# bruno-maruszczak/lap-time-optimization

Hardware: AMD Instinct MI355X
Metric: MPC solves/sec (N=40, nx=8 [7 + progress s], nu=2) (higher is better)
Workload: dtype f64

## Files before the change

### include/ltompc.h

```cpp
#ifndef LTOMPC_H
#define LTOMPC_H

#ifdef __cplusplus
extern "C" {
#endif

#define LTOMPC_NX 8
#define LTOMPC_NU 2
#define LTOMPC_NO_BOUND 1.0e30
#define LTOMPC_TABLE_ROWS 6
#define LTOMPC_NTHETA 16
#define LTOMPC_NLOOP 24

#define LTOMPC_STATUS_SOLVED 0
#define LTOMPC_STATUS_ACCEPTABLE 1
#define LTOMPC_STATUS_MAX_ITER 2
#define LTOMPC_STATUS_NUMERICAL 3
#define LTOMPC_STATUS_STALLED 4
#define LTOMPC_STATUS_INFEASIBLE 5

typedef struct ltompc_params {
  double mass, inertia_z, length_f, length_r, width;
  double B_f, C_f, D_f, B_r, C_r, D_r;
  double C_m, Cr_0, Cr_2, gravity;
  double ptv;
  double q_n, q_mu, q_vy, q_v, vref_scale, q_B;
  double r_du[LTOMPC_NU];
  double x_lb[LTOMPC_NX], x_ub[LTOMPC_NX];
  double u_lb[LTOMPC_NU], u_ub[LTOMPC_NU];
  double ell_penalty, ell_rho, ell_D_f, ell_D_r;
} ltompc_params;

typedef struct ltompc_options {
  double t_step;
  double tol;
  double acceptable_tol;
  double mu_init;
  double mu_min;
  double kappa_eps;
  double kappa_mu;
  double theta_mu;
  double tau_min;
  double bound_push;
  double s_max;
  double delta_w_first;
  double smooth_eps_min;
  double smooth_scale;
  double mu_init_warm;
  double soft_rho;
  double resto_rho;
  double resto_rho_max;
  double resto_rho_factor;
  double dual_inf_max;
  int max_iter;
  int acceptable_iter;
  int n_linesearch;
  int stall_iter;
  int max_ls_fail;
  int warm_shift;
  int warm_reset_on_fail;
  int periodic_tables;
  int max_soc;
  int resto_sticky;
  int node0_check;
  int warm_fallback_iter;
  int resto_shift_retry;
  int max_mu_stay;
  int infeasible_sticky;
  int latency_mode;
} ltompc_options;

typedef struct ltompc_solver* ltompc_handle;

void ltompc_default_params(ltompc_params* p);
void ltompc_default_options(ltompc_options* o);
const char* ltompc_last_error(void);
const char* ltompc_version(void);

int ltompc_create(const ltompc_params* params, const ltompc_options* options, const double* tables,
                  int n_table, int n_horizon, int batch, int device, ltompc_handle* out);
int ltompc_destroy(ltompc_handle h);

int ltompc_set_stream(ltompc_handle h, void* hip_stream);

int ltompc_set_initial_guess(ltompc_handle h, const double* x0);

int ltompc_make_step(ltompc_handle h, const double* x0, double* u0, int* status, int* iters);

int ltompc_make_step_dev(ltompc_handle h, const double* x0_dev, double* u0_dev);

int ltompc_synchronize(ltompc_handle h);

int ltompc_rollout_dev(ltompc_handle h, double* x_dev, int n_ticks, int n_sub, double* u_log_dev, int* status_log_dev,
                       int* iters_log_dev);
int ltompc_rollout_info(ltompc_handle h, long long* iterations, long long* launches);

int ltompc_get_prediction(ltompc_handle h, double* X, double* U);

int ltompc_get_stats(ltompc_handle h, int* status, int* iters, double* kkt_error, double* objective,
                     double* mu);

int ltompc_get_iterate(ltompc_handle h, double* X, double* C, double* U, double* L1, double* L2);

int ltompc_get_ineq(ltompc_handle h, double* T, double* NU, int* n_ineq);

int ltompc_plant_step(ltompc_handle h, const double* x, const double* u, int n_sub, double* x_next);
int ltompc_plant_step_dev(ltompc_handle h, const double* x_dev, const double* u_dev, int n_sub,
                          double* x_next_dev);

int ltompc_slip_forces(ltompc_handle h, const double* x, int batch, double* alpha, double* Fy);

int ltompc_set_initial_guess_dev(ltompc_handle h, const double* x0_dev);

int ltompc_get_counters(ltompc_handle h, int* n_reg, int* n_lsfail);

int ltompc_get_restoration(ltompc_handle h, int* n_resto, double* violation);

int ltompc_get_recovery(ltompc_handle h, int* n_shift, int* n_fallback, double* g0, int* solver_status, double* penalty);

int ltompc_get_sensitivities(ltompc_handle h, double* du0_dp, double* dX_dp, double* dU_dp, int* ok, double* margin);
int ltompc_sensitivities_dev(ltompc_handle h, double* du0_dp_dev, int* ok_dev);

int ltompc_get_param_sensitivities(ltompc_handle h, double* du0_dth, double* dX_dth, double* dU_dth, int* ok);
int ltompc_param_sensitivities_dev(ltompc_handle h, double* du0_dth_dev, int* ok_dev);

int ltompc_get_adjoint(ltompc_handle h, const double* gX, const double* gU, double* grad_p, double* grad_theta, int* ok);
int ltompc_adjoint_dev(ltompc_handle h, const double* gX_dev, const double* gU_dev, double* grad_p_dev, double* grad_theta_dev,
                       int* ok_dev);

int ltompc_get_adjoint_tables(ltompc_handle h, const double* gX, const double* gU, double* grad_tables, double* slot_grad, int* ok);
int ltompc_adjoint_tables_dev(ltompc_handle h, const double* gX_dev, const double* gU_dev, double* grad_tables_dev, double* slot_grad_dev,
                              int* ok_dev);
int ltompc_adjoint_tables_add_dev(ltompc_handle h, const double* gX_dev, const double* gU_dev, double* grad_tables_dev,
                                  double* slot_grad_dev, int* ok_dev);

int ltompc_get_prediction_dev(ltompc_handle h, double* X_dev, double* U_dev);

int ltompc_get_jvp(ltompc_handle h, const double* dp, const double* dtheta, double* tX, double* tU, int* ok);
int ltompc_jvp_dev(ltompc_handle h, const double* dp_dev, const double* dtheta_dev, double* tX_dev, double* tU_dev, int* ok_dev);

int ltompc_set_u_prev(ltompc_handle h, const double* u_prev);
int ltompc_set_u_prev_dev(ltompc_handle h, const double* u_prev_dev);

#define LTOMPC_TABLE_VALUE_ROWS 4
int ltompc_set_table_values(ltompc_handle h, int row, const double* values);
int ltompc_set_table_values_dev(ltompc_handle h, int row, const double* values_dev);
int ltompc_get_table_values(ltompc_handle h, int row, double* values);

int ltompc_set_table_sets(ltompc_handle h, int n_sets, const double* values, const int* set_of_instance);
int ltompc_set_table_sets_dev(ltompc_handle h, int n_sets, const double* values_dev, const int* set_of_instance_dev);
int ltompc_get_table_sets(ltompc_handle h, int* n_sets, double* values, int* set_of_instance);
int ltompc_get_adjoint_table_sets(ltompc_handle h, const double* gX, const double* gU, double* grad_sets, double* slot_grad, int* ok);
int ltompc_adjoint_table_sets_dev(ltompc_handle h, const double* gX_dev, const double* gU_dev, double* grad_sets_dev, double* slot_grad_dev,
                                  int* ok_dev);
int ltompc_adjoint_table_sets_add_dev(ltompc_handle h, const double* gX_dev, const double* gU_dev, double* grad_sets_dev,
                                      double* slot_grad_dev, int* ok_dev);

int ltompc_set_instance_params(ltompc_handle h, const double* theta);
int ltompc_set_instance_params_dev(ltompc_handle h, const double* theta_dev);
int ltompc_get_instance_params(ltompc_handle h, double* theta);

int ltompc_plant_sensitivities(ltompc_handle h, const double* x, const double* u, int n_sub, double* x_next, double* dxn_dx,
                               double* dxn_du, double* dxn_dtheta);
int ltompc_plant_sensitivities_dev(ltompc_handle h, const double* x_dev, const double* u_dev, int n_sub, double* x_next_dev,
                                   double* dxn_dx_dev, double* dxn_du_dev, double* dxn_dtheta_dev);

int ltompc_loop_begin(ltompc_handle h, int mode);
int ltompc_loop_tick_dev(ltompc_handle h, const double* x_dev, const double* u0_dev, int n_sub, double* x_next_dev);
int ltompc_loop_tick(ltompc_handle h, const double* x, const double* u0, int n_sub, double* x_next);
int ltompc_get_loop_sensitivities(ltompc_handle h, double* dx_dq, double* du_dq, int* ok, int* ticks);
int ltompc_loop_sensitivities_dev(ltompc_handle h, double* dx_dq_dev, double* du_dq_dev, int* ok_dev);
int ltompc_loop_end(ltompc_handle h);

int ltompc_reset_instances(ltompc_handle h, const int* mask, const double* x0);
int ltompc_reset_instances_dev(ltompc_handle h, const int* mask_dev, const double* x0_dev);
int ltompc_set_guess(ltompc_handle h, const int* mask, const double* X, const double* C, const double* U, const double* u_prev);
int ltompc_set_guess_dev(ltompc_handle h, const int* mask_dev, const double* X_dev, const double* C_dev, const double* U_dev,
                         const double* u_prev_dev);
int ltompc_warm_state_size(ltompc_handle h);
int ltompc_export_state(ltompc_handle h, const int* idx, int n, double* blob);
int ltompc_export_state_dev(ltompc_handle h, const int* idx_dev, int n, double* blob_dev);
int ltompc_import_state(ltompc_handle h, const int* idx, int n, const double* blob);
int ltompc_import_state_dev(ltompc_handle h, const int* idx_dev, int n, const double* blob_dev);

typedef struct ltompc_record_s* ltompc_record;
long long ltompc_record_size(ltompc_handle h);
int ltompc_record_save(ltompc_handle h, ltompc_record* rec);
int ltompc_record_select(ltompc_handle h, ltompc_record rec);
int ltompc_record_release(ltompc_handle h, ltompc_record rec);
int ltompc_record_trim(ltompc_handle h);
int ltompc_record_stats(ltompc_handle h, int* in_use, int* free_);

int ltompc_set_profiling(ltompc_handle h, int on);
int ltompc_get_timing(ltompc_handle h, double* ms_by_kernel8, int* launches_by_kernel8, int* launches,
                      int* ip_iterations);
int ltompc_get_launch_log(ltompc_handle h, int* kind, int* width, double* ms, int capacity);

int ltompc_get_launch_log_iterations(ltompc_handle h, int* iteration, int capacity);

int ltompc_get_active_history(ltompc_handle h, int* active, int capacity);

int ltompc_get_status_counts(ltompc_handle h, int* counts8, long long* iterations_sum);
int ltompc_get_solver_status_counts(ltompc_handle h, int* counts8);

int ltompc_get_history(ltompc_handle h, int* triples, int capacity);

int ltompc_set_poll_every(ltompc_handle h, int n);

int ltompc_set_narrow_width(ltompc_handle h, int width);

long long ltompc_debug_fetch(ltompc_handle h, int which, void* out, long long nbytes);

int ltompc_test_model(ltompc_handle h, int n, double eps, const double* x, const double* lam, double* f,
                      double* J, double* H, double* cval, double* cgrad, double* cH, double* gval,
                      double* ggrad, double* gH);

int ltompc_test_ellipse(ltompc_handle h, int n, const double* x, double* val, double* grad, double* H);

typedef struct ltompc_vp_vehicle {
  int kind;
  int n_map;
  double mass, friction_coef;
  double lam, D;
  double T, C_m, Cr_0, Cr_2;
  double map_v[16], map_f[16];
} ltompc_vp_vehicle;

int ltompc_velocity_profile(int device, const ltompc_vp_vehicle* vehicle, int n, int batch, const double* s, const double* k,
                            const double* s_max, double* v, double* v_local, double* v_acclim, double* v_declim);

#ifdef __cplusplus
}
#endif
#endif
```

### lap-time-optimization_amd/csrc/aux_kernels.h

```cpp
#pragma once
#include "linearise.h"

namespace ltompc {

template <bool PI = false, bool TS = false>
__device__ __forceinline__ void d_init_slot(const Consts& K, const Work& W, const int k, const int b, const int cold) {
  const int N = W.N;
  double x0[8];
#pragma unroll
  for (int i = 0; i < 8; i++) x0[i] = W.x0[(size_t)i * W.Bp + b];
  if (k == 0) {
#pragma unroll
    for (int i = 0; i < 8; i++) PL(W.X, i, 0, N + 1) = x0[i];
  }
  if (cold) {
#pragma unroll
    for (int i = 0; i < 8; i++) {
      PL(W.X, i, k + 1, N + 1) = x0[i], PL(W.C, i, k, N) = x0[i];
      PL(W.L1, i, k, N) = 0.0, PL(W.L2, i, k, N) = 0.0;
    }
    PL(W.U, 0, k, N) = 0.0, PL(W.U, 1, k, N) = 0.0;
  }
  const int prev = W.si[(size_t)SI_PREV * W.Bp + b];
  const bool resto_ok = K.o.resto_rho > 0.0 && !(K.o.soft_rho > 0.0);
// ... 62 lines not shown
  d_init_slot<true>(K, W, k, b, cold);
}
__global__ void k_init_ts(const Consts* __restrict__ Kp, const WorkTS* __restrict__ Wp, int cold) {
  const Consts& K = *Kp;
  const Work& W = *Wp;
  int tid = blockIdx.x * blockDim.x + threadIdx.x;
  int b = tid % W.Bp, k = tid / W.Bp;
  if (k >= W.N || b >= W.B) return;
  d_init_slot<true, true>(K, W, k, b, cold);
}

__global__ void k_shift(Work W, int pass) {
  int tid = blockIdx.x * blockDim.x + threadIdx.x;
  int b = tid % W.Bp, k = tid / W.Bp;
  const int N = W.N;
  if (k > N || b >= W.B) return;
  if (pass == 0) {
    const int kx = k + 1 <= N ? k + 1 : N, ks = k + 1 <= N - 1 ? k + 1 : N - 1;
#pragma unroll
    for (int i = 0; i < 8; i++) PL(W.dX, i, k, N + 1) = PL(W.X, i, kx, N + 1);
    if (k < N) {
#pragma unroll
      for (int i = 0; i < 8; i++) {
        PL(W.dC, i, k, N) = PL(W.C, i, ks, N);
        PL(W.nL1, i, k, N) = PL(W.L1, i, ks, N), PL(W.nL2, i, k, N) = PL(W.L2, i, ks, N);
      }
      PL(W.dU, 0, k, N) = PL(W.U, 0, ks, N), PL(W.dU, 1, k, N) = PL(W.U, 1, ks, N);
    }
  } else {
#pragma unroll
    for (int i = 0; i < 8; i++) PL(W.X, i, k, N + 1) = PL(W.dX, i, k, N + 1);
    if (k < N) {
#pragma unroll
      for (int i = 0; i < 8; i++) {
        PL(W.C, i, k, N) = PL(W.dC, i, k, N);
        PL(W.L1, i, k, N) = PL(W.nL1, i, k, N), PL(W.L2, i, k, N) = PL(W.nL2, i, k, N);
      }
      PL(W.U, 0, k, N) = PL(W.dU, 0, k, N), PL(W.U, 1, k, N) = PL(W.dU, 1, k, N);
    }
  }
}


__global__ void k_act_identity(int* act, int* nact, int B) {
  int b = blockIdx.x * blockDim.x + threadIdx.x;
  if (b < B) act[b] = b;
  if (b == 0) nact[0] = B;
}
__global__ void __launch_bounds__(1024) k_compact(const int* __restrict__ src, const int* __restrict__ nsrc_p,
                                                   const int* __restrict__ done, int* __restrict__ dst, int* __restrict__ ndst) {
  __shared__ int cnt[1024];
  const int t = threadIdx.x, nsrc = nsrc_p[0];
  const int chunk = (nsrc + 1023) / 1024, lo = t * chunk, hi = min(nsrc, lo + chunk);
  int c = 0;
  for (int j = lo; j < hi; j++) c += done[src[j]] ? 0 : 1;
  cnt[t] = c;
  __syncthreads();
  for (int off = 1; off < 1024; off <<= 1) {
    int v = t >= off ? cnt[t - off] : 0;
    __syncthreads();
    cnt[t] += v;
    __syncthreads();
  }
  int pos = cnt[t] - c;
  for (int j = lo; j < hi; j++) {
    int b = src[j];
    if (!done[b]) dst[pos++] = b;
  }
  if (t == 1023) ndst[0] = cnt[1023];
}

__global__ void __launch_bounds__(1024) k_pack_perm(const int* __restrict__ nslots_p, const int* __restrict__ done, int* __restrict__ perm,
                                                     int* __restrict__ act, int* __restrict__ nact) {
  __shared__ int cnt[1024];
  const int t = threadIdx.x, n = nslots_p[0];
  const int chunk = (n + 1023) / 1024, lo = min(n, t * chunk), hi = min(n, lo + chunk);
  int c = 0;
  for (int j = lo; j < hi; j++) c += done[j] ? 0 : 1;
  cnt[t] = c;
  __syncthreads();
  for (int off = 1; off < 1024; off <<= 1) {
    int v = t >= off ? cnt[t - off] : 0;
    __syncthreads();
    cnt[t] += v;
    __syncthreads();
  }
  const int n_act = cnt[1023];
  int pa = cnt[t] - c, pd = n_act + lo - pa;
  for (int j = lo; j < hi; j++) {
    if (!done[j]) act[pa] = pa, perm[pa++] = j;
    else perm[pd++] = j;
  }
  if (t == 0) nact[0] = n_act;
}
__global__ void k_pack_inverse(const int* __restrict__ orig, int* __restrict__ inv, int B) {
  int j = blockIdx.x * blockDim.x + threadIdx.x;
  if (j < B) inv[orig[j]] = j;
}
__global__ void k_pack(Work W, const int* __restrict__ perm, const int* __restrict__ nslots_p, int nslots_max, int* __restrict__ orig,
                       int ni, int nel, int pass) {
  const int tid = blockIdx.x * blockDim.x + threadIdx.x;
  const int j = tid % nslots_max, k = tid / nslots_max, N = W.N;
  const int nslots = nslots_p ? nslots_p[0] : nslots_max;
  if (k > N || j >= nslots) return;
  const size_t Bp = W.Bp;
  const size_t s = pass == 0 ? perm[j] : j;
  auto mv = [&](gptr<double> dst, gptr<double> src, int nf, int NK) {
    for (int f = 0; f < nf; f++) dst[((size_t)f * NK + k) * Bp + j] = src[((size_t)f * NK + k) * Bp + s];
  };
  if (pass == 0) {
    mv(W.dX, W.X, 8, N + 1);
    if (k < N) mv(W.dC, W.C, 8, N), mv(W.dU, W.U, 2, N), mv(W.nL1, W.L1, 8, N), mv(W.nL2, W.L2, 8, N), mv(W.dT, W.T, ni + 3 + nel, N), mv(W.dNU, W.NU, ni, N);
  } else {
    mv(W.X, W.dX, 8, N + 1);
    if (k < N) mv(W.C, W.dC, 8, N), mv(W.U, W.dU, 2, N), mv(W.L1, W.nL1, 8, N), mv(W.L2, W.nL2, 8, N), mv(W.T, W.dT, ni + 3 + nel, N), mv(W.NU, W.dNU, ni, N);
  }
  if (k == 0) {
    gptr<double> tmp = W.RC;
    gptr<int> itmp = (gptr<int>)(W.RC + (size_t)(10 + ST_NF + 2 * FILTER_MAX) * Bp);
    for (int f = 0; f < 10 + ST_NF + 2 * FILTER_MAX; f++) {
      gptr<double> a = f < 8 ? W.x0 + (size_t)f * Bp : f < 10 ? W.uprev + (size_t)(f - 8) * Bp
                       : f < 10 + ST_NF ? W.st + (size_t)(f - 10) * Bp : W.filt + (size_t)(f - 10 - ST_NF) * Bp;
      if (pass == 0) tmp[(size_t)f * Bp + j] = a[s];
      else a[j] = tmp[(size_t)f * Bp + j];
    }
    for (int f = 0; f <= SI_NF; f++) {
      gptr<int> a = f < SI_NF ? W.si + (size_t)f * Bp : (gptr<int>)orig;
      if (pass == 0) itmp[(size_t)f * Bp + j] = a[s];
      else a[j] = itmp[(size_t)f * Bp + j];
    }
  }
}

__device__ __forceinline__ void d_load_x0(const Work& W, const double* __restrict__ x0_rm, const int b, const size_t r, const int sticky, const int update) {
#pragma unroll
  for (int i = 0; i < 8; i++) W.x0[(size_t)i * W.Bp + b] = x0_rm[r * 8 + i];
  const int node0 = W.si[(size_t)SI_NODE0 * W.Bp + b];
  const int prev = node0 ? node0 - 1 : W.si[(size_t)SI_STATUS * W.Bp + b];
  W.si[(size_t)SI_PREV * W.Bp + b] = prev;
  if (update && sticky > 0) {
    const bool jammed = W.si[(size_t)SI_NRESTO * W.Bp + b] > 0 && !W.si[(size_t)SI_STARTEL * W.Bp + b];
    const int c = W.si[(size_t)SI_STICKY * W.Bp + b];
    W.si[(size_t)SI_STICKY * W.Bp + b] = (prev == LTOMPC_STATUS_INFEASIBLE || jammed) ? sticky : (c > 0 ? c - 1 : 0);
  }
}
__global__ void k_load_x0(Work W, const double* __restrict__ x0_rm, const int* __restrict__ orig, int sticky, int update) {
  int b = blockIdx.x * blockDim.x + threadIdx.x;
  if (b >= W.B) return;
  d_load_x0(W, x0_rm, b, orig ? orig[b] : b, sticky, update);
}
__global__ void k_zero_uprev(Work W) {
  int b = blockIdx.x * blockDim.x + threadIdx.x;
  if (b >= W.B) return;
  W.uprev[b] = 0.0, W.uprev[(size_t)W.Bp + b] = 0.0;
}
__global__ void k_store_u0(Work W, double* __restrict__ u0_rm, const int* __restrict__ orig) {
  int b = blockIdx.x * blockDim.x + threadIdx.x;
  if (b >= W.B) return;
  const int N = W.N;
  const size_t r = orig ? orig[b] : b;
  double a = PL(W.U, 0, 0, N), c = PL(W.U, 1, 0, N);
  if (u0_rm) u0_rm[r * 2] = a, u0_rm[r * 2 + 1] = c;
  W.uprev[b] = a, W.uprev[(size_t)W.Bp + b] = c;
}

__global__ void k_status_counts(Work W, int* __restrict__ counts, unsigned long long* __restrict__ iters_sum) {
  int b = blockIdx.x * blockDim.x + threadIdx.x;
  if (b >= W.B) return;
  const int s = W.si[(size_t)SI_STATUS * W.Bp + b];
  atomicAdd(&counts[s < 0 ? 7 : (s > 7 ? 7 : s)], 1);
  const int n0 = W.si[(size_t)SI_NODE0 * W.Bp + b], ss = n0 ? n0 - 1 : s;
  atomicAdd(&counts[16 + (ss < 0 ? 7 : (ss > 7 ? 7 : ss))], 1);
  atomicAdd(iters_sum, (unsigned long long)W.si[(size_t)SI_ITERS * W.Bp + b]);
}

template <bool PI = false, class TP = const double*, bool TS = false, class VP = const double*>
__device__ __forceinline__ void d_plant(const Consts& K, const double* x, const double* uu, const double dt, const int n_sub, double* y,
                                        const TP th = nullptr, const size_t Bp = 0, const size_t col = 0, const VP tsv = nullptr,
                                        const int set = 0) {
  decltype(auto) p = sel_params<PI>(K.p, th, Bp, col);
  decltype(auto) T = sel_tables<TS>(K.T, tsv, set);
#pragma unroll
  for (int i = 0; i < 8; i++) y[i] = x[i];
  const double hs = dt / n_sub;
  for (int s = 0; s < n_sub; s++) {
    double k1[8], k2[8], k3[8], k4[8], z[8];
    rhs_val(p, T, 0.0, y, uu, k1);
#pragma unroll
    for (int i = 0; i < 8; i++) z[i] = y[i] + 0.5 * hs * k1[i];
    rhs_val(p, T, 0.0, z, uu, k2);
#pragma unroll
    for (int i = 0; i < 8; i++) z[i] = y[i] + 0.5 * hs * k2[i];
    rhs_val(p, T, 0.0, z, uu, k3);
#pragma unroll
    for (int i = 0; i < 8; i++) z[i] = y[i] + hs * k3[i];
    rhs_val(p, T, 0.0, z, uu, k4);
#pragma unroll
    for (int i = 0; i < 8; i++) y[i] += hs / 6.0 * (k1[i] + 2.0 * k2[i] + 2.0 * k3[i] + k4[i]);
  }
}
__global__ void __launch_bounds__(64) k_plant(Consts K, int B, const double* __restrict__ x, const double* __restrict__ u, double dt,
                                              int n_sub, double* __restrict__ xn) {
  int b = blockIdx.x * blockDim.x + threadIdx.x;
  if (b >= B) return;
  double xb[8], y[8], uu[2] = {u[(size_t)b * 2], u[(size_t)b * 2 + 1]};
#pragma unroll
  for (int i = 0; i < 8; i++) xb[i] = x[(size_t)b * 8 + i];
  d_plant(K, xb, uu, dt, n_sub, y);
#pragma unroll
  for (int i = 0; i < 8; i++) xn[(size_t)b * 8 + i] = y[i];
}
__global__ void __launch_bounds__(64) k_plant_pi(Consts K, const double* __restrict__ th, int Bp, int B, const double* __restrict__ x,
                                                 const double* __restrict__ u, double dt, int n_sub, double* __restrict__ xn) {
  int b = blockIdx.x * blockDim.x + threadIdx.x;
  if (b >= B) return;
  double xb[8], y[8], uu[2] = {u[(size_t)b * 2], u[(size_t)b * 2 + 1]};
#pragma unroll
  for (int i = 0; i < 8; i++) xb[i] = x[(size_t)b * 8 + i];
  d_plant<true>(K, xb, uu, dt, n_sub, y, th, Bp, b);
#pragma unroll
  for (int i = 0; i < 8; i++) xn[(size_t)b * 8 + i] = y[i];
}
__global__ void __launch_bounds__(64) k_plant_ts(Consts K, const double* __restrict__ th, const double* __restrict__ tsv,
                                                 const int* __restrict__ tsi, int Bp, int B, const double* __restrict__ x,
                                                 const double* __restrict__ u, double dt, int n_sub, double* __restrict__ xn) {
  int b = blockIdx.x * blockDim.x + threadIdx.x;
  if (b >= B) return;
  double xb[8], y[8], uu[2] = {u[(size_t)b * 2], u[(size_t)b * 2 + 1]};
#pragma unroll
  for (int i = 0; i < 8; i++) xb[i] = x[(size_t)b * 8 + i];
  d_plant<true, const double*, true>(K, xb, uu, dt, n_sub, y, th, Bp, b, tsv, tsi[b]);
#pragma unroll
  for (int i = 0; i < 8; i++) xn[(size_t)b * 8 + i] = y[i];
}

__global__ void k_ts_index(const int* __restrict__ idx, int* __restrict__ tsi, int B, int n_sets) {
  const int b = blockIdx.x * blockDim.x + threadIdx.x;
  if (b >= B) return;
  const int s = idx[b];
  tsi[b] = s < 0 ? 0 : (s >= n_sets ? n_sets - 1 : s);
}

__global__ void k_theta_rows(const double* __restrict__ rows, double* __restrict__ th, int B, int Bp) {
  const int t = blockIdx.x * blockDim.x + threadIdx.x;
  if (t >= B * LTOMPC_NTHETA) return;
  const int b = t / LTOMPC_NTHETA, j = t % LTOMPC_NTHETA;
  th[(size_t)j * Bp + b] = rows[t];
}

__global__ void k_slip_forces(Consts K, int B, const double* __restrict__ x, double* __restrict__ alpha,
                              double* __restrict__ Fy) {
  int b = blockIdx.x * blockDim.x + threadIdx.x;
  if (b >= B) return;
  const ltompc_params& p = K.p;
  const double* xb = x + (size_t)b * 8;
  double af = atan2(xb[4] + p.length_f * xb[5], xb[3]) - xb[6];
  double ar = atan2(xb[4] - p.length_r * xb[5], xb[3]);
  double L = p.length_f + p.length_r;
  double Fnf = p.length_r * p.mass * p.gravity / L, Fnr = p.length_f * p.mass * p.gravity / L;
  alpha[(size_t)b * 2] = af, alpha[(size_t)b * 2 + 1] = ar;
  Fy[(size_t)b * 2] = -Fnf * p.D_f * sin(p.C_f * atan(p.B_f * af));
  Fy[(size_t)b * 2 + 1] = -Fnr * p.D_r * sin(p.C_r * atan(p.B_r * ar));
}

__global__ void k_test_model(Consts K, int n, double eps, const double* __restrict__ x, const double* __restrict__ lam,
                             double* __restrict__ f, double* __restrict__ J, double* __restrict__ H,
                             double* __restrict__ cval, double* __restrict__ cgrad, double* __restrict__ cH,
                             double* __restrict__ gval, double* __restrict__ ggrad, double* __restrict__ gH) {
  int t = blockIdx.x * blockDim.x + threadIdx.x;
  if (t >= n) return;
  double xx[8], ll[8], ff[8], JJ[48], HH[36];
#pragma unroll
  for (int i = 0; i < 8; i++) xx[i] = x[(size_t)t * 8 + i], ll[i] = lam[(size_t)t * 8 + i];
#pragma unroll
  for (int i = 0; i < 36; i++) HH[i] = 0.0;
  rhs_derivs(K.p, K.T, eps, xx, ff, JJ, ll, 1.0, HH);
  for (int i = 0; i < 6; i++) f[(size_t)t * 8 + i] = ff[i];
  f[(size_t)t * 8 + 6] = f[(size_t)t * 8 + 7] = 0.0;
  for (int i = 0; i < 48; i++) J[(size_t)t * 64 + i] = JJ[i];
  for (int i = 48; i < 64; i++) J[(size_t)t * 64 + i] = 0.0;
  for (int i = 0; i < 8; i++)
    for (int j = 0; j < 8; j++) H[(size_t)t * 64 + i * 8 + j] = HH[sidx(i, j)];
  for (int term = 0; term < 2; term++) {
    double g[8] = {0, 0, 0, 0, 0, 0, 0, 0}, Hc[36];
    for (int i = 0; i < 36; i++) Hc[i] = 0.0;
    cval[(size_t)t * 2 + term] = cost_eval(K.p, K.T, eps, xx, term == 1, g, Hc);
    for (int i = 0; i < 8; i++) {
      cgrad[((size_t)t * 2 + term) * 8 + i] = g[i];
      for (int j = 0; j < 8; j++) cH[((size_t)t * 2 + term) * 64 + i * 8 + j] = Hc[sidx(i, j)];
    }
  }
  double gv[3], gs[3], gn[3], gm[3], hss[3], hmm[3];
  cons_eval(K.p, K.T, eps, xx, gv, gs, gn, gm, hss, hmm);
  for (int q = 0; q < 3; q++) {
    gval[(size_t)t * 3 + q] = gv[q];
    for (int i = 0; i < 8; i++) ggrad[((size_t)t * 3 + q) * 8 + i] = 0.0;
    ggrad[((size_t)t * 3 + q) * 8 + 0] = gs[q], ggrad[((size_t)t * 3 + q) * 8 + 1] = gn[q], ggrad[((size_t)t * 3 + q) * 8 + 2] = gm[q];
    for (int i = 0; i < 64; i++) gH[((size_t)t * 3 + q) * 64 + i] = 0.0;
    gH[((size_t)t * 3 + q) * 64 + 0] = hss[q], gH[((size_t)t * 3 + q) * 64 + 2 * 8 + 2] = hmm[q];
  }
}


__global__ void k_test_ellipse(Consts K, int n, const double* __restrict__ x, double* __restrict__ val, double* __restrict__ grad, double* __restrict__ H) {
  int t = blockIdx.x * blockDim.x + threadIdx.x;
  if (t >= n) return;
  double xx[8], v[2], g[2][5], h[2][15], v2[2];
  for (int i = 0; i < 8; i++) xx[i] = x[(size_t)t * 8 + i];
  ellipse_eval(K.p, xx, v, g, h);
  ellipse_val(K.p, xx, v2);
  for (int q = 0; q < 2; q++) {
    val[(size_t)t * 2 + q] = v[q] + (v2[q] - v[q]) * 0.0 + (fabs(v2[q] - v[q]) <= 1e-12 * (1.0 + fabs(v[q])) ? 0.0 : 1e300);
    for (int i = 0; i < 8; i++) grad[((size_t)t * 2 + q) * 8 + i] = i >= 3 ? g[q][i - 3] : 0.0;
    for (int i = 0; i < 8; i++)
      for (int j = 0; j < 8; j++) H[((size_t)t * 2 + q) * 64 + i * 8 + j] = (i >= 3 && j >= 3) ? h[q][sidx(i - 3, j - 3)] : 0.0;
  }
}

}
```

### lap-time-optimization_amd/csrc/linearise.h

```cpp
#pragma once
#include "layout.h"

namespace ltompc {

__device__ __forceinline__ double sym_get(const double* H, int i, int j) { return H[sidx(i, j)]; }


struct BoundsAny {
  static constexpr bool fixed = false;
  static constexpr unsigned ulb = 0, uub = 0, xlb = 0, xub = 0;
};
template <unsigned ULB, unsigned UUB, unsigned XLB, unsigned XUB>
struct BoundsFixed {
  static constexpr bool fixed = true;
  static constexpr unsigned ulb = ULB, uub = UUB, xlb = XLB, xub = XUB;
};
using BoundsRef = BoundsFixed<0x3, 0x3, 0xCD, 0xC4>;

template <class BP, typename F>
__device__ __forceinline__ int for_each_bound(const ltompc_params& p, F&& f) {
  int m = 0;
#pragma unroll
  for (int i = 0; i < 2; i++) {
    if (BP::fixed ? ((BP::ulb >> i) & 1u) != 0 : p.u_lb[i] > -LTOMPC_NO_BOUND) f(m++, 0, i, -1.0, p.u_lb[i]);
    if (BP::fixed ? ((BP::uub >> i) & 1u) != 0 : p.u_ub[i] < LTOMPC_NO_BOUND) f(m++, 0, i, 1.0, p.u_ub[i]);
  }
#pragma unroll
  for (int kind = 1; kind <= 2; kind++) {
#pragma unroll
    for (int i = 0; i < 8; i++) {
      if (BP::fixed ? ((BP::xlb >> i) & 1u) != 0 : p.x_lb[i] > -LTOMPC_NO_BOUND) f(m++, kind, i, -1.0, p.x_lb[i]);
      if (BP::fixed ? ((BP::xub >> i) & 1u) != 0 : p.x_ub[i] < LTOMPC_NO_BOUND) f(m++, kind, i, 1.0, p.x_ub[i]);
    }
  }
  return m;
}

__device__ __forceinline__ void track_barrier(const double rho, const double gv, const double t, const double nu,
                                              const double e, double& Sg, double& s0, double& s1) {
  if (rho > 0.0) {
    const double inu = 1.0 / nu, iz = 1.0 / (rho - nu);
    Sg = 1.0 / (t * inu + e * iz), s0 = nu + Sg * gv, s1 = Sg * (inu - iz);
  } else {
    const double it = 1.0 / t;
    Sg = nu * it, s0 = nu * (gv + t) * it, s1 = it;
  }
}
__device__ __forceinline__ void track_soft_step(const double rho, const double mu, const double tau, const double gv,
                                                const double gd, const double t, const double nu, const double e,
                                                double& dtt, double& dn, double& dee, double& r_pri, double& a_dua,
                                                double& gphid) {
  const double z = rho - nu, inu = 1.0 / nu, iz = 1.0 / z, it = 1.0 / t, ie = 1.0 / e;
  const double Sg = 1.0 / (t * inu + e * iz);
  dn = Sg * (gd + gv + mu * inu - mu * iz);
  dtt = mu * inu - t - t * inu * dn;
  dee = mu * iz - e + e * iz * dn;
  r_pri = fmax(r_pri, fmax(-dtt * it, -dee * ie));
  if (dn < 0.0) a_dua = fmin(a_dua, -tau * nu / dn);
  if (dn > 0.0) a_dua = fmin(a_dua, tau * z / dn);
  gphid += rho * dee - mu * dtt * it - mu * dee * ie;
}

template <class BP, bool TS = false>
__device__ __forceinline__ void init_slot_slacks(const Consts& K, const Work& W, const int k, const int b, const double mu,
                                                 const double eps, const double rho, const double* xp, const double* c,
                                                 const double* u) {
  const int N = W.N;
  const int m = for_each_bound<BP>(K.p, [&](int mm, int kind, int j, double sg, double val) {
    const double xv = kind == 0 ? u[j] : (kind == 1 ? c[j] : xp[j]);
    const double hv = sg * (xv - val);
    const double t = -hv > K.o.bound_push ? -hv : K.o.bound_push;
    PL(W.T, mm, k, N) = t, PL(W.NU, mm, k, N) = mu / t;
  });
  double gv[3] = {-1.0, -1.0, -1.0};
  if (k + 1 <= N - 1) cons_eval(K.p, inst_tables<TS>(K.T, W, b), eps, xp, gv, nullptr, nullptr, nullptr, nullptr, nullptr);
#pragma unroll
  for (int q = 0; q < 3; q++) {
    double t = -gv[q] > K.o.bound_push ? -gv[q] : K.o.bound_push, e = 0.0;
    if (rho > 0.0) {
      t = fmax(t, 2.0 * mu / rho);
      e = mu / (rho - mu / t);
      if (gv[q] > ELASTIC_CP_VIOL) {
        const double g = gv[q], bq = rho * g - 2.0 * mu;
        t = (-bq + sqrt(bq * bq + 4.0 * rho * mu * g)) / (2.0 * rho);
        e = g + t;
      }
    }
    PL(W.T, m + q, k, N) = t, PL(W.T, K.bd.ni + q, k, N) = e, PL(W.NU, m + q, k, N) = mu / t;
  }
  if (K.bd.nel) {
    const double pen = K.p.ell_penalty;
    double ge[2] = {-1.0, -1.0};
    if (k + 1 <= N - 1) ellipse_val(K.p, xp, ge);
#pragma unroll
    for (int q = 0; q < 2; q++) {
      double t = fmax(-ge[q] > K.o.bound_push ? -ge[q] : K.o.bound_push, 2.0 * mu / pen), e = mu / (pen - mu / t);
      if (ge[q] > ELASTIC_CP_VIOL) {
        const double g = ge[q], bq = pen * g - 2.0 * mu;
        t = (-bq + sqrt(bq * bq + 4.0 * pen * mu * g)) / (2.0 * pen);
        e = g + t;
      }
      PL(W.T, m + 3 + q, k, N) = t, PL(W.T, K.bd.ni + 3 + q, k, N) = e, PL(W.NU, m + 3 + q, k, N) = mu / t;
    }
  }
}
template <class BP, bool TS = false>
__device__ __forceinline__ void reinit_slot(const Consts& K, const Work& W, const int k, const int b) {
  const int N = W.N;
  const double mu = W.st[(size_t)ST_MU * W.Bp + b], eps = W.st[(size_t)ST_EPS * W.Bp + b], rho = W.st[(size_t)ST_RHO * W.Bp + b];
  double xp[8], c[8], u[2];
#pragma unroll
  for (int i = 0; i < 8; i++) xp[i] = PL(W.X, i, k + 1, N + 1), c[i] = PL(W.C, i, k, N);
  u[0] = PL(W.U, 0, k, N), u[1] = PL(W.U, 1, k, N);
  init_slot_slacks<BP, TS>(K, W, k, b, mu, eps, rho, xp, c, u);
#pragma unroll
  for (int i = 0; i < 8; i++) PL(W.L1, i, k, N) = 0.0, PL(W.L2, i, k, N) = 0.0;
}

struct Slot {
  double xk[8], xp[8], c[8], u[2];
  double E1[64], E2[64], G1[8], G2[8];
  double Hc[36], gc0[8], gc1[8];
  double Hxp[36], gxp0[8], gxp1[8];
  double Du[2], gub0[2], gub1[2];
  double dcd[8], dxd[8], dud[2];
  double gcost[8];
  double gs[3], gn[3], gm[3];
  double gv[3];
  double gve[2], ge[2][5];
  double rp_ineq, cmax, cmin, smult;
  double th_ineq, sumlog;
  double emax;
  double cost;
  int m_nl;
  bool nl;
};

template <bool WITH_DUAL, class BP, bool ELL, bool PI = false, bool TS = false>
__device__ __forceinline__ void linearise_slot(const Consts& K, const Work& W, int k, int b, double eps, Slot& S) {
  const int N = W.N;
  const double hdt = K.o.t_step, rho = W.st[(size_t)ST_RHO * W.Bp + b];
#pragma unroll
  for (int i = 0; i < 8; i++) {
    S.xk[i] = k == 0 ? W.x0[(size_t)i * W.Bp + b] : PL(W.X, i, k, N + 1);
    S.xp[i] = PL(W.X, i, k + 1, N + 1);
    S.c[i] = PL(W.C, i, k, N);
  }
  S.u[0] = PL(W.U, 0, k, N), S.u[1] = PL(W.U, 1, k, N);
  double l1[8], l2[8];
#pragma unroll
  for (int i = 0; i < 8; i++) l1[i] = PL(W.L1, i, k, N), l2[i] = PL(W.L2, i, k, N);
#pragma unroll
  for (int i = 0; i < 36; i++) S.Hc[i] = 0.0, S.Hxp[i] = 0.0;
  double f1[8], f2[8], J[48];
  rhs_derivs(inst_params<PI>(K.p, W, b), inst_tables<TS>(K.T, W, b), eps, S.c, f1, J, l1, hdt, S.Hc);
#pragma unroll
  for (int i = 0; i < 64; i++) S.E1[i] = 0.0, S.E2[i] = 0.0;
#pragma unroll
  for (int i = 0; i < 48; i++) S.E1[i] = hdt * J[i];
  rhs_derivs(inst_params<PI>(K.p, W, b), inst_tables<TS>(K.T, W, b), eps, S.xp, f2, J, l2, hdt, S.Hxp);
#pragma unroll
  for (int i = 0; i < 48; i++) S.E2[i] = hdt * J[i];
  f1[6] = f2[6] = S.u[0], f1[7] = f2[7] = S.u[1];
#pragma unroll
  for (int i = 0; i < 8; i++) {
    S.E1[i * 8 + i] -= 1.5, S.E2[i * 8 + i] -= 2.5;
    S.G1[i] = hdt * f1[i] + 2.0 * S.xk[i] - 1.5 * S.c[i] - 0.5 * S.xp[i];
    S.G2[i] = hdt * f2[i] - 2.0 * S.xk[i] + 4.5 * S.c[i] - 2.5 * S.xp[i];
  }
#pragma unroll
  for (int i = 0; i < 8; i++) S.gcost[i] = 0.0, S.gc0[i] = 0.0, S.gc1[i] = 0.0, S.gxp1[i] = 0.0, S.dcd[i] = 0.0;
  S.cost = cost_eval(inst_params<PI>(K.p, W, b), inst_tables<TS>(K.T, W, b), eps, S.xp, k == N - 1, S.gcost, S.Hxp);
#pragma unroll
  for (int i = 0; i < 8; i++) S.gxp0[i] = S.gcost[i], S.dxd[i] = S.gcost[i];
  S.Du[0] = S.Du[1] = 0.0, S.gub0[0] = S.gub0[1] = 0.0, S.gub1[0] = S.gub1[1] = 0.0, S.dud[0] = S.dud[1] = 0.0;
  S.rp_ineq = 0.0, S.cmax = 0.0, S.cmin = 1e300, S.smult = 0.0, S.th_ineq = 0.0, S.sumlog = 0.0, S.emax = 0.0;
  double lprod = 1.0;
  const int m_nl = for_each_bound<BP>(K.p, [&](int m, int kind, int j, double sg, double val) {
    const double xv = kind == 0 ? S.u[j] : (kind == 1 ? S.c[j] : S.xp[j]);
    const double hv = sg * (xv - val);
    const double t = PL(W.T, m, k, N), nu = PL(W.NU, m, k, N), it = 1.0 / t;
    const double Sg = nu * it, g0 = sg * nu * (hv + t) * it, g1 = sg * it;
    if (kind == 0) {
      S.Du[j] += Sg, S.gub0[j] += g0, S.gub1[j] += g1;
      if (WITH_DUAL) S.dud[j] += sg * nu;
    } else if (kind == 1) {
      S.Hc[sidx(j, j)] += Sg, S.gc0[j] += g0, S.gc1[j] += g1;
      if (WITH_DUAL) S.dcd[j] += sg * nu;
    } else {
      S.Hxp[sidx(j, j)] += Sg, S.gxp0[j] += g0, S.gxp1[j] += g1;
      if (WITH_DUAL) S.dxd[j] += sg * nu;
    }
    if (WITH_DUAL) {
      S.rp_ineq = fmax(S.rp_ineq, fabs(hv + t));
      S.cmax = fmax(S.cmax, t * nu), S.cmin = fmin(S.cmin, t * nu), S.smult += fabs(nu);
      S.th_ineq += fabs(hv + t), lprod *= t;
      if ((m & 7) == 7) S.sumlog += log(lprod), lprod = 1.0;
    }
  });
  S.m_nl = m_nl;
  S.nl = (k + 1 <= N - 1);
  if (S.nl) {
    double tq[3], nq[3], eq[3];
#pragma unroll
    for (int q = 0; q < 3; q++) {
      tq[q] = PL(W.T, m_nl + q, k, N), nq[q] = PL(W.NU, m_nl + q, k, N);
      eq[q] = rho > 0.0 ? PL(W.T, K.bd.ni + q, k, N) : 0.0;
    }
#if defined(__HIP_DEVICE_COMPILE__)
    asm volatile("" : "+v"(tq[0]), "+v"(tq[1]), "+v"(tq[2]), "+v"(nq[0]), "+v"(nq[1]), "+v"(nq[2]), "+v"(eq[0]), "+v"(eq[1]), "+v"(eq[2]));
#endif
    double hss[3], hmm[3];
    cons_eval(K.p, inst_tables<TS>(K.T, W, b), eps, S.xp, S.gv, S.gs, S.gn, S.gm, hss, hmm);
#pragma unroll
    for (int q = 0; q < 3; q++) {
      int mm = m_nl + q;
      double t = tq[q], nu = nq[q];
      const double e = eq[q];
      double Sg, s0, s1;
      track_barrier(rho, S.gv[q], t, nu, e, Sg, s0, s1);
      double g3[3] = {S.gs[q], S.gn[q], S.gm[q]};
#pragma unroll
      for (int a = 0; a < 3; a++) {
        S.gxp0[a] += s0 * g3[a], S.gxp1[a] += s1 * g3[a];
        if (WITH_DUAL) S.dxd[a] += nu * g3[a];
#pragma unroll
        for (int c = 0; c <= a; c++) S.Hxp[sidx(a, c)] += Sg * g3[a] * g3[c];
      }
      S.Hxp[sidx(0, 0)] += nu * hss[q];
      S.Hxp[sidx(2, 2)] += nu * hmm[q];
      if (WITH_DUAL) {
        S.rp_ineq = fmax(S.rp_ineq, fabs(S.gv[q] - e + t));
        S.cmax = fmax(S.cmax, t * nu), S.cmin = fmin(S.cmin, t * nu), S.smult += fabs(nu);
        S.th_ineq += fabs(S.gv[q] - e + t), lprod *= t;
        if (rho > 0.0) {
          const double ez = e * (rho - nu);
          S.cmax = fmax(S.cmax, ez), S.cmin = fmin(S.cmin, ez), S.smult += fabs(rho - nu);
          lprod *= e, S.cost += rho * e, S.emax = fmax(S.emax, e);
        }
        if ((mm & 7) == 7) S.sumlog += log(lprod), lprod = 1.0;
      }
    }
  } else {
#pragma unroll
    for (int q = 0; q < 3; q++) S.gv[q] = -1.0, S.gs[q] = S.gn[q] = S.gm[q] = 0.0;
  }
  if (ELL && S.nl) {
    const double pen = K.p.ell_penalty;
    double te[2], ne[2], ee[2];
#pragma unroll
    for (int q = 0; q < 2; q++) te[q] = PL(W.T, m_nl + 3 + q, k, N), ne[q] = PL(W.NU, m_nl + 3 + q, k, N), ee[q] = PL(W.T, K.bd.ni + 3 + q, k, N);
    double h15[2][15];
    ellipse_eval(K.p, S.xp, S.gve, S.ge, h15);
#pragma unroll
    for (int q = 0; q < 2; q++) {
      const int mm = m_nl + 3 + q;
      const double t = te[q], nu = ne[q], e = ee[q];
      double Sg, s0, s1;
      track_barrier(pen, S.gve[q], t, nu, e, Sg, s0, s1);
#pragma unroll
      for (int a = 0; a < 5; a++) {
        S.gxp0[3 + a] += s0 * S.ge[q][a], S.gxp1[3 + a] += s1 * S.ge[q][a];
        if (WITH_DUAL) S.dxd[3 + a] += nu * S.ge[q][a];
#pragma unroll
        for (int c = 0; c <= a; c++) S.Hxp[sidx(3 + a, 3 + c)] += Sg * S.ge[q][a] * S.ge[q][c] + nu * h15[q][sidx(a, c)];
      }
      if (WITH_DUAL) {
        const double ez = e * (pen - nu);
        S.rp_ineq = fmax(S.rp_ineq, fabs(S.gve[q] - e + t));
        S.cmax = fmax(S.cmax, fmax(t * nu, ez)), S.cmin = fmin(S.cmin, fmin(t * nu, ez)), S.smult += fabs(nu) + fabs(pen - nu);
        S.th_ineq += fabs(S.gve[q] - e + t), lprod *= t, lprod *= e, S.cost += pen * e;
        if ((mm & 7) == 7) S.sumlog += log(lprod), lprod = 1.0;
      }
    }
  }
  if (WITH_DUAL) S.sumlog += log(lprod);
}

__host__ __device__ constexpr int gs_(int i) { return i < 3 ? 0 : (i < 6 ? 3 : 6); }
__host__ __device__ constexpr int ge_(int i) { return i < 3 ? 2 : (i < 6 ? 5 : 7); }
__host__ __device__ constexpr int elo_(int i) { return i < 6 ? gs_(i) : i; }
__host__ __device__ constexpr int ehi_(int i) { return i < 3 ? 5 : (i < 6 ? 7 : i); }
__host__ __device__ constexpr int yrow_(int col) { return col < 8 ? ge_(col) : 7; }
__host__ __device__ constexpr bool hnz_(int i, int j) { return (i <= 4 && j <= 4) || (i >= 3 && i <= 6 && j >= 3 && j <= 6) || i == j; }
__host__ __device__ constexpr int imin_(int x, int y) { return x < y ? x : y; }
__host__ __device__ constexpr int imax_(int x, int y) { return x > y ? x : y; }

struct M8Blocks {
  double iaa[9], ibb[9];
  double ab[9], ac[6], bc[6];
};

__device__ __forceinline__ bool inv33(const double* m, double* r) {
  const double c00 = m[4] * m[8] - m[5] * m[7], c01 = m[5] * m[6] - m[3] * m[8], c02 = m[3] * m[7] - m[4] * m[6];
  const double det = m[0] * c00 + m[1] * c01 + m[2] * c02;
  const double id = 1.0 / det;
  r[0] = c00 * id, r[1] = (m[2] * m[7] - m[1] * m[8]) * id, r[2] = (m[1] * m[5] - m[2] * m[4]) * id;
  r[3] = c01 * id, r[4] = (m[0] * m[8] - m[2] * m[6]) * id, r[5] = (m[2] * m[3] - m[0] * m[5]) * id;
  r[6] = c02 * id, r[7] = (m[1] * m[6] - m[0] * m[7]) * id, r[8] = (m[0] * m[4] - m[1] * m[3]) * id;
  return fabs(det) > 1e-12;
}

template <int RMAX>
__device__ __forceinline__ void m8_solve(const M8Blocks& M, const double* v, double* y) {
  double yc[2] = {0.0, 0.0}, yb[3] = {0.0, 0.0, 0.0};
  if (RMAX >= 6) {
    yc[0] = v[6] * (1.0 / 12.0), yc[1] = v[7] * (1.0 / 12.0);
    y[6] = yc[0], y[7] = yc[1];
  }
  if (RMAX >= 3) {
    double rb[3];
#pragma unroll
    for (int i = 0; i < 3; i++) {
      rb[i] = v[3 + i];
      if (RMAX >= 6) rb[i] -= M.bc[i * 2] * yc[0] + M.bc[i * 2 + 1] * yc[1];
    }
#pragma unroll
    for (int i = 0; i < 3; i++) yb[i] = M.ibb[i * 3] * rb[0] + M.ibb[i * 3 + 1] * rb[1] + M.ibb[i * 3 + 2] * rb[2], y[3 + i] = yb[i];
  }
  double ra[3];
#pragma unroll
  for (int i = 0; i < 3; i++) {
    ra[i] = v[i];
    if (RMAX >= 3) ra[i] -= M.ab[i * 3] * yb[0] + M.ab[i * 3 + 1] * yb[1] + M.ab[i * 3 + 2] * yb[2];
    if (RMAX >= 6) ra[i] -= M.ac[i * 2] * yc[0] + M.ac[i * 2 + 1] * yc[1];
  }
#pragma unroll
  for (int i = 0; i < 3; i++) y[i] = M.iaa[i * 3] * ra[0] + M.iaa[i * 3 + 1] * ra[1] + M.iaa[i * 3 + 2] * ra[2];
}
__device__ __forceinline__ void m8_solve_t(const M8Blocks& M, const double* v, double* x) {
#pragma unroll
  for (int i = 0; i < 3; i++) x[i] = M.iaa[i] * v[0] + M.iaa[3 + i] * v[1] + M.iaa[6 + i] * v[2];
  double rb[3];
#pragma unroll
  for (int i = 0; i < 3; i++) rb[i] = v[3 + i] - (M.ab[i] * x[0] + M.ab[3 + i] * x[1] + M.ab[6 + i] * x[2]);
#pragma unroll
  for (int i = 0; i < 3; i++) x[3 + i] = M.ibb[i] * rb[0] + M.ibb[3 + i] * rb[1] + M.ibb[6 + i] * rb[2];
#pragma unroll
  for (int i = 0; i < 2; i++) {
    double s = v[6 + i];
#pragma unroll
    for (int l = 0; l < 3; l++) s -= M.ac[l * 2 + i] * x[l] + M.bc[l * 2 + i] * x[3 + l];
    x[6 + i] = s * (1.0 / 12.0);
  }
}

template <int COL>
__device__ __forceinline__ void condense_column(const Consts& K, const Slot& S, const M8Blocks& M, double* Y, double* AB) {
  const double hdt = K.o.t_step;
  constexpr int RM = yrow_(COL);
  double v[8] = {0, 0, 0, 0, 0, 0, 0, 0}, y[8] = {0, 0, 0, 0, 0, 0, 0, 0};
  if (COL < 8) {
#pragma unroll
    for (int i = 0; i <= RM; i++) v[i] = ((i == COL) ? 2.0 : 0.0) - ((COL >= elo_(i) && COL <= ehi_(i)) ? 4.0 * S.E2[i * 8 + COL] : 0.0);
  } else if (COL < 10) {
    constexpr int j = 6 + COL - 8;
#pragma unroll
    for (int i = 0; i < 8; i++) v[i] = -hdt * (((i == j) ? 1.0 : 0.0) + ((j >= elo_(i) && j <= ehi_(i)) ? 2.0 * S.E2[i * 8 + j] : 0.0));
  } else {
#pragma unroll
    for (int i = 0; i < 8; i++) {
      double s = -S.G2[i];
#pragma unroll
      for (int l = elo_(i); l <= ehi_(i); l++) s -= 2.0 * S.E2[i * 8 + l] * S.G1[l];
      v[i] = s;
    }
  }
  m8_solve<RM>(M, v, y);
#pragma unroll
  for (int i = 0; i <= RM; i++) Y[i * 11 + COL] = y[i];
#pragma unroll
  for (int i = 0; i < 8; i++) {
    double s;
    if (COL < 8) s = (i == COL) ? 2.0 : 0.0;
    else if (COL < 10) s = (i == 6 + COL - 8) ? hdt : 0.0;
    else s = S.G1[i];
#pragma unroll
    for (int l = elo_(i); l <= imin_(ehi_(i), RM); l++) s += S.E1[i * 8 + l] * y[l];
    AB[i * 11 + COL] = 2.0 * s;
  }
}

__device__ __forceinline__ bool factor_m8(const Slot& S, M8Blocks& M) {
  double maa[9], mbb[9];
#pragma unroll
  for (int i = 0; i < 6; i++)
#pragma unroll
    for (int j = gs_(i); j < 8; j++) {
      double s = (i == j) ? 4.5 : 0.0;
#pragma unroll
      for (int l = elo_(i); l <= imin_(ehi_(i), ge_(j)); l++)
        if (j >= elo_(l) && j <= ehi_(l)) s += 2.0 * S.E2[i * 8 + l] * S.E1[l * 8 + j];
      if (i < 3) {
        if (j < 3) maa[i * 3 + j] = s;
        else if (j < 6) M.ab[i * 3 + j - 3] = s;
        else M.ac[i * 2 + j - 6] = s;
      } else {
        if (j < 6) mbb[(i - 3) * 3 + j - 3] = s;
        else M.bc[(i - 3) * 2 + j - 6] = s;
      }
    }
  return inv33(maa, M.iaa) & inv33(mbb, M.ibb);
}

__device__ __forceinline__ bool condense_slot(const Consts& K, const Slot& S, M8Blocks& M, double* Y, double* AB) {
  const bool ok = factor_m8(S, M);
#pragma unroll
  for (int q = 0; q < 88; q++) Y[q] = 0.0, AB[q] = 0.0;
  condense_column<0>(K, S, M, Y, AB), condense_column<1>(K, S, M, Y, AB), condense_column<2>(K, S, M, Y, AB);
  condense_column<3>(K, S, M, Y, AB), condense_column<4>(K, S, M, Y, AB), condense_column<5>(K, S, M, Y, AB);
  condense_column<6>(K, S, M, Y, AB), condense_column<7>(K, S, M, Y, AB), condense_column<8>(K, S, M, Y, AB);
  condense_column<9>(K, S, M, Y, AB), condense_column<10>(K, S, M, Y, AB);
  return ok;
}


template <class BP, bool ELL, bool PI = false, bool TS = false>
__device__ __forceinline__ void d_eval(const Consts& K, const Work& W, const int k, const int b, const bool force) {
  const int N = W.N;
  if (W.si[(size_t)SI_DONE * W.Bp + b]) return;
  if (!force && (W.si[(size_t)SI_RETRY * W.Bp + b] || W.si[(size_t)SI_SKIP_EVAL * W.Bp + b])) return;
  const double hdt = K.o.t_step;
  const double eps = W.st[(size_t)ST_EPS * W.Bp + b];
  const bool reinit = W.si[(size_t)SI_REINIT * W.Bp + b] != 0;
  if (reinit) reinit_slot<BP, TS>(K, W, k, b);
  Slot S;
  linearise_slot<true, BP, ELL, PI, TS>(K, W, k, b, eps, S);
#pragma unroll
  for (int i = 0; i < 36; i++) PG(W.QP, QP_Qx + i, k + 1, QP_NF) = S.Hxp[i];
#pragma unroll
  for (int i = 0; i < 8; i++) PG(W.QP, QP_qx0 + i, k + 1, QP_NF) = S.gxp0[i], PG(W.QP, QP_qx1 + i, k + 1, QP_NF) = S.gxp1[i];
  {
    double l1[8], l2[8], l1n[8], l2n[8], rd = 0.0, rp = 0.0, sm = 0.0;
    const int kn = k + 1 < N ? k + 1 : k;
    const bool nxt = k + 1 < N && !reinit;
#pragma unroll
    for (int i = 0; i < 8; i++) l1[i] = PL(W.L1, i, k, N), l2[i] = PL(W.L2, i, k, N), l1n[i] = PL(W.L1, i, kn, N), l2n[i] = PL(W.L2, i, kn, N);
#pragma unroll
    for (int a = 0; a < 8; a++) {
      double rcx = S.dcd[a] + 4.5 * l2[a];
      double rxp = S.dxd[a] - 0.5 * l1[a];
#pragma unroll
      for (int i = 0; i <= ge_(a); i++)
        if (a >= elo_(i) && a <= ehi_(i)) rcx += S.E1[i * 8 + a] * l1[i], rxp += S.E2[i * 8 + a] * l2[i];
      {
        const double t = 2.0 * l1n[a] - 2.0 * l2n[a];
        const double r2 = rxp + t;
        rxp = nxt ? r2 : rxp;
      }
      rd = fmax(rd, fmax(fabs(rcx), fabs(rxp)));
      rp = fmax(rp, fmax(fabs(S.G1[a]), fabs(S.G2[a])));
      sm += fabs(l1[a]) + fabs(l2[a]);
    }
    double cost = S.cost;
#pragma unroll
    for (int i = 0; i < 2; i++) {
      double v = k ? PL(W.U, i, k - 1, N) : W.uprev[(size_t)i * W.Bp + b];
      double du = S.u[i] - v;
      const double rdu = inst_r_du<PI>(K.p, W, b, i);
      cost += rdu * du * du;
      double ru = S.dud[i] + 2.0 * rdu * du + hdt * (l1[6 + i] + l2[6 + i]);
      if (k + 1 < N) ru -= 2.0 * rdu * (PL(W.U, i, k + 1, N) - S.u[i]);
      rd = fmax(rd, fabs(ru));
    }
    rp = fmax(rp, S.rp_ineq), sm += S.smult;
    const double cmax = S.cmax, cmin = S.cmin;
    double th0 = S.th_ineq;
#pragma unroll
    for (int a = 0; a < 8; a++) th0 += fabs(S.G1[a]) + fabs(S.G2[a]);
    PL(W.LS, 0, k, N) = th0, PL(W.LS, 1, k, N) = cost, PL(W.LS, 2, k, N) = S.sumlog;
    PL(W.RS, RS_rd, k, N) = rd, PL(W.RS, RS_rp, k, N) = rp, PL(W.RS, RS_cmax, k, N) = cmax;
    PL(W.RS, RS_cmin, k, N) = cmin, PL(W.RS, RS_smult, k, N) = sm, PL(W.RS, RS_cost, k, N) = cost;
    PL(W.RS, RS_emax, k, N) = S.emax;
  }
  M8Blocks M8;
  double Y[88], AB[88];
  condense_slot(K, S, M8, Y, AB);
#pragma unroll
  for (int i = 0; i < 8; i++) {
#pragma unroll
    for (int j = 0; j < 8; j++) PG(W.QP, QP_A + i * 8 + j, k, QP_NF) = AB[i * 11 + j];
    PG(W.QP, QP_B + i * 2 + 0, k, QP_NF) = AB[i * 11 + 8], PG(W.QP, QP_B + i * 2 + 1, k, QP_NF) = AB[i * 11 + 9];
    PG(W.QP, QP_b + i, k, QP_NF) = AB[i * 11 + 10];
  }
  double HY[88];
#pragma unroll
  for (int i = 0; i < 8; i++)
#pragma unroll
    for (int col = 0; col < 11; col++) {
      double s = 0.0;
#pragma unroll
      for (int l = 0; l <= yrow_(col); l++)
        if (hnz_(i, l)) s += sym_get(S.Hc, i, l) * Y[l * 11 + col];
      HY[i * 11 + col] = s;
    }
#pragma unroll
  for (int i = 0; i < 10; i++) {
#pragma unroll
    for (int j = 0; j < 10; j++) {
      if (j > i) continue;
      double s = 0.0;
#pragma unroll
      for (int l = 0; l <= yrow_(i); l++) s += Y[l * 11 + i] * HY[l * 11 + j];
      if (i < 8) PG(W.QP, QP_Q + sidx(i, j), k, QP_NF) = s;
      else if (j < 8) PG(W.QP, QP_S + (i - 8) * 8 + j, k, QP_NF) = s;
      else PG(W.QP, QP_R + sidx(i - 8, j - 8), k, QP_NF) = s + ((i == j) ? S.Du[i - 8] : 0.0);
    }
    double s0 = 0.0, s1 = 0.0;
#pragma unroll
    for (int l = 0; l <= yrow_(i); l++) s0 += Y[l * 11 + i] * (HY[l * 11 + 10] + S.gc0[l]), s1 += Y[l * 11 + i] * S.gc1[l];
    if (i < 8) PG(W.QP, QP_q0 + i, k, QP_NF) = s0, PG(W.QP, QP_q1 + i, k, QP_NF) = s1;
    else PG(W.QP, QP_r0 + i - 8, k, QP_NF) = s0 + S.gub0[i - 8], PG(W.QP, QP_r1 + i - 8, k, QP_NF) = s1 + S.gub1[i - 8];
  }
}

template <class BP, bool ELL>
// ... 207 lines not shown
```

### lap-time-optimization_amd/csrc/linesearch.h

```cpp
#pragma once
#include "layout.h"

namespace ltompc {

template <class BP, bool PIN, bool ELL, bool PI = false, bool TS = false>
__device__ __forceinline__ void d_linesearch(const Consts& K, const Work& W, const int k, const int b, const int l_begin,
                                             const int l_end) {
  const int N = W.N;
  const double hdt = K.o.t_step;
  if (W.si[(size_t)SI_DONE * W.Bp + b] || !W.si[(size_t)SI_STEP * W.Bp + b]) return;
  const double eps = W.st[(size_t)ST_EPS * W.Bp + b], rho = W.st[(size_t)ST_RHO * W.Bp + b];
  double a_pri = 1.0;
  for (int kk = 0; kk < N; kk += 20) {
    double v20[20];
#pragma unroll
    for (int q = 0; q < 20; q++) v20[q] = PL(W.SP, SP_apri, kk + q < N ? kk + q : N - 1, N);
#pragma unroll
    for (int q = 0; q < 20; q++) a_pri = fmin(a_pri, v20[q]);
  }
  double xk[8], xp[8], c[8], u[2], v[2], dxk[8], dxp[8], dc[8], du[2], dv[2];
#pragma unroll
  for (int i = 0; i < 8; i++) {
    xk[i] = k == 0 ? W.x0[(size_t)i * W.Bp + b] : PL(W.X, i, k, N + 1);
    dxk[i] = PL(W.dX, i, k, N + 1);
    xp[i] = PL(W.X, i, k + 1, N + 1), dxp[i] = PL(W.dX, i, k + 1, N + 1);
    c[i] = PL(W.C, i, k, N), dc[i] = PL(W.dC, i, k, N);
  }
#pragma unroll
  for (int i = 0; i < 2; i++) {
    u[i] = PL(W.U, i, k, N), du[i] = PL(W.dU, i, k, N);
    v[i] = k ? PL(W.U, i, k - 1, N) : W.uprev[(size_t)i * W.Bp + b];
    dv[i] = k ? PL(W.dU, i, k - 1, N) : 0.0;
  }
  const bool nl = (k + 1 <= N - 1);
  for (int l = l_begin; l <= l_end; l++) {
    const double alpha = l == 0 ? 0.0 : ldexp(a_pri, -(l - 1));
    double txk[8], txp[8], tc[8], tu[2], tv[2];
#pragma unroll
    for (int i = 0; i < 8; i++) txk[i] = xk[i] + alpha * dxk[i], txp[i] = xp[i] + alpha * dxp[i], tc[i] = c[i] + alpha * dc[i];
#pragma unroll
    for (int i = 0; i < 2; i++) tu[i] = u[i] + alpha * du[i], tv[i] = v[i] + alpha * dv[i];
    double f1[8], f2[8];
    rhs_val(inst_params<PI>(K.p, W, b), inst_tables<TS>(K.T, W, b), eps, tc, tu, f1);
    rhs_val(inst_params<PI>(K.p, W, b), inst_tables<TS>(K.T, W, b), eps, txp, tu, f2);
    double th = 0.0;
#pragma unroll
    for (int i = 0; i < 8; i++) {
      th += fabs(hdt * f1[i] + 2.0 * txk[i] - 1.5 * tc[i] - 0.5 * txp[i]);
      th += fabs(hdt * f2[i] - 2.0 * txk[i] + 4.5 * tc[i] - 2.5 * txp[i]);
    }
    double co = cost_eval(inst_params<PI>(K.p, W, b), inst_tables<TS>(K.T, W, b), eps, txp, k == N - 1, nullptr, nullptr);
#pragma unroll
    for (int i = 0; i < 2; i++) co += inst_r_du<PI>(K.p, W, b, i) * (tu[i] - tv[i]) * (tu[i] - tv[i]);
    double sl = 0.0, pr = 1.0;
    double tt[BP::fixed ? MAX_NI : 1];
    if (BP::fixed) {
      double t0[MAX_NI] = {}, d0[MAX_NI] = {};
      const int nb = for_each_bound<BP>(K.p, [&](int mm, int, int, double, double) { t0[mm] = PL(W.T, mm, k, N), d0[mm] = PL(W.dT, mm, k, N); });
#pragma unroll
      for (int q = 0; q < MAX_NI; q += 8)
        if (PIN && q < nb) {
#if defined(__HIP_DEVICE_COMPILE__)
          double* a = t0 + q;
          double* c = d0 + q;
          asm volatile("" : "+v"(a[0]), "+v"(a[1]), "+v"(a[2]), "+v"(a[3]), "+v"(a[4]), "+v"(a[5]), "+v"(a[6]), "+v"(a[7]),
                            "+v"(c[0]), "+v"(c[1]), "+v"(c[2]), "+v"(c[3]), "+v"(c[4]), "+v"(c[5]), "+v"(c[6]), "+v"(c[7]));
#endif
        }
#pragma unroll
      for (int q = 0; q < MAX_NI; q++)
        if (q < nb) tt[q] = t0[q] + alpha * d0[q];
    }
    const int m = for_each_bound<BP>(K.p, [&](int mm, int kind, int jj, double sg, double val) {
      const double xv = kind == 0 ? tu[jj] : (kind == 1 ? tc[jj] : txp[jj]);
      const double t = BP::fixed ? tt[mm] : PL(W.T, mm, k, N) + alpha * PL(W.dT, mm, k, N);
      th += fabs(sg * (xv - val) + t), pr *= t;
      if ((mm & 7) == 7) sl += log(pr), pr = 1.0;
    });
    if (nl) {
      double gv[3];
      cons_eval(K.p, inst_tables<TS>(K.T, W, b), eps, txp, gv, nullptr, nullptr, nullptr, nullptr, nullptr);
#pragma unroll
      for (int q = 0; q < 3; q++) {
        double t = PL(W.T, m + q, k, N) + alpha * PL(W.dT, m + q, k, N);
        double e = 0.0;
        pr *= t;
        if (rho > 0.0) {
          e = PL(W.T, K.bd.ni + q, k, N) + alpha * PL(W.dT, K.bd.ni + q, k, N);
          pr *= e, co += rho * e;
        }
        th += fabs(gv[q] - e + t);
        if (((m + q) & 7) == 7) sl += log(pr), pr = 1.0;
      }
      if (ELL) {
        double ge[2];
        ellipse_val(K.p, txp, ge);
#pragma unroll
        for (int q = 0; q < 2; q++) {
          const int mm = m + 3 + q, me = K.bd.ni + 3 + q;
          const double t = PL(W.T, mm, k, N) + alpha * PL(W.dT, mm, k, N);
          const double e = PL(W.T, me, k, N) + alpha * PL(W.dT, me, k, N);
          pr *= t, pr *= e, co += K.p.ell_penalty * e;
          th += fabs(ge[q] - e + t);
          if ((mm & 7) == 7) sl += log(pr), pr = 1.0;
        }
      }
    }
    sl += log(pr);
    PL(W.LS, 3 * l + 0, k, N) = th, PL(W.LS, 3 * l + 1, k, N) = co, PL(W.LS, 3 * l + 2, k, N) = sl;
  }
}

template <class BP, bool ELL>
__global__ void __launch_bounds__(64) k_linesearch(const Consts* __restrict__ Kp, const Work* __restrict__ Wp, Launch la, int phase, int jw) {
  const Consts& K = *Kp;
  const Work& W = *Wp;
  const int tid = blockIdx.x * blockDim.x + threadIdx.x;
  const int N = W.N;
  const int j0 = tid % jw, rest = tid / jw, k = rest % N, cand = rest / N;
  if (phase == 0 ? (rest >= N) : (cand >= K.o.n_linesearch - 1)) return;
  const int count = phase == 0 ? la.nact[0] : W.ls_count[0];
  const int l = phase == 0 ? 1 : 2 + cand;
  for (int j = j0; j < count; j += jw) d_linesearch<BP, true, ELL>(K, W, k, phase == 0 ? la.act[j] : W.ls_list[j], l, l);
}
template <class BP>
__global__ void __launch_bounds__(64) k_linesearch_pi(const Consts* __restrict__ Kp, const WorkPI* __restrict__ Wp, Launch la, int phase, int jw) {
  const Consts& K = *Kp;
  const Work& W = *Wp;
  const int tid = blockIdx.x * blockDim.x + threadIdx.x;
  const int N = W.N;
  const int j0 = tid % jw, rest = tid / jw, k = rest % N, cand = rest / N;
  if (phase == 0 ? (rest >= N) : (cand >= K.o.n_linesearch - 1)) return;
  const int count = phase == 0 ? la.nact[0] : W.ls_count[0];
  const int l = phase == 0 ? 1 : 2 + cand;
  for (int j = j0; j < count; j += jw) d_linesearch<BP, true, false, true>(K, W, k, phase == 0 ? la.act[j] : W.ls_list[j], l, l);
}

template <class BP>
__global__ void __launch_bounds__(64) k_linesearch_ts(const Consts* __restrict__ Kp, const WorkTS* __restrict__ Wp, Launch la, int phase, int jw) {
  const Consts& K = *Kp;
  const Work& W = *Wp;
  const int tid = blockIdx.x * blockDim.x + threadIdx.x;
  const int N = W.N;
  const int j0 = tid % jw, rest = tid / jw, k = rest % N, cand = rest / N;
  if (phase == 0 ? (rest >= N) : (cand >= K.o.n_linesearch - 1)) return;
  const int count = phase == 0 ? la.nact[0] : W.ls_count[0];
  const int l = phase == 0 ? 1 : 2 + cand;
  for (int j = j0; j < count; j += jw) d_linesearch<BP, true, false, true, true>(K, W, k, phase == 0 ? la.act[j] : W.ls_list[j], l, l);
}

constexpr int PICK_Q = 5;
template <bool PI = false, bool TS = false>
__device__ __forceinline__ void d_pick(const Consts& K, const Work& W, const int b, const int i, const int phase,
                                       const bool append_list) {
  const int N = W.N;
  double* st = W.st;
  int* si = W.si;
  const ltompc_options& o = K.o;
  int done = STI(SI_DONE), step = STI(SI_STEP);
  double mu = STD(ST_MU), eps = STD(ST_EPS), eps_next = STD(ST_EPS_NEXT), force_reg = STD(ST_FORCE_REG), theta0 = STD(ST_THETA0);
  double theta_max = STD(ST_THMAX), theta_min = STD(ST_THMIN), c00 = STD(ST_C00), rho = STD(ST_RHO);
  int nfilt = STI(SI_NFILT), nlsfail = STI(SI_NLSFAIL), ntiny = STI(SI_NTINY), resto = STI(SI_RESTO), nresto = STI(SI_NRESTO);
  int warm = STI(SI_WARM), nshift = STI(SI_NSHIFT), blowup = STI(SI_BLOWUP), iters = STI(SI_ITERS);
  double x0[8];
#pragma unroll
  for (int q = 0; q < 8; q++) x0[q] = W.x0[(size_t)q * W.Bp + b];
  double fth[FILTER_MAX], fph[FILTER_MAX];
#pragma unroll
  for (int f = 0; f < FILTER_MAX; f++) fth[f] = W.filt[(size_t)(2 * f) * W.Bp + b], fph[f] = W.filt[(size_t)(2 * f + 1) * W.Bp + b];
  double sp[3][PICK_Q], ls[6][PICK_Q];
#pragma unroll
  for (int q = 0; q < PICK_Q; q++) {
    const int k = i + 8 * q < N ? i + 8 * q : N - 1;
    sp[0][q] = PL(W.SP, SP_apri, k, N), sp[1][q] = PL(W.SP, SP_adua, k, N), sp[2][q] = PL(W.SP, SP_gphid, k, N);
#pragma unroll
    for (int f = 0; f < 6; f++) ls[f][q] = PL(W.LS, f, k, N);
  }
#if defined(__HIP_DEVICE_COMPILE__)
#define LT_PIN8(a) asm volatile("" : "+v"((a)[0]), "+v"((a)[1]), "+v"((a)[2]), "+v"((a)[3]), "+v"((a)[4]), "+v"((a)[5]), "+v"((a)[6]), "+v"((a)[7]))
  asm volatile("" : "+v"(mu), "+v"(eps), "+v"(eps_next), "+v"(force_reg), "+v"(theta0), "+v"(theta_max), "+v"(theta_min), "+v"(c00), "+v"(rho));
  asm volatile("" : "+v"(nfilt), "+v"(nlsfail), "+v"(ntiny), "+v"(resto), "+v"(nresto), "+v"(warm), "+v"(nshift), "+v"(blowup), "+v"(iters),
                    "+v"(done), "+v"(step));
  LT_PIN8(x0);
  static_assert(FILTER_MAX % 8 == 0, "the filter is pinned in chunks of 8 pairs");
#pragma unroll
  for (int f = 0; f < FILTER_MAX; f += 8) LT_PIN8(fth + f);
#pragma unroll
  for (int f = 0; f < FILTER_MAX; f += 8) LT_PIN8(fph + f);
#pragma unroll
  for (int q = 0; q < PICK_Q; q++)
    asm volatile("" : "+v"(sp[0][q]), "+v"(sp[1][q]), "+v"(sp[2][q]), "+v"(ls[0][q]), "+v"(ls[1][q]), "+v"(ls[2][q]), "+v"(ls[3][q]), "+v"(ls[4][q]), "+v"(ls[5][q]));
#undef LT_PIN8
#endif
  if (done || !step) return;
  double a_pri = 1.0, a_dua = 1.0, gphid = 0.0;
#pragma unroll
  for (int q = 0; q < PICK_Q; q++)
    if (i + 8 * q < N) a_pri = fmin(a_pri, sp[0][q]), a_dua = fmin(a_dua, sp[1][q]), gphid += sp[2][q];
  for (int k0 = i + 8 * PICK_Q; k0 < N; k0 += 8 * PICK_Q) {
    double v[3][PICK_Q];
#pragma unroll
    for (int q = 0; q < PICK_Q; q++) {
      const int k = k0 + 8 * q < N ? k0 + 8 * q : k0;
      v[0][q] = PL(W.SP, SP_apri, k, N), v[1][q] = PL(W.SP, SP_adua, k, N), v[2][q] = PL(W.SP, SP_gphid, k, N);
    }
#pragma unroll
    for (int q = 0; q < PICK_Q; q++)
      if (k0 + 8 * q < N) a_pri = fmin(a_pri, v[0][q]), a_dua = fmin(a_dua, v[1][q]), gphid += v[2][q];
  }
  a_pri = grp_min(a_pri), a_dua = grp_min(a_dua), gphid = grp_sum(gphid);
  auto sums6 = [&](const int lA, const int lB, const int kbeg, double (&s)[6]) {
    for (int k0 = kbeg; k0 < N; k0 += 8 * PICK_Q) {
      double v[6][PICK_Q];
#pragma unroll
      for (int q = 0; q < PICK_Q; q++) {
        const int k = k0 + 8 * q < N ? k0 + 8 * q : k0;
#pragma unroll
        for (int f = 0; f < 3; f++) v[f][q] = PL(W.LS, 3 * lA + f, k, N), v[3 + f][q] = PL(W.LS, 3 * lB + f, k, N);
      }
#pragma unroll
      for (int q = 0; q < PICK_Q; q++)
        if (k0 + 8 * q < N) {
#pragma unroll
          for (int f = 0; f < 6; f++) s[f] += v[f][q];
        }
    }
  };
  auto measures = [&](double (&s)[6], double& thA, double& phA, double& thB, double& phB) {
#pragma unroll
    for (int f = 0; f < 6; f++) s[f] = grp_sum(s[f]);
    thA = s[0], phA = (c00 + s[1]) - mu * s[2], thB = s[3], phB = (c00 + s[4]) - mu * s[5];
  };
  double th0, ph0, th1, ph1;
  {
    double s[6] = {};
#pragma unroll
    for (int q = 0; q < PICK_Q; q++)
      if (i + 8 * q < N) {
#pragma unroll
        for (int f = 0; f < 6; f++) s[f] += ls[f][q];
      }
    sums6(0, 1, i + 8 * PICK_Q, s);
    measures(s, th0, ph0, th1, ph1);
  }
  const bool th_init = theta0 < 0.0;
  if (th_init) {
    theta0 = th0, theta_max = 1e4 * fmax(1.0, theta0), theta_min = 1e-4 * fmax(1.0, theta0);
    nfilt = 0;
  }
  const double g_th = 1e-5, g_ph = 1e-8, eta_ph = 1e-8, s_th = 1.1, s_ph = 2.3, dlt = 1.0;
  const double S = pen_scale(rho), iS = 1.0 / S;
  bool accepted = false;
  double alpha = a_pri;
  const int n_ls = o.n_linesearch;
  const int n_try = (phase == 0) ? 1 : n_ls;
  bool f_shift = false;
  int f_at = -1;
  auto try_candidate = [&](const double th, const double ph) -> bool {
    if (!isfinite(th) || !isfinite(ph) || th > theta_max) return false;
    bool in_filter = false;
#pragma unroll
    for (int f = 0; f < FILTER_MAX; f++) in_filter = in_filter || (f < nfilt && th >= fth[f] && ph >= fph[f]);
    if (in_filter) return false;
    bool sw = (gphid < 0.0) && (alpha * pow(-gphid * iS, s_ph) > dlt * pow(th0, s_th));
    bool armijo = ph <= ph0 + eta_ph * alpha * gphid;
    bool ok;
    if (th0 <= theta_min && sw) ok = armijo;
    else ok = (th <= (1.0 - g_th) * th0) || (ph <= ph0 - g_ph * S * th0);
    if (!ok) return false;
    if (!(sw && armijo)) {
      if (nfilt == FILTER_MAX) f_shift = true, nfilt--;
      f_at = nfilt;
      nfilt++;
    }
    return true;
  };
  accepted = try_candidate(th1, ph1);
  if (!accepted) alpha *= 0.5;
  for (int l = 1; l < n_try && !accepted; l += 2) {
    double thA, phA, thB, phB;
    double s[6] = {};
    sums6(l + 1, l + 2 <= n_ls ? l + 2 : l + 1, i, s);
    measures(s, thA, phA, thB, phB);
    accepted = try_candidate(thA, phA);
    if (!accepted) {
      alpha *= 0.5;
      if (l + 1 < n_try) {
        accepted = try_candidate(thB, phB);
        if (!accepted) alpha *= 0.5;
      }
    }
  }
  if (i != 0) return;
  if (phase == 0 && !accepted && n_ls > 1) {
    STI(SI_LSMORE) = 1;
    if (th_init) STD(ST_THETA0) = theta0, STD(ST_THMAX) = theta_max, STD(ST_THMIN) = theta_min;
    if (append_list) W.ls_list[atomicAdd(W.ls_count, 1)] = b;
    return;
  }
  const bool resto_ready = o.resto_rho > 0.0 && !(o.soft_rho > 0.0) && resto == 0;
  bool take = true, give_up = false, enter_resto = false, stalled = false, shift = false;
  bool th_reset = false;
  if (!accepted) {
    nlsfail += 1;
    const double fr = force_reg;
    if (resto_ready) {
      enter_resto = true, take = false;
    } else if (o.max_ls_fail > 0 && nlsfail >= o.max_ls_fail) {
      give_up = true, take = false;
    } else if (fr < 1e4 * S) {
      force_reg = fr == 0.0 ? 1e-2 * S : fr * 100.0;
      take = false;
    } else {
      nfilt = 0;
      alpha = a_pri * pow(0.5, (double)(n_ls - 1));
    }
  }
  if (give_up) stalled = true;
  if (take) {
    force_reg = 0.0;
    ntiny = alpha <= 1e-3 ? ntiny + 1 : 0;
    if ((o.stall_iter > 0 && ntiny >= o.stall_iter) || (resto_ready && blowup)) {
      if (resto_ready) enter_resto = true;
      else stalled = true;
      take = false;
    }
  }
  if (enter_resto) {
    shift = o.resto_shift_retry && !o.warm_shift && warm && nshift == 0;
    double rho_new = 0.0;
    if (!shift) resto = 1, nresto += 1, rho_new = o.resto_rho;
    rho = rho_new, mu = o.mu_init * pen_scale(rho_new);
    eps_next = (o.smooth_scale > 0 || o.smooth_eps_min > 0) ? fmax(o.smooth_eps_min, o.smooth_scale * o.mu_init) : 0.0;
    if (eps_next == eps) nfilt = 0, th_reset = true;
    force_reg = 0.0, ntiny = 0;
  }
  if (!stalled) iters += 1;
  const bool eps_switched = eps_next != eps;
  if (eps_switched) {
    c00 = cost_eval(inst_params<PI>(K.p, W, b), inst_tables<TS>(K.T, W, b), eps_next, x0, false, nullptr, nullptr);
    nfilt = 0, th_reset = true;
  }
  STI(SI_LSMORE) = 0;
  if (f_shift) {
#pragma unroll
    for (int f = 0; f + 1 < FILTER_MAX; f++) W.filt[(size_t)(2 * f) * W.Bp + b] = fth[f + 1], W.filt[(size_t)(2 * f + 1) * W.Bp + b] = fph[f + 1];
  }
  if (f_at >= 0) {
    W.filt[(size_t)(2 * f_at) * W.Bp + b] = (1.0 - g_th) * th0;
    W.filt[(size_t)(2 * f_at + 1) * W.Bp + b] = ph0 - g_ph * S * th0;
  }
  if (th_init) STD(ST_THMAX) = theta_max, STD(ST_THMIN) = theta_min;
  if (th_init || th_reset) STD(ST_THETA0) = th_reset ? -1.0 : theta0;
  if (!accepted) STI(SI_NLSFAIL) = nlsfail;
  if (stalled) STI(SI_STATUS) = LTOMPC_STATUS_STALLED, STI(SI_DONE) = 1;
  if (enter_resto) {
    if (shift) STI(SI_SHIFT) = 1, STI(SI_NSHIFT) = 1;
    else STI(SI_RESTO) = resto, STI(SI_NRESTO) = nresto;
    STI(SI_REINIT) = 1;
    STD(ST_RHO) = rho, STD(ST_MU) = mu;
    STD(ST_EPS_NEXT) = eps_next;
    STD(ST_DW_LAST) = 0.0;
    STI(SI_NACC) = 0, STI(SI_SINCEMU) = 0;
  }
  STD(ST_FORCE_REG) = force_reg;
  STI(SI_NTINY) = ntiny;
  STD(ST_ALPHA) = take ? alpha : 0.0, STD(ST_ADUA) = a_dua;
  STI(SI_STEP) = take ? 1 : 0;
  STI(SI_ITERS) = iters;
  if (eps_switched) STD(ST_EPS) = eps_next, STD(ST_C00) = c00;
  STI(SI_NFILT) = nfilt;
  STI(SI_SKIP_EVAL) = (!take && !eps_switched && !enter_resto) ? 1 : 0;
}

__global__ void __launch_bounds__(64) k_pick(const Consts* __restrict__ Kp, const Work* __restrict__ Wp, Launch la, int phase) {
  const Consts& K = *Kp;
  const Work& W = *Wp;
  const int lane = threadIdx.x, g = lane & 7, i = lane >> 3;
  const int count = phase == 0 ? la.nact[0] : W.ls_count[0];
  for (int j = blockIdx.x * 8 + g; j < count; j += gridDim.x * 8) d_pick(K, W, phase == 0 ? la.act[j] : W.ls_list[j], i, phase, true);
}
__global__ void __launch_bounds__(64) k_pick_pi(const Consts* __restrict__ Kp, const WorkPI* __restrict__ Wp, Launch la, int phase) {
  const Consts& K = *Kp;
  const Work& W = *Wp;
  const int lane = threadIdx.x, g = lane & 7, i = lane >> 3;
  const int count = phase == 0 ? la.nact[0] : W.ls_count[0];
  for (int j = blockIdx.x * 8 + g; j < count; j += gridDim.x * 8) d_pick<true>(K, W, phase == 0 ? la.act[j] : W.ls_list[j], i, phase, true);
}

__global__ void __launch_bounds__(64) k_pick_ts(const Consts* __restrict__ Kp, const WorkTS* __restrict__ Wp, Launch la, int phase) {
  const Consts& K = *Kp;
  const Work& W = *Wp;
  const int lane = threadIdx.x, g = lane & 7, i = lane >> 3;
  const int count = phase == 0 ? la.nact[0] : W.ls_count[0];
  for (int j = blockIdx.x * 8 + g; j < count; j += gridDim.x * 8) d_pick<true, true>(K, W, phase == 0 ? la.act[j] : W.ls_list[j], i, phase, true);
}

__device__ __forceinline__ void d_update(const Consts& K, const Work& W, const int k, const int b) {
  const int N = W.N;
  if (W.si[(size_t)SI_SHIFT * W.Bp + b] && !W.si[(size_t)SI_DONE * W.Bp + b]) {
    const size_t ob = W.orig[b];
    const int ks = k + 1 <= N - 1 ? k + 1 : N - 1;
    double v[18];
#pragma unroll
// ... 147 lines not shown
```

### lap-time-optimization_amd/csrc/ltompc.hip

```cpp
#include <hip/hip_runtime.h>

#include <algorithm>
#include <cmath>
#include <cstdio>
#include <cstdlib>
#include <cstring>
#include <string>
#include <type_traits>
#include <vector>

#include "kernels.h"

using namespace ltompc;

namespace {

thread_local std::string g_err;

int fail(const std::string& msg) {
  g_err = msg;
  return -1;
}
#define HIPCHECK(expr)                                                                         \
  do {                                                                                         \
// ... 1105 lines not shown
        hipLaunchKernelGGL(k_roll_plant_ts, dim3((n_launch + 63) / 64), dim3(64), 0, ps, h->K, h->Wts, x_dev, h->K.o.t_step, n_sub, (const int*)(d_cnt + 1),
                           (const int*)d_list);
      else if (h->pi_solve)
        hipLaunchKernelGGL(k_roll_plant_pi, dim3((n_launch + 63) / 64), dim3(64), 0, ps, h->K, h->Wpi, x_dev, h->K.o.t_step, n_sub, (const int*)(d_cnt + 1),
                           (const int*)d_list);
      else
      hipLaunchKernelGGL(k_roll_plant, dim3((n_launch + 63) / 64), dim3(64), 0, ps, h->K, h->W, x_dev, h->K.o.t_step, n_sub, (const int*)(d_cnt + 1),
                         (const int*)d_list);
      ROLLCHECK(hipEventRecord(h->ev_done[slot], ps));
      done_pending[slot] = true;
    }
    first = false;
    if ((it + 1) % h->poll_every == 0) {
      ROLLCHECK(hipMemcpyAsync(h->h_active, d_cnt, sizeof(int), hipMemcpyDeviceToHost, h->stream));
      ROLLCHECK(hipMemcpyAsync(h->h_active + 1, h->W.ls_count + 1, sizeof(int), hipMemcpyDeviceToHost, h->stream));
      ROLLCHECK(hipStreamSynchronize(h->stream));
      const int n_left = h->h_active[0];
      h->history.push_back((int)it), h->history.push_back(n_left), h->history.push_back(n_launch);
      if (h->ls_width_env == 0) {
        const int last = h->h_active[1];
        ls_width = std::min(std::max(64, (last + last / 2 + 63) / 64 * 64), 2048);
      }
      if (n_left == 0) break;
      if (it >= it_cap) { rc = fail("ltompc_rollout: iteration cap reached (internal error)"); break; }
      if (h->compaction && n_left <= (h->pack_num * n_launch) / 8) {
        hipLaunchKernelGGL(k_compact, dim3(1), dim3(1024), 0, h->stream, h->d_act[cur], h->d_nact[cur], h->W.si + (size_t)SI_FINAL * Bp,
                           h->d_act[cur ^ 1], h->d_nact[cur ^ 1]);
        cur ^= 1;
        set_launch(n_left);
      }
    }
  }
#undef ROLLCHECK
  for (int i = 0; i < h->n_plant_streams; i++)
    if (hipStreamSynchronize(h->plant_streams[i]) != hipSuccess && rc == 0) rc = fail("ltompc_rollout: plant stream failed");
  if (hipStreamSynchronize(h->stream) != hipSuccess && rc == 0) rc = fail("ltompc_rollout: solver stream failed");
  if (hipGetLastError() != hipSuccess && rc == 0) rc = fail("ltompc_rollout: a kernel launch failed");
  h->profiling = prof;
  h->cold_next = false;
  h->roll_iterations = it + 1, h->roll_launches = L.launches;
  h->last_iterations = 0;
  h->after_rollout = true;
  if (rc == 0) h->dv.solved(false);
  return rc;
}

int ltompc_get_prediction_dev(ltompc_handle h, double* X_dev, double* U_dev) {
  if (!h) return fail("null handle");
  if (!X_dev && !U_dev) return 0;
  HIPCHECK(hipSetDevice(h->device));
  const size_t nthreads = (size_t)(h->N + 1) * h->Bp;
  hipLaunchKernelGGL(k_prediction_dev, dim3((unsigned)((nthreads + 255) / 256)), dim3(256), 0, h->stream, h->W, X_dev, U_dev);
  HIPCHECK(hipGetLastError());
  return 0;
}

int ltompc_set_instance_params(ltompc_handle h, const double* theta) {
  static const char* names[LTOMPC_NTHETA] = {"mass", "inertia_z", "B_f", "C_f", "D_f", "B_r", "C_r", "D_r", "C_m", "Cr_0", "Cr_2",
                                             "q_n", "q_mu", "q_B", "r_du[0]", "r_du[1]"};
  if (!h) return fail("null handle");
  if (!theta) {
    h->pi_pend = false;
    return 0;
  }
  const char* who = "ltompc_set_instance_params";
  for (int b = 0; b < h->B; b++)
    for (int j = 0; j < LTOMPC_NTHETA; j++) {
      const double v = theta[(size_t)b * LTOMPC_NTHETA + j];
      const char* why = !std::isfinite(v) ? "is not finite" : (j < 2 && !(v > 0.0)) ? "must be > 0" : (j >= 11 && !(v >= 0.0)) ? "must be >= 0" : nullptr;
      if (why) return fail(std::string(who) + ": row " + std::to_string(b) + ", column " + std::to_string(j) + " (" + names[j] + ") " + why);
    }
  HIPCHECK(hipSetDevice(h->device));
  if (theta_prepare(h, who)) return -1;
  const size_t Bp = h->Bp;
  std::vector<double> plane((size_t)LTOMPC_NTHETA * h->B);
  for (int b = 0; b < h->B; b++)
    for (int j = 0; j < LTOMPC_NTHETA; j++) plane[(size_t)j * h->B + b] = theta[(size_t)b * LTOMPC_NTHETA + j];
  HIPCHECK(hipMemcpy2DAsync(h->d_th_pend, Bp * sizeof(double), plane.data(), h->B * sizeof(double), h->B * sizeof(double), LTOMPC_NTHETA,
                            hipMemcpyHostToDevice, h->stream));
  HIPCHECK(hipStreamSynchronize(h->stream));
  h->pi_pend = true;
  return 0;
}

int ltompc_set_instance_params_dev(ltompc_handle h, const double* theta_dev) {
  if (!h) return fail("null handle");
  if (!theta_dev) {
    h->pi_pend = false;
    return 0;
  }
  HIPCHECK(hipSetDevice(h->device));
  if (theta_prepare(h, "ltompc_set_instance_params_dev")) return -1;
  hipLaunchKernelGGL(k_theta_rows, dim3((h->B * LTOMPC_NTHETA + 255) / 256), dim3(256), 0, h->stream, theta_dev, h->d_th_pend, h->B, h->Bp);
  HIPCHECK(hipGetLastError());
  h->pi_pend = true;
  return 0;
}

int ltompc_get_instance_params(ltompc_handle h, double* theta) {
  if (!h || !theta) return fail("ltompc_get_instance_params: null argument");
  if (!h->pi_pend) {
    for (int b = 0; b < h->B; b++) theta_of(h->K.p, theta + (size_t)b * LTOMPC_NTHETA);
    return 0;
  }
  HIPCHECK(hipSetDevice(h->device));
  return planes_to_host(h, h->d_th_pend, LTOMPC_NTHETA, 1, theta);
}

int ltompc_rollout_info(ltompc_handle h, long long* iterations, long long* launches) {
  if (!h) return fail("null handle");
  if (iterations) *iterations = h->roll_iterations;
  if (launches) *launches = h->roll_launches;
  return 0;
}

int ltompc_make_step(ltompc_handle h, const double* x0, double* u0, int* status, int* iters) {
  if (!h || !x0 || !u0) return fail("ltompc_make_step: null argument");
  HIPCHECK(hipSetDevice(h->device));
  for (size_t i = 0; i < (size_t)8 * h->B; i++)
    if (!std::isfinite(x0[i])) return fail("ltompc_make_step: non-finite x0");
  HIPCHECK(hipMemcpyAsync(h->d_x0_rm, x0, sizeof(double) * 8 * h->B, hipMemcpyHostToDevice, h->stream));
  int rc = ltompc_make_step_dev(h, h->d_x0_rm, h->d_u0_rm);
  if (rc) return rc;
  HIPCHECK(hipMemcpyAsync(u0, h->d_u0_rm, sizeof(double) * 2 * h->B, hipMemcpyDeviceToHost, h->stream));
  HIPCHECK(hipStreamSynchronize(h->stream));
  if (status || iters) return ltompc_get_stats(h, status, iters, nullptr, nullptr, nullptr);
  return 0;
}

int ltompc_get_prediction(ltompc_handle h, double* X, double* U) {
  if (!h) return fail("null handle");
  HIPCHECK(hipSetDevice(h->device));
  if (ensure_unpacked(h)) return -1;
  if (planes_to_host(h, h->W.X, 8, h->N + 1, X)) return -1;
  return planes_to_host(h, h->W.U, 2, h->N, U);
}

int ltompc_get_iterate(ltompc_handle h, double* X, double* C, double* U, double* L1, double* L2) {
  if (!h) return fail("null handle");
  HIPCHECK(hipSetDevice(h->device));
  if (ensure_unpacked(h)) return -1;
  if (planes_to_host(h, h->W.X, 8, h->N + 1, X)) return -1;
  if (planes_to_host(h, h->W.C, 8, h->N, C)) return -1;
  if (planes_to_host(h, h->W.U, 2, h->N, U)) return -1;
  if (planes_to_host(h, h->W.L1, 8, h->N, L1)) return -1;
  return planes_to_host(h, h->W.L2, 8, h->N, L2);
}

int ltompc_get_ineq(ltompc_handle h, double* T, double* NU, int* n_ineq) {
  if (!h) return fail("null handle");
  HIPCHECK(hipSetDevice(h->device));
  if (ensure_unpacked(h)) return -1;
  if (n_ineq) *n_ineq = h->K.bd.ni;
  if (planes_to_host(h, h->W.T, h->K.bd.ni, h->N, T)) return -1;
  return planes_to_host(h, h->W.NU, h->K.bd.ni, h->N, NU);
}

int ltompc_plant_step_dev(ltompc_handle h, const double* x_dev, const double* u_dev, int n_sub, double* x_next_dev) {
  if (!h || !x_dev || !u_dev || !x_next_dev) return fail("ltompc_plant_step: null argument");
  if (n_sub < 1) return fail("ltompc_plant_step: n_sub must be >= 1");
  HIPCHECK(hipSetDevice(h->device));
  if (h->n_sets)
    hipLaunchKernelGGL(k_plant_ts, dim3((h->B + 63) / 64), dim3(64), 0, h->stream, h->K, (const double*)(h->pi_pend ? h->d_th_pend : h->d_th_unif),
                       (const double*)h->d_ts_vals, (const int*)h->d_ts_idx, h->Bp, h->B, x_dev, u_dev, h->K.o.t_step, n_sub, x_next_dev);
  else if (h->pi_pend)
    hipLaunchKernelGGL(k_plant_pi, dim3((h->B + 63) / 64), dim3(64), 0, h->stream, h->K, (const double*)h->d_th_pend, h->Bp, h->B, x_dev, u_dev,
                       h->K.o.t_step, n_sub, x_next_dev);
  else hipLaunchKernelGGL(k_plant, dim3((h->B + 63) / 64), dim3(64), 0, h->stream, h->K, h->B, x_dev, u_dev, h->K.o.t_step, n_sub, x_next_dev);
  HIPCHECK(hipGetLastError());
  return 0;
}

int ltompc_plant_step(ltompc_handle h, const double* x, const double* u, int n_sub, double* x_next) {
  if (!h || !x || !u || !x_next) return fail("ltompc_plant_step: null argument");
  HIPCHECK(hipSetDevice(h->device));
  return via_io(h, x, u, x_next, [&](double* dx, double* du, double* dn) { return ltompc_plant_step_dev(h, dx, du, n_sub, dn); });
}

int ltompc_slip_forces(ltompc_handle h, const double* x, int batch, double* alpha, double* Fy) {
  if (!h || !x || !alpha || !Fy) return fail("ltompc_slip_forces: null argument");
  if (batch < 1 || batch > h->B) return fail("ltompc_slip_forces: batch must be in [1, handle batch]");
  HIPCHECK(hipSetDevice(h->device));
  double *dx = h->d_io, *da = h->d_io + 8 * (size_t)h->Bp, *df = h->d_io + 10 * (size_t)h->Bp;
  HIPCHECK(hipMemcpyAsync(dx, x, sizeof(double) * 8 * batch, hipMemcpyHostToDevice, h->stream));
  hipLaunchKernelGGL(k_slip_forces, dim3((batch + 63) / 64), dim3(64), 0, h->stream, h->K, batch, dx, da, df);
  HIPCHECK(hipGetLastError());
  HIPCHECK(hipMemcpyAsync(alpha, da, sizeof(double) * 2 * batch, hipMemcpyDeviceToHost, h->stream));
  HIPCHECK(hipMemcpyAsync(Fy, df, sizeof(double) * 2 * batch, hipMemcpyDeviceToHost, h->stream));
  HIPCHECK(hipStreamSynchronize(h->stream));
  return 0;
}

int ltompc_get_timing(ltompc_handle h, double* ms_by_kernel8, int* launches_by_kernel8, int* launches, int* ip_iterations) {
  if (!h) return fail("null handle");
  for (int i = 0; i < NKERN; i++) {
    if (ms_by_kernel8) ms_by_kernel8[i] = h->ms_by_kernel[i];
    if (launches_by_kernel8) launches_by_kernel8[i] = h->launches_by_kernel[i];
  }
  if (launches) *launches = h->last_launches;
  if (ip_iterations) *ip_iterations = h->last_iterations;
  return 0;
}

int ltompc_get_launch_log(ltompc_handle h, int* kind, int* width, double* ms, int capacity) {
  if (!h) return fail("null handle");
  const int n = (int)h->log_kind.size();
  for (int i = 0; i < n && i < capacity; i++) {
    if (kind) kind[i] = h->log_kind[i];
    if (width) width[i] = h->log_width[i];
    if (ms) ms[i] = h->log_ms[i];
  }
  return n;
}

int ltompc_get_launch_log_iterations(ltompc_handle h, int* iteration, int capacity) {
  if (!h) return fail("null handle");
  const int n = (int)h->log_iter.size();
  for (int i = 0; i < n && i < capacity; i++)
    if (iteration) iteration[i] = h->log_iter[i];
  return n;
}

int ltompc_get_active_history(ltompc_handle h, int* active, int capacity) {
  if (!h) return fail("null handle");
  HIPCHECK(hipSetDevice(h->device));
  const int n = h->after_rollout ? 0 : std::min(h->last_iterations, h->max_iter + 2);
  if (active && capacity > 0 && n > 0) {
    HIPCHECK(hipMemcpyAsync(active, h->W.active, sizeof(int) * std::min(n, capacity), hipMemcpyDeviceToHost, h->stream));
    HIPCHECK(hipStreamSynchronize(h->stream));
  }
  return n;
}

int ltompc_get_status_counts(ltompc_handle h, int* counts8, long long* iterations_sum) {
  if (!h) return fail("null handle");
  HIPCHECK(hipSetDevice(h->device));
  HIPCHECK(hipMemsetAsync(h->d_counts, 0, sizeof(int) * 32, h->stream));
  hipLaunchKernelGGL(k_status_counts, dim3((h->B + 255) / 256), dim3(256), 0, h->stream, h->W, h->d_counts,
                     reinterpret_cast<unsigned long long*>(h->d_counts + 8));
  HIPCHECK(hipGetLastError());
  int host[32];
  HIPCHECK(hipMemcpyAsync(host, h->d_counts, sizeof host, hipMemcpyDeviceToHost, h->stream));
  HIPCHECK(hipStreamSynchronize(h->stream));
  for (int i = 0; i < 8; i++) {
    if (counts8) counts8[i] = host[i];
    h->solver_counts[i] = host[16 + i];
  }
  if (iterations_sum) std::memcpy(iterations_sum, host + 8, sizeof(long long));
  return 0;
}

int ltompc_get_solver_status_counts(ltompc_handle h, int* counts8) {
  if (!h || !counts8) return fail("ltompc_get_solver_status_counts: null argument");
  for (int i = 0; i < 8; i++) counts8[i] = h->solver_counts[i];
  return 0;
}

int ltompc_get_history(ltompc_handle h, int* triples, int capacity) {
  if (!h) return fail("null handle");
  int n = (int)h->history.size() / 3;
  for (int i = 0; i < n && i < capacity; i++)
    for (int j = 0; j < 3; j++) triples[3 * i + j] = h->history[3 * i + j];
  return n;
}

long long ltompc_debug_fetch(ltompc_handle h, int which, void* out, long long nbytes) {
  if (!h) return fail("null handle");
  if (hipSetDevice(h->device) != hipSuccess || ensure_unpacked(h)) return fail("ltompc_debug_fetch: could not restore the caller's order");
  const size_t N = h->N, Bp = h->Bp, ni = h->K.bd.ni;
  const Work& W = h->W;
  const void* src[15] = {W.QP, W.RC, W.RS, W.SP, W.LS, W.dX, W.dU, W.dC, W.dT, W.dNU, W.nL1, W.nL2, W.st, W.si, W.DBG};
  const size_t sz[15] = {QP_NF * (N + 1) * Bp * 8, RC_NF * (N + 1) * Bp * 8, RS_NF * N * Bp * 8, SP_NF * N * Bp * 8,
                         3 * ((size_t)h->K.o.n_linesearch + 1) * N * Bp * 8, 8 * (N + 1) * Bp * 8, 2 * N * Bp * 8, 8 * N * Bp * 8,
                         ni * N * Bp * 8, ni * N * Bp * 8, 8 * N * Bp * 8, 8 * N * Bp * 8, (size_t)ST_NF * Bp * 8, (size_t)SI_NF * Bp * 4,
                         W.DBG ? 8 * N * Bp * 8 : 0};
  if (which < 0 || which > 14) return fail("ltompc_debug_fetch: bad array id");
  if (out && nbytes > 0) {
    size_t n = std::min((size_t)nbytes, sz[which]);
    if (hipSetDevice(h->device) != hipSuccess || hipMemcpyAsync(out, src[which], n, hipMemcpyDeviceToHost, h->stream) != hipSuccess ||
        hipStreamSynchronize(h->stream) != hipSuccess)
      return fail("ltompc_debug_fetch: copy failed");
  }
  return (long long)sz[which];
}

int ltompc_test_model(ltompc_handle h, int n, double eps, const double* x, const double* lam, double* f, double* J,
                      double* H, double* cval, double* cgrad, double* cH, double* gval, double* ggrad, double* gH) {
  if (!h || n < 1) return fail("ltompc_test_model: bad argument");
  HIPCHECK(hipSetDevice(h->device));
  const size_t sizes[12] = {8, 8, 8, 64, 64, 2, 16, 128, 3, 24, 192, 0};
  double* dev[11];
  const double* src[2] = {x, lam};
  double* dst[9] = {f, J, H, cval, cgrad, cH, gval, ggrad, gH};
  for (int i = 0; i < 11; i++) HIPCHECK(hipMalloc((void**)&dev[i], sizeof(double) * sizes[i] * n));
  for (int i = 0; i < 2; i++) HIPCHECK(hipMemcpy(dev[i], src[i], sizeof(double) * sizes[i] * n, hipMemcpyHostToDevice));
  hipLaunchKernelGGL(k_test_model, dim3((n + 63) / 64), dim3(64), 0, h->stream, h->K, n, eps, dev[0], dev[1], dev[2], dev[3],
                     dev[4], dev[5], dev[6], dev[7], dev[8], dev[9], dev[10]);
  HIPCHECK(hipStreamSynchronize(h->stream));
  for (int i = 0; i < 9; i++) HIPCHECK(hipMemcpy(dst[i], dev[2 + i], sizeof(double) * sizes[2 + i] * n, hipMemcpyDeviceToHost));
  for (int i = 0; i < 11; i++) (void)hipFree(dev[i]);
  return 0;
}

int ltompc_test_ellipse(ltompc_handle h, int n, const double* x, double* val, double* grad, double* H) {
  if (!h || n < 1 || !x || !val || !grad || !H) return fail("ltompc_test_ellipse: bad argument");
  HIPCHECK(hipSetDevice(h->device));
  double *dx, *dv, *dg, *dH;
  HIPCHECK(hipMalloc((void**)&dx, sizeof(double) * 8 * n));
  HIPCHECK(hipMalloc((void**)&dv, sizeof(double) * 2 * n));
  HIPCHECK(hipMalloc((void**)&dg, sizeof(double) * 16 * n));
  HIPCHECK(hipMalloc((void**)&dH, sizeof(double) * 128 * n));
  HIPCHECK(hipMemcpy(dx, x, sizeof(double) * 8 * n, hipMemcpyHostToDevice));
  hipLaunchKernelGGL(k_test_ellipse, dim3((n + 63) / 64), dim3(64), 0, h->stream, h->K, n, dx, dv, dg, dH);
  HIPCHECK(hipStreamSynchronize(h->stream));
  HIPCHECK(hipMemcpy(val, dv, sizeof(double) * 2 * n, hipMemcpyDeviceToHost));
  HIPCHECK(hipMemcpy(grad, dg, sizeof(double) * 16 * n, hipMemcpyDeviceToHost));
  HIPCHECK(hipMemcpy(H, dH, sizeof(double) * 128 * n, hipMemcpyDeviceToHost));
  (void)hipFree(dx), (void)hipFree(dv), (void)hipFree(dg), (void)hipFree(dH);
  return 0;
}

int ltompc_velocity_profile(int device, const ltompc_vp_vehicle* veh, int n, int batch, const double* s, const double* k,
                            const double* s_max, double* v, double* v_local, double* v_acclim, double* v_declim) {
  if (!veh || !s || !k || !s_max || !v) return fail("ltompc_velocity_profile: null argument");
  if (n < 2 || batch < 1) return fail("ltompc_velocity_profile: need n >= 2 samples and batch >= 1");
  if (veh->kind != 0 && veh->kind != 1) return fail("ltompc_velocity_profile: vehicle kind must be 0 (engine map) or 1 (MX-5)");
  if (veh->kind == 0 && (veh->n_map < 2 || veh->n_map > 16)) return fail("ltompc_velocity_profile: engine map needs 2 .. 16 points");
  if (!(veh->mass > 0)) return fail("ltompc_velocity_profile: mass must be positive");
  for (size_t i = 0; i < (size_t)n * batch; i++)
    if (!(k[i] >= 0.0) || !std::isfinite(s[i])) return fail("ltompc_velocity_profile: curvature must be >= 0 and s finite");
  int ndev = 0;
  HIPCHECK(hipGetDeviceCount(&ndev));
  if (device < 0 || device >= ndev) return fail("ltompc_velocity_profile: no such HIP device");
  HIPCHECK(hipSetDevice(device));
  const size_t nb = sizeof(double) * (size_t)n * batch;
  double *d_s = nullptr, *d_k = nullptr, *d_m = nullptr, *d_out = nullptr;
  hipError_t e = hipMalloc((void**)&d_s, nb);
  if (e == hipSuccess) e = hipMalloc((void**)&d_k, nb);
  if (e == hipSuccess) e = hipMalloc((void**)&d_m, sizeof(double) * batch);
  if (e == hipSuccess) e = hipMalloc((void**)&d_out, 4 * nb);
  if (e == hipSuccess) e = hipMemcpy(d_s, s, nb, hipMemcpyHostToDevice);
  if (e == hipSuccess) e = hipMemcpy(d_k, k, nb, hipMemcpyHostToDevice);
  if (e == hipSuccess) e = hipMemcpy(d_m, s_max, sizeof(double) * batch, hipMemcpyHostToDevice);
  if (e == hipSuccess) {
    const size_t nn = (size_t)n * batch;
    hipLaunchKernelGGL(k_velocity_profile, dim3((batch + 63) / 64), dim3(64), 0, 0, *veh, n, batch, d_s, d_k, d_m, d_out, d_out + nn, d_out + 2 * nn, d_out + 3 * nn);
    e = hipGetLastError();
    if (e == hipSuccess) e = hipDeviceSynchronize();
    if (e == hipSuccess) e = hipMemcpy(v, d_out, nb, hipMemcpyDeviceToHost);
    if (e == hipSuccess && v_local) e = hipMemcpy(v_local, d_out + nn, nb, hipMemcpyDeviceToHost);
    if (e == hipSuccess && v_acclim) e = hipMemcpy(v_acclim, d_out + 2 * nn, nb, hipMemcpyDeviceToHost);
    if (e == hipSuccess && v_declim) e = hipMemcpy(v_declim, d_out + 3 * nn, nb, hipMemcpyDeviceToHost);
  }
  (void)hipFree(d_s), (void)hipFree(d_k), (void)hipFree(d_m), (void)hipFree(d_out);
  if (e != hipSuccess) return fail(std::string("ltompc_velocity_profile: ") + hipGetErrorString(e));
  return 0;
}

}
```

### lap-time-optimization_amd/csrc/model.h

```cpp
#pragma once
#if defined(LTOMPC_HOST_HARNESS)
#include "hip_shim.h"
#else
#include <hip/hip_runtime.h>
#endif

#include "../../include/ltompc.h"

namespace ltompc {

constexpr int NX = 8;
constexpr int NU = 2;
constexpr int MAX_XB = 16;
constexpr int MAX_UB = 4;
constexpr int NNL = 3;
constexpr int NEL = 2;
constexpr int MAX_NI = MAX_UB + 2 * MAX_XB + NNL + NEL;

__host__ __device__ constexpr int sidx(int i, int j) { return i >= j ? i * (i + 1) / 2 + j : j * (j + 1) / 2 + i; }

#if defined(__HIP_DEVICE_COMPILE__)
template <class T> using gptr = __attribute__((address_space(1))) T*;
#else
template <class T> using gptr = T*;
#endif

struct Tables {
  int n;
  gptr<const double> s_kappa, kappa, s_arc, n_left, n_right, v_ref;
  double g0_kappa, inv_kappa, g0_arc, inv_arc;
  double period;
};

struct Bounds {
  int n_xb, n_ub, ni;
  int nel;
  int xb_idx[MAX_XB];
  double xb_sgn[MAX_XB];
  double xb_val[MAX_XB];
  int ub_idx[MAX_UB];
  double ub_sgn[MAX_UB];
  double ub_val[MAX_UB];
};

__device__ __forceinline__ void lut_eval(const double* __restrict__ grid, const double* __restrict__ y, int n, double g0,
                                         double inv, double period, double s, double eps, double& val, double& slope, double& curv) {
  if (period > 0.0) s -= period * floor((s - g0) / period);
  const double fi = (s - g0) * inv;
  int i = fi <= 0.0 ? 0 : (fi >= (double)(n - 2) ? n - 2 : (int)fi);
  int im = i > 0 ? i - 1 : 0, ip = i + 2 < n ? i + 2 : n - 1;
  double gm = grid[im], gi = grid[i], gi1 = grid[i + 1], gp = grid[ip];
  double ym = y[im], yi = y[i], yi1 = y[i + 1], yp = y[ip];
#if defined(__HIP_DEVICE_COMPILE__)
  asm volatile("" : "+v"(gm), "+v"(gi), "+v"(gi1), "+v"(gp), "+v"(ym), "+v"(yi), "+v"(yi1), "+v"(yp));
#endif
  if ((i > 0 && s < gi) || (i < n - 2 && s >= gi1)) {
    while (i > 0 && s < grid[i]) --i;
    while (i < n - 2 && s >= grid[i + 1]) ++i;
    im = i > 0 ? i - 1 : 0, ip = i + 2 < n ? i + 2 : n - 1;
    gm = grid[im], gi = grid[i], gi1 = grid[i + 1], gp = grid[ip];
    ym = y[im], yi = y[i], yi1 = y[i + 1], yp = y[ip];
  }
  double d = gi1 - gi;
  double sl = (yi1 - yi) / d;
  val = yi + sl * (s - gi);
  slope = sl;
  curv = 0.0;
  if (eps > 0.0) {
    int kn = -1;
    double z = 0.0, W = 0.0, sg = 0.0;
    if (i > 0) {
      double Wk = 0.5 * fmin(gi - gm, d), zz = s - gi;
      if (zz >= 0.0 && zz < Wk) kn = i, z = zz, W = Wk, sg = 1.0;
    }
    if (kn < 0 && i + 1 < n - 1) {
      double Wk = 0.5 * fmin(d, gp - gi1), zz = s - gi1;
      if (zz < 0.0 && -zz < Wk) kn = i + 1, z = zz, W = Wk, sg = -1.0;
    }
    if (kn > 0) {
      const bool left = kn == i;
      const double ga = left ? gm : gi, gb = left ? gi : gi1, gc = left ? gi1 : gp;
      const double ya = left ? ym : yi, yb = left ? yi : yi1, yc = left ? yi1 : yp;
      double sa = (yb - ya) / (gb - ga);
      double sb = (yc - yb) / (gc - gb);
      double J = sb - sa, R = sqrt(z * z + eps * eps), RW = sqrt(W * W + eps * eps);
      double a = (1.0 - W / RW) / (2.0 * W), b = W - RW - a * W * W;
      val += 0.5 * J * (R + a * z * z + b - sg * z);
      slope += 0.5 * J * (z / R + 2.0 * a * z - sg);
      curv = 0.5 * J * (eps * eps / (R * R * R) + 2.0 * a);
    }
  }
}
__device__ __forceinline__ double lut_val(const double* __restrict__ grid, const double* __restrict__ y, int n, double g0,
                                          double inv, double period, double s, double eps) {
  double v, sl, cv;
  lut_eval(grid, y, n, g0, inv, period, s, eps, v, sl, cv);
  return v;
}

struct Jet4 {
  double v, g[4], h[10];
};

__device__ __forceinline__ void pacejka_jet(double vx, double vy, double r, double delta, double l, double delta_on,
                                            double Bp, double Cp, double K, Jet4& F) {
  double a = vy + l * r;
  double q = a * a + vx * vx, iq = 1.0 / q;
  double ta = vx * iq, tb = -a * iq;
  double taa = -2.0 * a * vx * iq * iq, tbb = -taa, tab = (a * a - vx * vx) * iq * iq;
  double alpha = atan2(a, vx) - delta_on * delta;
  double ag[4] = {tb, ta, l * ta, -delta_on};
  double ah[10];
  ah[sidx(0, 0)] = tbb;
  ah[sidx(1, 0)] = tab;
  ah[sidx(1, 1)] = taa;
  ah[sidx(2, 0)] = l * tab;
  ah[sidx(2, 1)] = l * taa;
  ah[sidx(2, 2)] = l * l * taa;
  ah[sidx(3, 0)] = ah[sidx(3, 1)] = ah[sidx(3, 2)] = ah[sidx(3, 3)] = 0.0;
  double z = Bp * alpha, d = 1.0 + z * z, t = atan(z);
  double sc, cc;
  sincos(Cp * t, &sc, &cc);
  double cb = Cp * Bp / d;
  double p0 = -K * sc;
  double p1 = -K * cc * cb;
  double p2 = K * sc * cb * cb + 2.0 * K * cc * Cp * Bp * Bp * z / (d * d);
  F.v = p0;
#pragma unroll
  for (int i = 0; i < 4; i++) F.g[i] = p1 * ag[i];
#pragma unroll
  for (int i = 0; i < 4; i++)
#pragma unroll
    for (int j = 0; j <= i; j++) F.h[sidx(i, j)] = p2 * ag[i] * ag[j] + p1 * ah[sidx(i, j)];
}

__device__ __forceinline__ void jet4_mul_delta(const Jet4& F, double s0, double s1, double s2, Jet4& P) {
  P.v = F.v * s0;
#pragma unroll
  for (int i = 0; i < 4; i++) P.g[i] = F.g[i] * s0;
  P.g[3] += F.v * s1;
#pragma unroll
  for (int i = 0; i < 4; i++)
#pragma unroll
    for (int j = 0; j <= i; j++) P.h[sidx(i, j)] = F.h[sidx(i, j)] * s0;
#pragma unroll
  for (int i = 0; i < 3; i++) P.h[sidx(3, i)] += F.g[i] * s1;
  P.h[sidx(3, 3)] += 2.0 * F.g[3] * s1 + F.v * s2;
}

__device__ __forceinline__ void rhs_val(const ltompc_params& p, const Tables& T, double eps, const double* x,
                                        const double* u, double* f) {
  double kap = lut_val(T.s_kappa, T.kappa, T.n, T.g0_kappa, T.inv_kappa, T.period, x[0], eps);
  double n = x[1], mu = x[2], vx = x[3], vy = x[4], r = x[5], de = x[6], th = x[7];
  double sm, cm, sd, cd;
  sincos(mu, &sm, &cm);
  sincos(de, &sd, &cd);
  double sdot = (vx * cm - vy * sm) / (1.0 - n * kap);
  double af = atan2(vy + p.length_f * r, vx) - de;
  double ar = atan2(vy - p.length_r * r, vx);
  double L = p.length_f + p.length_r;
  double Fnf = p.length_r * p.mass * p.gravity / L, Fnr = p.length_f * p.mass * p.gravity / L;
  double Fyf = -Fnf * p.D_f * sin(p.C_f * atan(p.B_f * af));
  double Fyr = -Fnr * p.D_r * sin(p.C_r * atan(p.B_r * ar));
  double Fx = p.C_m * th - p.Cr_0 - p.Cr_2 * vx * vx;
  f[0] = sdot;
  f[1] = vx * sm + vy * cm;
  f[2] = r - kap * sdot;
  f[3] = (Fx - Fyf * sd + p.mass * vy * r) / p.mass;
  f[4] = (Fyr + Fyf * cd - p.mass * vx * r) / p.mass;
  f[5] = (Fyf * p.length_f * cd - Fyr * p.length_r + p.ptv * (sd / cd * vx / L - r)) / p.inertia_z;
  f[6] = u[0];
  f[7] = u[1];
}

__device__ __forceinline__ void rhs_derivs(const ltompc_params& p, const Tables& T, double eps, const double* x,
                                           double* f, double* J, const double* lam, double scale, double* H) {
  double s = x[0], n = x[1], mu = x[2], vx = x[3], vy = x[4], r = x[5], de = x[6], th = x[7];
#pragma unroll
  for (int i = 0; i < 48; i++) J[i] = 0.0;
  double kap, kp, kpp;
  lut_eval(T.s_kappa, T.kappa, T.n, T.g0_kappa, T.inv_kappa, T.period, s, eps, kap, kp, kpp);
  double sm, cm;
  sincos(mu, &sm, &cm);
  double w = vx * cm - vy * sm, nd = vx * sm + vy * cm;
  double g = 1.0 / (1.0 - n * kap), g2 = g * g, g3 = g2 * g;
  double g_s = n * kp * g2, g_n = kap * g2;
  double g_ss = n * kpp * g2 + 2.0 * n * n * kp * kp * g3;
  double g_sn = kp * g2 + 2.0 * n * kap * kp * g3;
  double g_nn = 2.0 * kap * kap * g3;
  double sdot = w * g;
  double S1[5] = {w * g_s, w * g_n, -nd * g, cm * g, -sm * g};
  f[0] = sdot;
  f[1] = nd;
  f[2] = r - kap * sdot;
#pragma unroll
  for (int j = 0; j < 5; j++) J[0 * 8 + j] = S1[j];
  J[1 * 8 + 2] = w, J[1 * 8 + 3] = sm, J[1 * 8 + 4] = cm;
  J[2 * 8 + 0] = -kp * sdot - kap * S1[0];
#pragma unroll
  for (int j = 1; j < 5; j++) J[2 * 8 + j] = -kap * S1[j];
  J[2 * 8 + 5] = 1.0;
  if (lam) {
    double S2[15];
    S2[sidx(0, 0)] = w * g_ss;
    S2[sidx(1, 0)] = w * g_sn;
    S2[sidx(1, 1)] = w * g_nn;
    S2[sidx(2, 0)] = -nd * g_s;
    S2[sidx(2, 1)] = -nd * g_n;
    S2[sidx(2, 2)] = -w * g;
    S2[sidx(3, 0)] = cm * g_s;
    S2[sidx(3, 1)] = cm * g_n;
    S2[sidx(3, 2)] = -sm * g;
    S2[sidx(3, 3)] = 0.0;
    S2[sidx(4, 0)] = -sm * g_s;
    S2[sidx(4, 1)] = -sm * g_n;
    S2[sidx(4, 2)] = -cm * g;
    S2[sidx(4, 3)] = 0.0;
    S2[sidx(4, 4)] = 0.0;
    double l0 = scale * lam[0], l1 = scale * lam[1], l2 = scale * lam[2];
    double c0 = l0 - l2 * kap;
#pragma unroll
    for (int i = 0; i < 15; i++) H[i] += c0 * S2[i];
    H[sidx(0, 0)] += l2 * (-kpp * sdot - 2.0 * kp * S1[0]);
#pragma unroll
    for (int j = 1; j < 5; j++) H[sidx(j, 0)] += l2 * (-kp * S1[j]);
    H[sidx(2, 2)] += l1 * (-nd);
    H[sidx(3, 2)] += l1 * cm;
    H[sidx(4, 2)] += l1 * (-sm);
  }
  double L = p.length_f + p.length_r;
  double Kf = p.length_r * p.mass * p.gravity / L * p.D_f, Kr = p.length_f * p.mass * p.gravity / L * p.D_r;
  Jet4 Ff, Fr, Ps, Pc;
  pacejka_jet(vx, vy, r, de, p.length_f, 1.0, p.B_f, p.C_f, Kf, Ff);
  pacejka_jet(vx, vy, r, de, -p.length_r, 0.0, p.B_r, p.C_r, Kr, Fr);
  double sd, cd;
  sincos(de, &sd, &cd);
  jet4_mul_delta(Ff, sd, cd, -sd, Ps);
  jet4_mul_delta(Ff, cd, -sd, -cd, Pc);
  double im = 1.0 / p.mass, iz = 1.0 / p.inertia_z;
  f[3] = (p.C_m * th - p.Cr_0 - p.Cr_2 * vx * vx - Ps.v) * im + vy * r;
  f[4] = (Fr.v + Pc.v) * im - vx * r;
  const double td = sd / cd, sec2 = 1.0 / (cd * cd), pz = p.ptv * iz, iL = 1.0 / L;
  f[5] = (p.length_f * Pc.v - p.length_r * Fr.v) * iz + pz * (td * vx * iL - r);
#pragma unroll
  for (int j = 0; j < 4; j++) {
    J[3 * 8 + 3 + j] = -Ps.g[j] * im;
    J[4 * 8 + 3 + j] = (Fr.g[j] + Pc.g[j]) * im;
    J[5 * 8 + 3 + j] = (p.length_f * Pc.g[j] - p.length_r * Fr.g[j]) * iz;
  }
  J[5 * 8 + 3] += pz * td * iL, J[5 * 8 + 5] += -pz, J[5 * 8 + 6] += pz * vx * sec2 * iL;
  J[3 * 8 + 3] += -2.0 * p.Cr_2 * vx * im;
  J[3 * 8 + 4] += r;
  J[3 * 8 + 5] += vy;
  J[3 * 8 + 7] = p.C_m * im;
  J[4 * 8 + 3] += -r;
  J[4 * 8 + 5] += -vx;
  if (lam) {
    double l3 = scale * lam[3], l4 = scale * lam[4], l5 = scale * lam[5];
    double cs = -l3 * im;
    double cc = l4 * im + l5 * p.length_f * iz;
    double cr = l4 * im - l5 * p.length_r * iz;
#pragma unroll
    for (int i = 0; i < 4; i++)
#pragma unroll
      for (int j = 0; j <= i; j++)
        H[sidx(3 + i, 3 + j)] += cs * Ps.h[sidx(i, j)] + cc * Pc.h[sidx(i, j)] + cr * Fr.h[sidx(i, j)];
    H[sidx(3, 3)] += l3 * (-2.0 * p.Cr_2 * im);
    H[sidx(6, 3)] += l5 * pz * sec2 * iL;
    H[sidx(6, 6)] += l5 * pz * vx * 2.0 * sec2 * td * iL;
    H[sidx(5, 4)] += l3;
    H[sidx(5, 3)] += -l4;
  }
}

__device__ __forceinline__ double cost_eval(const ltompc_params& p, const Tables& T, double eps, const double* x,
                                            bool terminal, double* g, double* H) {
  double n = x[1], mu = x[2], vx = x[3], vy = x[4], de = x[6];
  double val = p.q_n * n * n + p.q_mu * mu * mu + p.q_vy * vy * vy;
  if (g) {
    g[1] += 2.0 * p.q_n * n, g[2] += 2.0 * p.q_mu * mu, g[4] += 2.0 * p.q_vy * vy;
    H[sidx(1, 1)] += 2.0 * p.q_n, H[sidx(2, 2)] += 2.0 * p.q_mu, H[sidx(4, 4)] += 2.0 * p.q_vy;
  }
  if (terminal) return val;
  double vr, vr1, vr2;
  lut_eval(T.s_arc, T.v_ref, T.n, T.g0_arc, T.inv_arc, T.period, x[0], eps, vr, vr1, vr2);
  double cv = p.vref_scale;
  double e = vx - cv * vr;
  double rho = p.length_r / (p.length_f + p.length_r);
  double q = vx * vx + vy * vy, iq = 1.0 / q;
  double d = 1.0 + rho * rho * de * de;
  double b = atan(vy / vx) - atan(rho * de);
  val += p.q_v * e * e + p.q_B * b * b;
  if (g) {
    g[0] += -2.0 * p.q_v * e * cv * vr1;
    g[3] += 2.0 * p.q_v * e;
    H[sidx(0, 0)] += 2.0 * p.q_v * (cv * cv * vr1 * vr1 - e * cv * vr2);
    H[sidx(3, 0)] += -2.0 * p.q_v * cv * vr1;
    H[sidx(3, 3)] += 2.0 * p.q_v;
    double bx = -vy * iq, by = vx * iq, bd = -rho / d;
    double bxx = 2.0 * vx * vy * iq * iq, byy = -bxx, bxy = (vy * vy - vx * vx) * iq * iq;
    double bdd = 2.0 * rho * rho * rho * de / (d * d);
    double k2 = 2.0 * p.q_B;
    g[3] += k2 * b * bx, g[4] += k2 * b * by, g[6] += k2 * b * bd;
    H[sidx(3, 3)] += k2 * (bx * bx + b * bxx);
    H[sidx(4, 3)] += k2 * (bx * by + b * bxy);
    H[sidx(4, 4)] += k2 * (by * by + b * byy);
    H[sidx(6, 3)] += k2 * (bx * bd);
    H[sidx(6, 4)] += k2 * (by * bd);
    H[sidx(6, 6)] += k2 * (bd * bd + b * bdd);
  }
  return val;
}

__device__ __forceinline__ void cons_eval(const ltompc_params& p, const Tables& T, double eps, const double* x,
                                          double* val, double* gs, double* gn, double* gm, double* hss, double* hmm) {
  double NL, NL1, NL2, NR, NR1, NR2;
  lut_eval(T.s_arc, T.n_left, T.n, T.g0_arc, T.inv_arc, T.period, x[0], eps, NL, NL1, NL2);
  lut_eval(T.s_arc, T.n_right, T.n, T.g0_arc, T.inv_arc, T.period, x[0], eps, NR, NR1, NR2);
  double hl = 0.5 * (p.length_f + p.length_r), hw = 0.5 * p.width;
  double mu = x[2], sm, cm;
  sincos(mu, &sm, &cm);
  double sg = (mu > 0.0) - (mu < 0.0);
  double sabs = sg * sm;
  val[0] = x[1] - hl * sabs + hw * cm - NL;
  val[1] = -x[1] + hl * sm + hw * cm - NR;
  val[2] = -x[1] - hl * sm + hw * cm - NR;
  if (gs) {
    gs[0] = -NL1, gs[1] = -NR1, gs[2] = -NR1;
    gn[0] = 1.0, gn[1] = -1.0, gn[2] = -1.0;
    gm[0] = -hl * sg * cm - hw * sm;
    gm[1] = hl * cm - hw * sm;
    gm[2] = -hl * cm - hw * sm;
    hss[0] = -NL2, hss[1] = -NR2, hss[2] = -NR2;
    hmm[0] = hl * sg * sg * sabs - hw * cm;
    hmm[1] = -hl * sm - hw * cm;
    hmm[2] = hl * sm - hw * cm;
  }
}

__device__ __forceinline__ void ellipse_eval(const ltompc_params& p, const double* x, double* val, double (*g)[5], double (*h)[15]) {
  const double vx = x[3], vy = x[4], r = x[5], de = x[6], th = x[7];
  const double L = p.length_f + p.length_r;
  const double Kf = p.length_r * p.mass * p.gravity / L * p.D_f, Kr = p.length_f * p.mass * p.gravity / L * p.D_r;
  Jet4 F[2];
  pacejka_jet(vx, vy, r, de, p.length_f, 1.0, p.B_f, p.C_f, Kf, F[0]);
  pacejka_jet(vx, vy, r, de, -p.length_r, 0.0, p.B_r, p.C_r, Kr, F[1]);
  const double c = p.ell_rho * 0.5 * p.C_m, lng = c * th;
  const double iD[2] = {1.0 / (p.ell_D_f * p.ell_D_f), 1.0 / (p.ell_D_r * p.ell_D_r)};
#pragma unroll
  for (int q = 0; q < 2; q++) {
    val[q] = (lng * lng + F[q].v * F[q].v) * iD[q] - 1.0;
    if (g) {
#pragma unroll
      for (int a = 0; a < 4; a++) g[q][a] = 2.0 * F[q].v * F[q].g[a] * iD[q];
      g[q][4] = 2.0 * c * c * th * iD[q];
#pragma unroll
      for (int a = 0; a < 5; a++)
#pragma unroll
        for (int b = 0; b <= a; b++)
          h[q][sidx(a, b)] = a < 4 ? 2.0 * (F[q].g[a] * F[q].g[b] + F[q].v * F[q].h[sidx(a, b)]) * iD[q] : (b == 4 ? 2.0 * c * c * iD[q] : 0.0);
    }
  }
}
__device__ __forceinline__ void ellipse_val(const ltompc_params& p, const double* x, double* val) {
  const double vx = x[3], vy = x[4], r = x[5], de = x[6], th = x[7];
  const double af = atan2(vy + p.length_f * r, vx) - de, ar = atan2(vy - p.length_r * r, vx);
  const double L = p.length_f + p.length_r;
  const double Fnf = p.length_r * p.mass * p.gravity / L, Fnr = p.length_f * p.mass * p.gravity / L;
  const double Fyf = -Fnf * p.D_f * sin(p.C_f * atan(p.B_f * af)), Fyr = -Fnr * p.D_r * sin(p.C_r * atan(p.B_r * ar));
  const double lng = p.ell_rho * 0.5 * p.C_m * th;
  val[0] = (lng * lng + Fyf * Fyf) / (p.ell_D_f * p.ell_D_f) - 1.0;
  val[1] = (lng * lng + Fyr * Fyr) / (p.ell_D_r * p.ell_D_r) - 1.0;
}

__device__ __forceinline__ double bound_h(double sgn, double val, double x) { return sgn < 0.0 ? val - x : x - val; }

}
```

### lap-time-optimization_amd/solver.py

```python
from __future__ import annotations

import ctypes as C

import numpy as np

from . import _lib
from ._lib import LOOP_NAMES, NLOOP, NTHETA, NX, NU, TABLE_ROW_NAMES, TABLE_SLOT_NAMES, THETA_NAMES, Options, Params, check, dptr, iptr, lib
from .tables import TrackTables

KERNEL_CLASSES = ("eval", "riccati", "expand", "linesearch", "pick", "update", "riccati1", "step1")


class SolveRecord:

    def __init__(self, mpc, rec=None, parts=None):
        self._mpc, self._rec, self.parts, self._released = mpc, rec, parts, False

    @property
    def released(self) -> bool:
        return self._released

    def release(self):
        if self._released:
            return
# ... 324 lines not shown
                                               dptr(dth) if theta else None))
        out = dict(x_next=xn, dx=dx, du=du, names=THETA_NAMES)
        if theta:
            out["dtheta"] = dth
        return out

    def plant_sensitivities_dev(self, x_ptr: int, u_ptr: int, xn_ptr: int = 0, dx_ptr: int = 0, du_ptr: int = 0, dtheta_ptr: int = 0,
                                n_sub: int = 400):
        check(lib().ltompc_plant_sensitivities_dev(self._h, C.c_void_p(x_ptr), C.c_void_p(u_ptr), int(n_sub), C.c_void_p(xn_ptr or None),
                                                   C.c_void_p(dx_ptr or None), C.c_void_p(du_ptr or None), C.c_void_p(dtheta_ptr or None)))

    def loop_begin(self, mode: int = 3):
        check(lib().ltompc_loop_begin(self._h, int(mode)))

    def loop_tick_dev(self, x_ptr: int, u_ptr: int, xn_ptr: int, n_sub: int = 400):
        check(lib().ltompc_loop_tick_dev(self._h, C.c_void_p(x_ptr), C.c_void_p(u_ptr), int(n_sub), C.c_void_p(xn_ptr)))

    def loop_tick(self, x, u0, n_sub: int = 400):
        x, u0 = self._x(x), np.ascontiguousarray(np.asarray(u0, float).reshape(self.B, NU))
        xn = np.empty_like(x)
        check(lib().ltompc_loop_tick(self._h, dptr(x), dptr(u0), int(n_sub), dptr(xn)))
        return xn

    def loop_sensitivities(self):
        dx, du = np.empty((self.B, NX, NLOOP)), np.empty((self.B, NU, NLOOP))
        ok, ticks = np.empty(self.B, dtype=np.int32), np.empty(self.B, dtype=np.int32)
        check(lib().ltompc_get_loop_sensitivities(self._h, dptr(dx), dptr(du), iptr(ok), iptr(ticks)))
        return dict(dx=dx, du=du, ok=ok != 0, ticks=ticks, names=LOOP_NAMES)

    def loop_sensitivities_dev(self, dx_ptr: int = 0, du_ptr: int = 0, ok_ptr: int = 0):
        check(lib().ltompc_loop_sensitivities_dev(self._h, C.c_void_p(dx_ptr or None), C.c_void_p(du_ptr or None), C.c_void_p(ok_ptr or None)))

    def loop_end(self):
        check(lib().ltompc_loop_end(self._h))

    def theta(self):
        p = self.params
        return np.array([getattr(p, n) for n in THETA_NAMES[:-2]] + [p.r_du[0], p.r_du[1]])

    def set_table_values(self, row, values):
        r = _table_row(row)
        v = _table_values(values, self._tab.shape[1])
        check(lib().ltompc_set_table_values(self._h, r, dptr(v)))
        self._tables_changed()

    def set_table_values_dev(self, row, values_ptr: int):
        check(lib().ltompc_set_table_values_dev(self._h, _table_row(row), C.c_void_p(values_ptr)))
        self._tables_changed()

    def _tables_changed(self):
        self._solved = None
        self._fb = self._pfb = None
        self.solve_count += 1

    def table_values(self):
        out = np.empty((len(TABLE_ROW_NAMES), self._tab.shape[1]))
        for r in range(out.shape[0]):
            check(lib().ltompc_get_table_values(self._h, r, dptr(out[r])))
        return out

    def set_table_sets(self, values=None, index=None):
        if values is None and index is None:
            check(lib().ltompc_set_table_sets(self._h, 0, None, None))
            self.n_table_sets = 0
            self._tables_changed()
            return
        n_sets = self.n_table_sets
        if values is not None:
            values = _table_sets(values, self._tab.shape[1])
            n_sets = values.shape[0]
        elif not n_sets:
            raise ValueError("set_table_sets: values=None keeps the sets in effect, and there are none")
        if index is not None:
            index = _set_index(index, self.B, n_sets)
        elif n_sets < self._set_index_for:
            raise ValueError(f"set_table_sets: index=None keeps the index, which was written for {self._set_index_for} sets (now {n_sets})")
        check(lib().ltompc_set_table_sets(self._h, n_sets, dptr(values) if values is not None else None,
                                          iptr(index) if index is not None else None))
        self.n_table_sets = n_sets
        if index is not None:
            self._set_index_for = n_sets
        self._tables_changed()

    def set_table_sets_dev(self, n_sets: int, values_ptr: int = 0, index_ptr: int = 0):
        n_sets = int(n_sets)
        if n_sets < 0:
            raise ValueError(f"set_table_sets_dev: n_sets must be >= 0, got {n_sets}")
        if n_sets and not values_ptr and n_sets != self.n_table_sets:
            raise ValueError(f"set_table_sets_dev: values_ptr=0 keeps the sets in effect and needs n_sets unchanged ({self.n_table_sets} in effect, {n_sets} given)")
        if n_sets and not index_ptr and n_sets < self._set_index_for:
            raise ValueError(f"set_table_sets_dev: index_ptr=0 keeps the index, which was written for {self._set_index_for} sets (now {n_sets})")
        check(lib().ltompc_set_table_sets_dev(self._h, n_sets, C.c_void_p(values_ptr or None), C.c_void_p(index_ptr or None)))
        self.n_table_sets = n_sets
        if n_sets and index_ptr:
            self._set_index_for = n_sets
        self._tables_changed()

    def table_sets(self):
        n = C.c_int(0)
        check(lib().ltompc_get_table_sets(self._h, C.byref(n), None, None))
        if not n.value:
            return None
        values, index = np.empty((n.value, len(TABLE_ROW_NAMES), self._tab.shape[1])), np.empty(self.B, dtype=np.int32)
        check(lib().ltompc_get_table_sets(self._h, C.byref(n), dptr(values), iptr(index)))
        return values, index

    def adjoint_table_sets(self, gX=None, gU=None, slots: bool = False):
        B, N = self.B, self.N
        if not self.n_table_sets:
            raise ValueError("adjoint_table_sets: the handle has no table sets (set_table_sets); its table gradient is adjoint_tables()")
        if gX is not None:
            gX = _shaped("adjoint_table_sets", "gX", gX, (B, N + 1, NX))
        if gU is not None:
            gU = _shaped("adjoint_table_sets", "gU", gU, (B, N, NU))
        gs, ok = np.empty((self.n_table_sets, len(TABLE_ROW_NAMES), self._tab.shape[1])), np.empty(B, dtype=np.int32)
        sg = np.empty((B, N, len(TABLE_SLOT_NAMES))) if slots else None
        check(lib().ltompc_get_adjoint_table_sets(self._h, dptr(gX) if gX is not None else None, dptr(gU) if gU is not None else None,
                                                  dptr(gs), dptr(sg) if slots else None, iptr(ok)))
        out = dict(grad_sets=gs, names=TABLE_ROW_NAMES, ok=ok != 0)
        if slots:
            out.update(slot_grad=sg, slot_names=TABLE_SLOT_NAMES)
        return out

    def adjoint_table_sets_dev(self, gX_ptr: int, gU_ptr: int, grad_sets_ptr: int = 0, slot_grad_ptr: int = 0, ok_ptr: int = 0, add: bool = False):
        fn = lib().ltompc_adjoint_table_sets_add_dev if add else lib().ltompc_adjoint_table_sets_dev
        check(fn(self._h, C.c_void_p(gX_ptr or None), C.c_void_p(gU_ptr or None), C.c_void_p(grad_sets_ptr or None),
                 C.c_void_p(slot_grad_ptr or None), C.c_void_p(ok_ptr or None)))

    def set_theta(self, theta):
        if theta is None:
            check(lib().ltompc_set_instance_params(self._h, None))
            self._theta_rows = None
            return
        rows = self._theta_array(theta)
        check(lib().ltompc_set_instance_params(self._h, dptr(rows)))
        self._theta_rows = rows

    def set_theta_dev(self, theta_ptr: int):
        if not theta_ptr:
            self.set_theta(None)
            return
        check(lib().ltompc_set_instance_params_dev(self._h, C.c_void_p(theta_ptr)))
        self._theta_rows = _DEV_ROWS

    def _theta_array(self, theta):
        return _theta_rows(theta, self.B, self.theta())

    def instance_theta(self):
        out = np.empty((self.B, NTHETA))
        check(lib().ltompc_get_instance_params(self._h, dptr(out)))
        return out

    def feedback(self, x, u_prev=None, *, theta=None):
        if theta is not None:
            u = self.feedback(x, u_prev)
            if self._pfb is None:
                self._pfb = self.param_sensitivities()["du0_dtheta"]
            for name in theta:
                if name not in THETA_NAMES:
                    raise ValueError(f"feedback: unknown parameter {name!r} (one of {THETA_NAMES})")
            if self._theta_solved is None and all(np.ndim(v) == 0 for v in theta.values()):
                d = np.zeros(NTHETA)
                cur = self.theta()
                for name, v in theta.items():
                    j = THETA_NAMES.index(name)
                    d[j] = float(v) - cur[j]
                return u + np.einsum("bij,j->bi", self._pfb, d)
            cur = self._theta_solved if self._theta_solved is not None else np.tile(self.theta(), (self.B, 1))
            d = np.zeros((self.B, NTHETA))
            for name, v in theta.items():
                j = THETA_NAMES.index(name)
                v = np.asarray(v, dtype=np.float64)
                if v.shape not in ((), (self.B,)):
                    raise ValueError(f"feedback: {name} must be a scalar or a ({self.B},) array, got shape {v.shape}")
                d[:, j] = v - cur[:, j]
            return u + np.einsum("bij,bj->bi", self._pfb, d)
        if self._solved is None:
            raise _lib.LtompcError("feedback: no make_step to expand around (the last solve was not a host make_step, or an "
                                   "initial guess came after it)")
        x0s, ups, u0 = self._solved
        x = self._x(x)
        up = ups if u_prev is None else np.asarray(u_prev, dtype=np.float64).reshape(self.B, NU)
        if self._fb is None:
            S = self.sensitivities()
            self._fb = (S["du0_dx0"], S["du0_duprev"], S["ok"])
        Jx, Ju, ok = self._fb
        u = u0 + np.einsum("bij,bj->bi", Jx, x - x0s) + np.einsum("bij,bj->bi", Ju, up - ups)
        return np.where(ok[:, None], u, u0)

    def prediction(self):
        X, U = np.empty((self.B, self.N + 1, NX)), np.empty((self.B, self.N, NU))
        check(lib().ltompc_get_prediction(self._h, dptr(X), dptr(U)))
        return X, U

    def iterate(self):
        X, U = np.empty((self.B, self.N + 1, NX)), np.empty((self.B, self.N, NU))
        Cc, L1, L2 = (np.empty((self.B, self.N, NX)) for _ in range(3))
        check(lib().ltompc_get_iterate(self._h, dptr(X), dptr(Cc), dptr(U), dptr(L1), dptr(L2)))
        ni = C.c_int()
        check(lib().ltompc_get_ineq(self._h, None, None, C.byref(ni)))
        Tt, Nu = np.empty((self.B, self.N, ni.value)), np.empty((self.B, self.N, ni.value))
        check(lib().ltompc_get_ineq(self._h, dptr(Tt), dptr(Nu), C.byref(ni)))
        return dict(X=X, C=Cc, U=U, L1=L1, L2=L2, T=Tt, NU=Nu)

    def stats(self):
        st, it = np.empty(self.B, dtype=np.int32), np.empty(self.B, dtype=np.int32)
        kkt, obj, mu = np.empty(self.B), np.empty(self.B), np.empty(self.B)
        check(lib().ltompc_get_stats(self._h, iptr(st), iptr(it), dptr(kkt), dptr(obj), dptr(mu)))
        nr, nf = np.empty(self.B, dtype=np.int32), np.empty(self.B, dtype=np.int32)
        check(lib().ltompc_get_counters(self._h, iptr(nr), iptr(nf)))
        nre, viol = np.empty(self.B, dtype=np.int32), np.empty(self.B)
        check(lib().ltompc_get_restoration(self._h, iptr(nre), dptr(viol)))
        nsh, nfb, sst = (np.empty(self.B, dtype=np.int32) for _ in range(3))
        g0, pen = np.empty(self.B), np.empty(self.B)
        check(lib().ltompc_get_recovery(self._h, iptr(nsh), iptr(nfb), dptr(g0), iptr(sst), dptr(pen)))
        return dict(status=st, iters=it, kkt=kkt, obj=obj, mu=mu, n_reg=nr, n_lsfail=nf, n_resto=nre, viol=viol,
                    n_shift=nsh, n_fallback=nfb, g0=g0, status_solver=sst, penalty=pen)

    def plant_step(self, x, u, n_sub: int = 400):
        x, u = self._x(x), np.ascontiguousarray(np.asarray(u, float).reshape(self.B, NU))
        xn = np.empty_like(x)
        check(lib().ltompc_plant_step(self._h, dptr(x), dptr(u), int(n_sub), dptr(xn)))
        return xn

    def slip_forces(self, x):
        x = np.ascontiguousarray(np.asarray(x, float).reshape(-1, NX))
        a, F = np.empty((x.shape[0], 2)), np.empty((x.shape[0], 2))
        check(lib().ltompc_slip_forces(self._h, dptr(x), x.shape[0], dptr(a), dptr(F)))
        return a, F

    def synchronize(self):
        check(lib().ltompc_synchronize(self._h))

    def set_profiling(self, on, only: str | None = None):
        mode = int(bool(on))
        if on and only is not None:
            mode = 2 + KERNEL_CLASSES.index(only)
        check(lib().ltompc_set_profiling(self._h, mode))

    def set_poll_every(self, n: int):
        check(lib().ltompc_set_poll_every(self._h, int(n)))

    def set_narrow_width(self, width: int):
        check(lib().ltompc_set_narrow_width(self._h, int(width)))

    def timing(self):
        ms, ln = np.zeros(8), np.zeros(8, dtype=np.int32)
        launches, its = C.c_int(), C.c_int()
        check(lib().ltompc_get_timing(self._h, dptr(ms), iptr(ln), C.byref(launches), C.byref(its)))
        names = KERNEL_CLASSES
        return dict(ms={n: float(m) for n, m in zip(names, ms)}, launches_by_kernel={n: int(v) for n, v in zip(names, ln)},
                    launches=launches.value, ip_iterations=its.value)

    def launch_log(self, with_iterations: bool = False):
        L = lib()
        n = L.ltompc_get_launch_log(self._h, None, None, None, 0)
        kind, width, ms = np.empty(n, dtype=np.int32), np.empty(n, dtype=np.int32), np.empty(n)
        L.ltompc_get_launch_log(self._h, iptr(kind), iptr(width), dptr(ms), n)
        if not with_iterations:
            return kind, width, ms
        it = np.empty(n, dtype=np.int32)
        L.ltompc_get_launch_log_iterations(self._h, iptr(it), n)
        return kind, width, ms, it

    def active_history(self):
        n = lib().ltompc_get_active_history(self._h, None, 0)
        a = np.zeros(max(n, 1), dtype=np.int32)
        lib().ltompc_get_active_history(self._h, iptr(a), n)
        return a[:n]

    def status_counts(self):
        c, s = np.zeros(8, dtype=np.int32), C.c_longlong()
        check(lib().ltompc_get_status_counts(self._h, iptr(c), C.byref(s)))
        return c, int(s.value)

    def solver_status_counts(self):
        c = np.zeros(8, dtype=np.int32)
        check(lib().ltompc_get_solver_status_counts(self._h, iptr(c)))
        return c

    def history(self):
        buf = np.zeros((4096, 3), dtype=np.int32)
        n = lib().ltompc_get_history(self._h, iptr(buf), 4096)
        return buf[:max(0, min(n, 4096))]

    def debug_fetch(self, which: int):
        L = lib(); L.ltompc_debug_fetch.restype = C.c_longlong
        n = L.ltompc_debug_fetch(self._h, int(which), None, C.c_longlong(0))
        buf = np.empty(n // (4 if which == 13 else 8), dtype=np.int32 if which == 13 else np.float64)
        L.ltompc_debug_fetch(self._h, int(which), buf.ctypes.data_as(C.c_void_p), C.c_longlong(n))
        return buf

    def test_model(self, x, lam, eps: float = 0.0):
        x = np.ascontiguousarray(np.asarray(x, float).reshape(-1, NX))
        lam = np.ascontiguousarray(np.asarray(lam, float).reshape(-1, NX))
        n = x.shape[0]
        out = dict(f=np.empty((n, 8)), J=np.empty((n, 8, 8)), H=np.empty((n, 8, 8)), cval=np.empty((n, 2)),
                   cgrad=np.empty((n, 2, 8)), cH=np.empty((n, 2, 8, 8)), gval=np.empty((n, 3)),
                   ggrad=np.empty((n, 3, 8)), gH=np.empty((n, 3, 8, 8)))
        check(lib().ltompc_test_model(self._h, n, C.c_double(eps), dptr(x), dptr(lam),
                                      *(dptr(out[k]) for k in ("f", "J", "H", "cval", "cgrad", "cH", "gval", "ggrad", "gH"))))
        return out

    def test_ellipse(self, x):
        x = np.ascontiguousarray(np.asarray(x, float).reshape(-1, NX))
        n = x.shape[0]
        v, g, H = np.empty((n, 2)), np.empty((n, 2, 8)), np.empty((n, 2, 8, 8))
        check(lib().ltompc_test_ellipse(self._h, n, dptr(x), dptr(v), dptr(g), dptr(H)))
        return v, g, H

    def _x(self, x0):
        x0 = np.ascontiguousarray(np.asarray(x0, dtype=np.float64).reshape(-1, NX))
        if x0.shape[0] != self.B:
            raise ValueError(f"expected {self.B} states of dimension {NX}, got array of shape {x0.shape}")
        return x0


WS_UPREV = 7


def guess_collocation(X):
    X = np.asarray(X, dtype=np.float64)
    return np.ascontiguousarray(X[..., :-1, :] + (X[..., 1:, :] - X[..., :-1, :]) / 3.0)


def _mask(mask, B):
    m = np.asarray(mask)
    if m.shape != (B,):
        raise ValueError(f"mask must have shape ({B},), got {m.shape}")
    return np.ascontiguousarray(m != 0, dtype=np.int32)


def _indices(idx, B, unique):
    if idx is None:
        return None
    ix = np.ascontiguousarray(np.asarray(idx, dtype=np.int64).reshape(-1))
    if ix.size and (ix.min() < 0 or ix.max() >= B):
        raise ValueError(f"instance index out of range [0, {B})")
    if unique and np.unique(ix).size != ix.size:
        raise ValueError("an instance index appears twice")
    return ix.astype(np.int32)


def _shaped(who, name, a, shape):
    a = np.ascontiguousarray(a, dtype=np.float64)
    if a.shape != shape:
        raise ValueError(f"{who}: {name} must have shape {shape}, got {a.shape}")
    return a


_DEV_ROWS = object()


def _theta_rows(theta, B, base):
    if isinstance(theta, dict):
        rows = np.tile(base, (B, 1))
        for name, v in theta.items():
            if name not in THETA_NAMES:
                raise ValueError(f"set_theta: unknown parameter {name!r} (one of {THETA_NAMES})")
            v = np.asarray(v, dtype=np.float64)
            if v.shape not in ((), (B,)):
                raise ValueError(f"set_theta: {name} must be a scalar or a ({B},) array, got shape {v.shape}")
            rows[:, THETA_NAMES.index(name)] = v
    else:
        rows = np.asarray(theta, dtype=np.float64)
        if rows.shape != (B, NTHETA):
            raise ValueError(f"set_theta: theta must be ({B}, {NTHETA}) in THETA_NAMES order, got shape {rows.shape}")
    rows = np.array(rows, dtype=np.float64, order="C", copy=True)
    bad = ~np.isfinite(rows)
    bad[:, :2] |= ~(rows[:, :2] > 0)
    bad[:, 11:] |= ~(rows[:, 11:] >= 0)
    if bad.any():
        b, j = map(int, np.argwhere(bad)[0])
        raise ValueError(f"set_theta: row {b}, {THETA_NAMES[j]} = {rows[b, j]!r} (finite values; mass, inertia_z > 0; q_n, q_mu, q_B, "
                         f"r_du >= 0)")
    return rows


def _table_row(row):
    if isinstance(row, str):
        if row not in TABLE_ROW_NAMES:
            raise ValueError(f"set_table_values: unknown row {row!r} (one of {TABLE_ROW_NAMES})")
        return TABLE_ROW_NAMES.index(row)
    r = int(row)
    if not 0 <= r < len(TABLE_ROW_NAMES):
        raise ValueError(f"set_table_values: row must be in 0 .. {len(TABLE_ROW_NAMES) - 1} ({TABLE_ROW_NAMES}), got {row!r}")
    return r


def _table_values(values, n):
    v = np.array(values, dtype=np.float64, order="C", copy=True)
    if v.shape != (n,):
        raise ValueError(f"set_table_values: values must have shape ({n},), got {v.shape}")
    if not np.isfinite(v).all():
        raise ValueError(f"set_table_values: non-finite value at knot {int(np.argwhere(~np.isfinite(v))[0][0])}")
    return v


def _table_sets(values, n):
    v = np.array(values, dtype=np.float64, order="C", copy=True)
    if v.ndim != 3 or v.shape[0] < 1 or v.shape[1:] != (len(TABLE_ROW_NAMES), n):
        raise ValueError(f"set_table_sets: values must have shape (n_sets >= 1, {len(TABLE_ROW_NAMES)}, {n}), got {v.shape}")
    if not np.isfinite(v).all():
        g, r, i = map(int, np.argwhere(~np.isfinite(v))[0])
        raise ValueError(f"set_table_sets: non-finite value in set {g} ({TABLE_ROW_NAMES[r]}, knot {i})")
    return v


def _set_index(index, B, n_sets):
    ix = np.asarray(index)
    if ix.shape != (B,) or ix.dtype.kind not in "iu":
        raise ValueError(f"set_table_sets: index must be ({B},) integers, got shape {ix.shape}, dtype {ix.dtype}")
    bad = (ix < 0) | (ix >= n_sets)
    if bad.any():
        b = int(np.argwhere(bad)[0][0])
        raise ValueError(f"set_table_sets: index[{b}] = {int(ix[b])} is outside [0, {n_sets})")
    return np.array(ix, dtype=np.int32, order="C", copy=True)


class SplitMPC:

    def __init__(self, tables: TrackTables, n_horizon: int = 10, batch: int = 1, n_parts: int = 4, params: Params | None = None,
                 options: Options | None = None, device: int = 0, narrow_width: int | None = None):
        from concurrent.futures import ThreadPoolExecutor
        self.N, self.B, self.n_parts = int(n_horizon), int(batch), int(n_parts)
        base, rem = divmod(self.B, self.n_parts)
        self.bounds = []
        lo = 0
        for p in range(self.n_parts):
            hi = lo + base + (1 if p < rem else 0)
            self.bounds.append((lo, hi)); lo = hi
        self.parts = [BatchedMPC(tables, n_horizon, hi - lo, params=params, options=options, device=device) for lo, hi in self.bounds]
        self.options, self.params = self.parts[0].options, self.parts[0].params
        self.n_table = self.parts[0].n_table
        if narrow_width is None and self.n_parts >= 3:
            narrow_width = 128
        if narrow_width is not None:
            for p in self.parts:
                p.set_narrow_width(narrow_width)
        self._pool = ThreadPoolExecutor(max_workers=self.n_parts)

    def close(self):
        for p in self.parts:
            p.close()
        self._pool.shutdown(wait=True)

    def _each(self, fn):
        futs = [self._pool.submit(fn, p, lo, hi) for p, (lo, hi) in zip(self.parts, self.bounds)]
        return [f.result() for f in futs]

    def set_initial_guess_dev(self, x0_ptr: int):
        self._each(lambda p, lo, hi: (p.set_initial_guess_dev(x0_ptr + 8 * NX * lo), p.synchronize()))

    def make_step_dev(self, x0_ptr: int, u0_ptr: int):
        self._each(lambda p, lo, hi: p.make_step_dev(x0_ptr + 8 * NX * lo, u0_ptr + 8 * NU * lo))

    def run_ticks(self, x_ptr: int, u_ptr, xn_ptr: int, n_ticks: int, n_sub: int = 400, after_tick=None, before_tick=None,
                  loop: bool = False):
        ring = [int(u_ptr)] if isinstance(u_ptr, int) else [int(q) for q in u_ptr]
        def body(p, lo, hi):
            a, b = x_ptr + 8 * NX * lo, xn_ptr + 8 * NX * lo
            pi = self.parts.index(p)
            for t in range(n_ticks):
                if before_tick is not None:
                    before_tick(pi, t)
                u = ring[t % len(ring)] + 8 * NU * lo
                p.make_step_dev(a, u)
                (p.loop_tick_dev if loop else p.plant_step_dev)(a, u, b, n_sub)
                a, b = b, a
                if after_tick is not None:
                    after_tick(pi, t)
            p.synchronize()
        self._each(body)

    def rollout_dev(self, x_ptr: int, n_ticks: int, n_sub: int = 400, u_log_ptr: int = 0, status_log_ptr: int = 0, iters_log_ptr: int = 0):
        def body(p, lo, hi):
            return p.rollout_dev(x_ptr + 8 * NX * lo, n_ticks, n_sub, u_log_ptr + 8 * NU * n_ticks * lo if u_log_ptr else 0,
                                 status_log_ptr + 4 * n_ticks * lo if status_log_ptr else 0, iters_log_ptr + 4 * n_ticks * lo if iters_log_ptr else 0)
        r = self._each(body)
        return dict(iterations=max(q["iterations"] for q in r), launches=sum(q["launches"] for q in r), per_part=r)

    def synchronize(self):
        for p in self.parts:
            p.synchronize()

    def set_poll_every(self, n: int):
        for p in self.parts:
            p.set_poll_every(n)

    def set_profiling(self, on, only: str | None = None):
        for p in self.parts:
            p.set_profiling(on, only)

    def status_counts(self):
        r = [p.status_counts() for p in self.parts]
        return sum(c for c, _ in r), sum(s for _, s in r)

    def solver_status_counts(self):
        return sum(p.solver_status_counts() for p in self.parts)

    def stats(self):
        r = [p.stats() for p in self.parts]
        return {k: np.concatenate([q[k] for q in r]) for k in r[0]}

    def iterate(self):
        r = [p.iterate() for p in self.parts]
        return {k: np.concatenate([q[k] for q in r]) for k in r[0]}

    def reset(self, mask, x0):
        m = _mask(mask, self.B)
        x0 = np.asarray(x0, dtype=np.float64).reshape(-1, NX)
        if x0.shape[0] != self.B:
            raise ValueError(f"reset: expected {self.B} states of dimension {NX}, got array of shape {x0.shape}")
        if not np.isfinite(x0[m != 0]).all():
            raise ValueError("reset: non-finite x0 in a masked row")
        for p, (lo, hi) in zip(self.parts, self.bounds):
            if m[lo:hi].any():
                p.reset(m[lo:hi], x0[lo:hi])

    def reset_dev(self, mask_ptr: int, x0_ptr: int):
        for p, (lo, hi) in zip(self.parts, self.bounds):
            p.reset_dev(mask_ptr + 4 * lo, x0_ptr + 8 * NX * lo)

    def set_guess(self, mask, X, U, C=None, u_prev=None):
        B, N = self.B, self.N
        m = _mask(mask, B)
        X, U = _shaped("set_guess", "X", X, (B, N + 1, NX)), _shaped("set_guess", "U", U, (B, N, NU))
        Cc = guess_collocation(X) if C is None else _shaped("set_guess", "C", C, (B, N, NX))
        up = None if u_prev is None else _shaped("set_guess", "u_prev", u_prev, (B, NU))
        on = m != 0
        if not (np.isfinite(X[on]).all() and np.isfinite(U[on]).all() and np.isfinite(Cc[on]).all() and (up is None or np.isfinite(up[on]).all())):
            raise ValueError("set_guess: non-finite entry in a masked row")
        for p, (lo, hi) in zip(self.parts, self.bounds):
            if m[lo:hi].any():
                p.set_guess(m[lo:hi], X[lo:hi], U[lo:hi], Cc[lo:hi], None if up is None else up[lo:hi])

    def set_guess_dev(self, mask_ptr: int, X_ptr: int, C_ptr: int, U_ptr: int, u_prev_ptr: int = 0):
        N = self.N
        for p, (lo, hi) in zip(self.parts, self.bounds):
            p.set_guess_dev(mask_ptr + 4 * lo, X_ptr + 8 * (N + 1) * NX * lo, C_ptr + 8 * N * NX * lo, U_ptr + 8 * N * NU * lo,
                            u_prev_ptr + 8 * NU * lo if u_prev_ptr else 0)

    @property
    def warm_state_size(self) -> int:
        return self.parts[0].warm_state_size

    def _by_part(self, ix):
        for p, (lo, hi) in zip(self.parts, self.bounds):
            rows = np.flatnonzero((ix >= lo) & (ix < hi))
            if rows.size:
                yield p, rows, ix[rows] - lo

    def export_state(self, idx=None):
        ix = np.arange(self.B, dtype=np.int32) if idx is None else _indices(idx, self.B, unique=False)
        blob = np.empty((ix.size, self.warm_state_size))
        for p, rows, local in self._by_part(ix):
            blob[rows] = p.export_state(local)
        return blob

    def import_state(self, blob, idx=None):
        blob = np.asarray(blob, dtype=np.float64)
        ix = np.arange(blob.shape[0], dtype=np.int32) if idx is None else _indices(idx, self.B, unique=True)
        if blob.ndim != 2 or blob.shape != (ix.size, self.warm_state_size) or ix.size > self.B:
            raise ValueError(f"import_state: blob must be (n <= {self.B}, {self.warm_state_size}) with one row per index, got {blob.shape}")
        for p, rows, local in self._by_part(ix):
            p.import_state(blob[rows], local)

    def set_theta(self, theta):
        if theta is None:
            self._each(lambda p, lo, hi: p.set_theta(None))
            return
        rows = _theta_rows(theta, self.B, self.parts[0].theta())
        for p, (lo, hi) in zip(self.parts, self.bounds):
            p.set_theta(rows[lo:hi])

    def instance_theta(self):
        return np.concatenate([p.instance_theta() for p in self.parts])

    def set_table_values(self, row, values):
        r, v = _table_row(row), _table_values(values, self.n_table)
        for p in self.parts:
            p.set_table_values(r, v)

    def set_table_values_dev(self, row, values_ptr: int):
        r = _table_row(row)
        for p in self.parts:
            p.set_table_values_dev(r, values_ptr)

    def table_values(self):
        return self.parts[0].table_values()

    @property
    def n_table_sets(self):
        return self.parts[0].n_table_sets

    def set_table_sets(self, values=None, index=None):
        if values is None and index is None:
            for p in self.parts:
                p.set_table_sets(None, None)
            return
        n_sets = self.n_table_sets
        if values is not None:
            values = _table_sets(values, self.n_table)
            n_sets = values.shape[0]
        elif not n_sets:
            raise ValueError("set_table_sets: values=None keeps the sets in effect, and there are none")
# ... 186 lines not shown
```

Measured before the change: 166,200.

## Batch and prefetch track lookup-table loads ahead of model evaluation

Splits the lookup-table evaluation into three phases: a fetch of the grid and knot values, a register pin, and a finish step. All five lookups per slot (curvature at both points, reference speed, left and right track width) are issued up front, in the linearisation and in the line search, before the dynamics, cost and constraint code runs. Overloads of rhs, cost and constraint evaluation now take the precomputed values, and the line search also hoists its slack and dual loads next to the table fetches. The aim is to overlap global-memory latency with the sincos and tire-model arithmetic instead of stalling on serial dependent loads. In exchange, register pressure rises from holding the raw knots, and a new test entry point checks that batched and direct lookups agree.

```diff
diff --git a/include/ltompc.h b/include/ltompc.h
--- a/include/ltompc.h
+++ b/include/ltompc.h
@@ -215,6 +215,8 @@
                       double* J, double* H, double* cval, double* cgrad, double* cH, double* gval,
                       double* ggrad, double* gH);
 
+int ltompc_test_lut(ltompc_handle h, int n, double eps, const double* s, double* direct, double* batched);
+
 int ltompc_test_ellipse(ltompc_handle h, int n, const double* x, double* val, double* grad, double* H);
 
 typedef struct ltompc_vp_vehicle {
diff --git a/lap-time-optimization_amd/csrc/aux_kernels.h b/lap-time-optimization_amd/csrc/aux_kernels.h
--- a/lap-time-optimization_amd/csrc/aux_kernels.h
+++ b/lap-time-optimization_amd/csrc/aux_kernels.h
@@ -388,6 +388,29 @@
 }
 
 
+__device__ __forceinline__ void test_lut_point(const Tables& T, const double eps, const double sc, const double sx, double* direct,
+                                               double* batched) {
+  lut_eval(T.s_kappa, T.kappa, T.n, T.g0_kappa, T.inv_kappa, T.period, sc, eps, direct[0], direct[1], direct[2]);
+  lut_eval(T.s_kappa, T.kappa, T.n, T.g0_kappa, T.inv_kappa, T.period, sx, eps, direct[3], direct[4], direct[5]);
+  lut_eval(T.s_arc, T.v_ref, T.n, T.g0_arc, T.inv_arc, T.period, sx, eps, direct[6], direct[7], direct[8]);
+  lut_eval(T.s_arc, T.n_left, T.n, T.g0_arc, T.inv_arc, T.period, sx, eps, direct[9], direct[10], direct[11]);
+  lut_eval(T.s_arc, T.n_right, T.n, T.g0_arc, T.inv_arc, T.period, sx, eps, direct[12], direct[13], direct[14]);
+  SlotLutsRaw R;
+  SlotLuts L;
+  slot_luts_fetch(T, sc, sx, R);
+  slot_luts_pin(R);
+  slot_luts_finish(T, R, eps, true, true, L);
+  const Lut3 l[5] = {L.kc, L.kx, L.vr, L.nl, L.nr};
+  for (int q = 0; q < 5; q++) batched[3 * q] = l[q].v, batched[3 * q + 1] = l[q].d1, batched[3 * q + 2] = l[q].d2;
+}
+__global__ void k_test_lut(Consts K, int n, double eps, const double* __restrict__ s, double* __restrict__ direct, double* __restrict__ batched) {
+  int t = blockIdx.x * blockDim.x + threadIdx.x;
+  if (t >= n) return;
+  double d[15], c[15];
+  test_lut_point(K.T, eps, s[t], s[n - 1 - t], d, c);
+  for (int q = 0; q < 15; q++) direct[(size_t)t * 15 + q] = d[q], batched[(size_t)t * 15 + q] = c[q];
+}
+
 __global__ void k_test_ellipse(Consts K, int n, const double* __restrict__ x, double* __restrict__ val, double* __restrict__ grad, double* __restrict__ H) {
   int t = blockIdx.x * blockDim.x + threadIdx.x;
   if (t >= n) return;
diff --git a/lap-time-optimization_amd/csrc/linearise.h b/lap-time-optimization_amd/csrc/linearise.h
--- a/lap-time-optimization_amd/csrc/linearise.h
+++ b/lap-time-optimization_amd/csrc/linearise.h
@@ -139,6 +139,7 @@
 template <bool WITH_DUAL, class BP, bool ELL, bool PI = false, bool TS = false>
 __device__ __forceinline__ void linearise_slot(const Consts& K, const Work& W, int k, int b, double eps, Slot& S) {
   const int N = W.N;
+  constexpr bool LUT_ONE = WITH_DUAL, LUT_POINT = !WITH_DUAL && !TS;
   const double hdt = K.o.t_step, rho = W.st[(size_t)ST_RHO * W.Bp + b];
 #pragma unroll
   for (int i = 0; i < 8; i++) {
@@ -152,13 +153,35 @@
   for (int i = 0; i < 8; i++) l1[i] = PL(W.L1, i, k, N), l2[i] = PL(W.L2, i, k, N);
 #pragma unroll
   for (int i = 0; i < 36; i++) S.Hc[i] = 0.0, S.Hxp[i] = 0.0;
+  const bool nl_early = (k + 1 <= N - 1);
+  SlotLutsRaw lraw;
+  SlotLuts lut;
+  if constexpr (LUT_ONE) {
+    const Tables& Tb = inst_tables<TS>(K.T, W, b);
+    slot_luts_fetch(Tb, S.c[0], S.xp[0], lraw);
+    slot_luts_pin(lraw);
+    slot_luts_finish(Tb, lraw, eps, k != N - 1, nl_early, lut);
+  } else if constexpr (LUT_POINT) {
+    const Tables& Tb = inst_tables<TS>(K.T, W, b);
+    slot_luts_fetch_c(Tb, S.c[0], lraw);
+    slot_luts_pin_c(lraw);
+    slot_luts_finish_c(Tb, lraw, eps, lut);
+  }
   double f1[8], f2[8], J[48];
-  rhs_derivs(inst_params<PI>(K.p, W, b), inst_tables<TS>(K.T, W, b), eps, S.c, f1, J, l1, hdt, S.Hc);
+  if constexpr (LUT_ONE || LUT_POINT) rhs_derivs(inst_params<PI>(K.p, W, b), lut.kc, S.c, f1, J, l1, hdt, S.Hc);
+  else rhs_derivs(inst_params<PI>(K.p, W, b), inst_tables<TS>(K.T, W, b), eps, S.c, f1, J, l1, hdt, S.Hc);
 #pragma unroll
   for (int i = 0; i < 64; i++) S.E1[i] = 0.0, S.E2[i] = 0.0;
 #pragma unroll
   for (int i = 0; i < 48; i++) S.E1[i] = hdt * J[i];
-  rhs_derivs(inst_params<PI>(K.p, W, b), inst_tables<TS>(K.T, W, b), eps, S.xp, f2, J, l2, hdt, S.Hxp);
+  if constexpr (LUT_POINT) {
+    const Tables& Tb = inst_tables<TS>(K.T, W, b);
+    slot_luts_fetch_x(Tb, S.xp[0], lraw);
+    slot_luts_pin_x(lraw);
+    slot_luts_finish_x(Tb, lraw, eps, k != N - 1, nl_early, lut);
+  }
+  if constexpr (LUT_ONE || LUT_POINT) rhs_derivs(inst_params<PI>(K.p, W, b), lut.kx, S.xp, f2, J, l2, hdt, S.Hxp);
+  else rhs_derivs(inst_params<PI>(K.p, W, b), inst_tables<TS>(K.T, W, b), eps, S.xp, f2, J, l2, hdt, S.Hxp);
 #pragma unroll
   for (int i = 0; i < 48; i++) S.E2[i] = hdt * J[i];
   f1[6] = f2[6] = S.u[0], f1[7] = f2[7] = S.u[1];
@@ -170,7 +193,8 @@
   }
 #pragma unroll
   for (int i = 0; i < 8; i++) S.gcost[i] = 0.0, S.gc0[i] = 0.0, S.gc1[i] = 0.0, S.gxp1[i] = 0.0, S.dcd[i] = 0.0;
-  S.cost = cost_eval(inst_params<PI>(K.p, W, b), inst_tables<TS>(K.T, W, b), eps, S.xp, k == N - 1, S.gcost, S.Hxp);
+  if constexpr (LUT_ONE || LUT_POINT) S.cost = cost_eval(inst_params<PI>(K.p, W, b), lut.vr, S.xp, k == N - 1, S.gcost, S.Hxp);
+  else S.cost = cost_eval(inst_params<PI>(K.p, W, b), inst_tables<TS>(K.T, W, b), eps, S.xp, k == N - 1, S.gcost, S.Hxp);
 #pragma unroll
   for (int i = 0; i < 8; i++) S.gxp0[i] = S.gcost[i], S.dxd[i] = S.gcost[i];
   S.Du[0] = S.Du[1] = 0.0, S.gub0[0] = S.gub0[1] = 0.0, S.gub1[0] = S.gub1[1] = 0.0, S.dud[0] = S.dud[1] = 0.0;
@@ -211,7 +235,8 @@
     asm volatile("" : "+v"(tq[0]), "+v"(tq[1]), "+v"(tq[2]), "+v"(nq[0]), "+v"(nq[1]), "+v"(nq[2]), "+v"(eq[0]), "+v"(eq[1]), "+v"(eq[2]));
 #endif
     double hss[3], hmm[3];
-    cons_eval(K.p, inst_tables<TS>(K.T, W, b), eps, S.xp, S.gv, S.gs, S.gn, S.gm, hss, hmm);
+    if constexpr (LUT_ONE || LUT_POINT) cons_eval(K.p, lut.nl, lut.nr, S.xp, S.gv, S.gs, S.gn, S.gm, hss, hmm);
+    else cons_eval(K.p, inst_tables<TS>(K.T, W, b), eps, S.xp, S.gv, S.gs, S.gn, S.gm, hss, hmm);
 #pragma unroll
     for (int q = 0; q < 3; q++) {
       int mm = m_nl + q;
diff --git a/lap-time-optimization_amd/csrc/linesearch.h b/lap-time-optimization_amd/csrc/linesearch.h
--- a/lap-time-optimization_amd/csrc/linesearch.h
+++ b/lap-time-optimization_amd/csrc/linesearch.h
@@ -40,33 +40,64 @@
     for (int i = 0; i < 8; i++) txk[i] = xk[i] + alpha * dxk[i], txp[i] = xp[i] + alpha * dxp[i], tc[i] = c[i] + alpha * dc[i];
 #pragma unroll
     for (int i = 0; i < 2; i++) tu[i] = u[i] + alpha * du[i], tv[i] = v[i] + alpha * dv[i];
+    const Tables& Tb = inst_tables<TS>(K.T, W, b);
+#if defined(__HIP_DEVICE_COMPILE__)
+    if (!PIN) {
+      asm volatile("" : "+v"(tc[0]), "+v"(tc[1]), "+v"(tc[2]), "+v"(tc[3]), "+v"(tc[4]), "+v"(tc[5]), "+v"(tc[6]), "+v"(tc[7]),
+                        "+v"(txp[0]), "+v"(txp[1]), "+v"(txp[2]), "+v"(txp[3]), "+v"(txp[4]), "+v"(txp[5]), "+v"(txp[6]), "+v"(txp[7]),
+                        "+v"(txk[0]), "+v"(txk[1]), "+v"(txk[2]), "+v"(txk[3]), "+v"(txk[4]), "+v"(txk[5]), "+v"(txk[6]), "+v"(txk[7]),
+                        "+v"(tu[0]), "+v"(tu[1]), "+v"(tv[0]), "+v"(tv[1]));
+    }
+#endif
+    SlotLutsRaw lraw;
+    slot_luts_fetch(Tb, tc[0], txp[0], lraw);
+    constexpr int NTR = ELL ? 5 : 3;
+    double tn[NTR], dtn[NTR], en[NTR], den[NTR];
+    const auto fetch_track = [&](const int m0) {
+#pragma unroll
+      for (int q = 0; q < NTR; q++) {
+        tn[q] = PL(W.T, m0 + q, k, N), dtn[q] = PL(W.dT, m0 + q, k, N);
+        en[q] = PL(W.T, K.bd.ni + q, k, N), den[q] = PL(W.dT, K.bd.ni + q, k, N);
+      }
+    };
+    double t0[BP::fixed ? MAX_NI : 1] = {}, d0[BP::fixed ? MAX_NI : 1] = {};
+    const auto fetch_bounds = [&] { for_each_bound<BP>(K.p, [&](int mm, int, int, double, double) { t0[mm] = PL(W.T, mm, k, N), d0[mm] = PL(W.dT, mm, k, N); }); };
+    const int nb = BP::fixed ? for_each_bound<BP>(K.p, [](int, int, int, double, double) {}) : 0;
+    if (BP::fixed && PIN) fetch_bounds();
+    if (BP::fixed) fetch_track(nb);
+    slot_luts_pin(lraw);
+    SlotLuts lut;
+    slot_luts_finish(Tb, lraw, eps, k != N - 1, nl, lut);
+#if defined(__HIP_DEVICE_COMPILE__)
+    if (BP::fixed) {
+#pragma unroll
+      for (int q = 0; q < MAX_NI; q += 8)
+        if (PIN && q < nb) {
+          double* a = t0 + q;
+          double* c = d0 + q;
+          asm volatile("" : "+v"(a[0]), "+v"(a[1]), "+v"(a[2]), "+v"(a[3]), "+v"(a[4]), "+v"(a[5]), "+v"(a[6]), "+v"(a[7]),
+                            "+v"(c[0]), "+v"(c[1]), "+v"(c[2]), "+v"(c[3]), "+v"(c[4]), "+v"(c[5]), "+v"(c[6]), "+v"(c[7]));
+        }
+#pragma unroll
+      for (int q = 0; q < NTR; q++) asm volatile("" : "+v"(tn[q]), "+v"(dtn[q]), "+v"(en[q]), "+v"(den[q]));
+    }
+#endif
     double f1[8], f2[8];
-    rhs_val(inst_params<PI>(K.p, W, b), inst_tables<TS>(K.T, W, b), eps, tc, tu, f1);
-    rhs_val(inst_params<PI>(K.p, W, b), inst_tables<TS>(K.T, W, b), eps, txp, tu, f2);
+    rhs_val(inst_params<PI>(K.p, W, b), lut.kc.v, tc, tu, f1);
+    rhs_val(inst_params<PI>(K.p, W, b), lut.kx.v, txp, tu, f2);
     double th = 0.0;
 #pragma unroll
     for (int i = 0; i < 8; i++) {
       th += fabs(hdt * f1[i] + 2.0 * txk[i] - 1.5 * tc[i] - 0.5 * txp[i]);
       th += fabs(hdt * f2[i] - 2.0 * txk[i] + 4.5 * tc[i] - 2.5 * txp[i]);
     }
-    double co = cost_eval(inst_params<PI>(K.p, W, b), inst_tables<TS>(K.T, W, b), eps, txp, k == N - 1, nullptr, nullptr);
+    double co = cost_eval(inst_params<PI>(K.p, W, b), lut.vr, txp, k == N - 1, nullptr, nullptr);
 #pragma unroll
     for (int i = 0; i < 2; i++) co += inst_r_du<PI>(K.p, W, b, i) * (tu[i] - tv[i]) * (tu[i] - tv[i]);
     double sl = 0.0, pr = 1.0;
     double tt[BP::fixed ? MAX_NI : 1];
     if (BP::fixed) {
-      double t0[MAX_NI] = {}, d0[MAX_NI] = {};
-      const int nb = for_each_bound<BP>(K.p, [&](int mm, int, int, double, double) { t0[mm] = PL(W.T, mm, k, N), d0[mm] = PL(W.dT, mm, k, N); });
-#pragma unroll
-      for (int q = 0; q < MAX_NI; q += 8)
-        if (PIN && q < nb) {
-#if defined(__HIP_DEVICE_COMPILE__)
-          double* a = t0 + q;
-          double* c = d0 + q;
-          asm volatile("" : "+v"(a[0]), "+v"(a[1]), "+v"(a[2]), "+v"(a[3]), "+v"(a[4]), "+v"(a[5]), "+v"(a[6]), "+v"(a[7]),
-                            "+v"(c[0]), "+v"(c[1]), "+v"(c[2]), "+v"(c[3]), "+v"(c[4]), "+v"(c[5]), "+v"(c[6]), "+v"(c[7]));
-#endif
-        }
+      if (!PIN) fetch_bounds();
 #pragma unroll
       for (int q = 0; q < MAX_NI; q++)
         if (q < nb) tt[q] = t0[q] + alpha * d0[q];
@@ -77,16 +108,17 @@
       th += fabs(sg * (xv - val) + t), pr *= t;
       if ((mm & 7) == 7) sl += log(pr), pr = 1.0;
     });
+    if (!BP::fixed) fetch_track(m);
     if (nl) {
       double gv[3];
-      cons_eval(K.p, inst_tables<TS>(K.T, W, b), eps, txp, gv, nullptr, nullptr, nullptr, nullptr, nullptr);
+      cons_eval(K.p, lut.nl, lut.nr, txp, gv, nullptr, nullptr, nullptr, nullptr, nullptr);
 #pragma unroll
       for (int q = 0; q < 3; q++) {
-        double t = PL(W.T, m + q, k, N) + alpha * PL(W.dT, m + q, k, N);
+        double t = tn[q] + alpha * dtn[q];
         double e = 0.0;
         pr *= t;
         if (rho > 0.0) {
-          e = PL(W.T, K.bd.ni + q, k, N) + alpha * PL(W.dT, K.bd.ni + q, k, N);
+          e = en[q] + alpha * den[q];
           pr *= e, co += rho * e;
         }
         th += fabs(gv[q] - e + t);
@@ -97,9 +129,9 @@
         ellipse_val(K.p, txp, ge);
 #pragma unroll
         for (int q = 0; q < 2; q++) {
-          const int mm = m + 3 + q, me = K.bd.ni + 3 + q;
-          const double t = PL(W.T, mm, k, N) + alpha * PL(W.dT, mm, k, N);
-          const double e = PL(W.T, me, k, N) + alpha * PL(W.dT, me, k, N);
+          const int mm = m + 3 + q;
+          const double t = tn[NTR - 2 + q] + alpha * dtn[NTR - 2 + q];
+          const double e = en[NTR - 2 + q] + alpha * den[NTR - 2 + q];
           pr *= t, pr *= e, co += K.p.ell_penalty * e;
           th += fabs(ge[q] - e + t);
           if ((mm & 7) == 7) sl += log(pr), pr = 1.0;
diff --git a/lap-time-optimization_amd/csrc/ltompc.hip b/lap-time-optimization_amd/csrc/ltompc.hip
--- a/lap-time-optimization_amd/csrc/ltompc.hip
+++ b/lap-time-optimization_amd/csrc/ltompc.hip
@@ -1431,6 +1431,22 @@
   return 0;
 }
 
+int ltompc_test_lut(ltompc_handle h, int n, double eps, const double* s, double* direct, double* batched) {
+  if (!h || n < 1 || !s || !direct || !batched) return fail("ltompc_test_lut: bad argument");
+  HIPCHECK(hipSetDevice(h->device));
+  double *ds, *dd, *db;
+  HIPCHECK(hipMalloc((void**)&ds, sizeof(double) * n));
+  HIPCHECK(hipMalloc((void**)&dd, sizeof(double) * 15 * n));
+  HIPCHECK(hipMalloc((void**)&db, sizeof(double) * 15 * n));
+  HIPCHECK(hipMemcpy(ds, s, sizeof(double) * n, hipMemcpyHostToDevice));
+  hipLaunchKernelGGL(k_test_lut, dim3((n + 63) / 64), dim3(64), 0, h->stream, h->K, n, eps, ds, dd, db);
+  HIPCHECK(hipStreamSynchronize(h->stream));
+  HIPCHECK(hipMemcpy(direct, dd, sizeof(double) * 15 * n, hipMemcpyDeviceToHost));
+  HIPCHECK(hipMemcpy(batched, db, sizeof(double) * 15 * n, hipMemcpyDeviceToHost));
+  (void)hipFree(ds), (void)hipFree(dd), (void)hipFree(db);
+  return 0;
+}
+
 int ltompc_test_ellipse(ltompc_handle h, int n, const double* x, double* val, double* grad, double* H) {
   if (!h || n < 1 || !x || !val || !grad || !H) return fail("ltompc_test_ellipse: bad argument");
   HIPCHECK(hipSetDevice(h->device));
diff --git a/lap-time-optimization_amd/csrc/model.h b/lap-time-optimization_amd/csrc/model.h
--- a/lap-time-optimization_amd/csrc/model.h
+++ b/lap-time-optimization_amd/csrc/model.h
@@ -98,6 +98,128 @@
   return v;
 }
 
+struct LutAt {
+  double s;
+  int i;
+  double gm, gi, gi1, gp;
+};
+struct LutKnots {
+  double ym, yi, yi1, yp;
+};
+struct Lut3 {
+  double v, d1, d2;
+};
+__device__ __forceinline__ void lut_at(const double* __restrict__ grid, int n, double g0, double inv, double period, double s, LutAt& A) {
+  if (period > 0.0) s -= period * floor((s - g0) / period);
+  const double fi = (s - g0) * inv;
+  const int i = fi <= 0.0 ? 0 : (fi >= (double)(n - 2) ? n - 2 : (int)fi);
+  const int im = i > 0 ? i - 1 : 0, ip = i + 2 < n ? i + 2 : n - 1;
+  A.s = s, A.i = i;
+  A.gm = grid[im], A.gi = grid[i], A.gi1 = grid[i + 1], A.gp = grid[ip];
+}
+__device__ __forceinline__ void lut_knots(const double* __restrict__ y, int n, const LutAt& A, LutKnots& Y) {
+  const int i = A.i, im = i > 0 ? i - 1 : 0, ip = i + 2 < n ? i + 2 : n - 1;
+  Y.ym = y[im], Y.yi = y[i], Y.yi1 = y[i + 1], Y.yp = y[ip];
+}
+__device__ __forceinline__ void lut_pin(LutAt& A) {
+#if defined(__HIP_DEVICE_COMPILE__)
+  asm volatile("" : "+v"(A.gm), "+v"(A.gi), "+v"(A.gi1), "+v"(A.gp));
+#endif
+}
+__device__ __forceinline__ void lut_pin(LutKnots& Y) {
+#if defined(__HIP_DEVICE_COMPILE__)
+  asm volatile("" : "+v"(Y.ym), "+v"(Y.yi), "+v"(Y.yi1), "+v"(Y.yp));
+#endif
+}
+__device__ __forceinline__ void lut_finish(const double* __restrict__ grid, const double* __restrict__ y, int n, const LutAt& A,
+                                           const LutKnots& Y, double eps, Lut3& out) {
+  const double s = A.s;
+  int i = A.i;
+  int im, ip;
+  double gm = A.gm, gi = A.gi, gi1 = A.gi1, gp = A.gp;
+  double ym = Y.ym, yi = Y.yi, yi1 = Y.yi1, yp = Y.yp;
+  if ((i > 0 && s < gi) || (i < n - 2 && s >= gi1)) {
+    while (i > 0 && s < grid[i]) --i;
+    while (i < n - 2 && s >= grid[i + 1]) ++i;
+    im = i > 0 ? i - 1 : 0, ip = i + 2 < n ? i + 2 : n - 1;
+    gm = grid[im], gi = grid[i], gi1 = grid[i + 1], gp = grid[ip];
+    ym = y[im], yi = y[i], yi1 = y[i + 1], yp = y[ip];
+  }
+  double d = gi1 - gi;
+  double sl = (yi1 - yi) / d;
+  double val = yi + sl * (s - gi);
+  double slope = sl;
+  double curv = 0.0;
+  if (eps > 0.0) {
+    int kn = -1;
+    double z = 0.0, W = 0.0, sg = 0.0;
+    if (i > 0) {
+      double Wk = 0.5 * fmin(gi - gm, d), zz = s - gi;
+      if (zz >= 0.0 && zz < Wk) kn = i, z = zz, W = Wk, sg = 1.0;
+    }
+    if (kn < 0 && i + 1 < n - 1) {
+      double Wk = 0.5 * fmin(d, gp - gi1), zz = s - gi1;
+      if (zz < 0.0 && -zz < Wk) kn = i + 1, z = zz, W = Wk, sg = -1.0;
+    }
+    if (kn > 0) {
+      const bool left = kn == i;
+      const double ga = left ? gm : gi, gb = left ? gi : gi1, gc = left ? gi1 : gp;
+      const double ya = left ? ym : yi, yb = left ? yi : yi1, yc = left ? yi1 : yp;
+      double sa = (yb - ya) / (gb - ga);
+      double sb = (yc - yb) / (gc - gb);
+      double J = sb - sa, R = sqrt(z * z + eps * eps), RW = sqrt(W * W + eps * eps);
+      double a = (1.0 - W / RW) / (2.0 * W), b = W - RW - a * W * W;
+      val += 0.5 * J * (R + a * z * z + b - sg * z);
+      slope += 0.5 * J * (z / R + 2.0 * a * z - sg);
+      curv = 0.5 * J * (eps * eps / (R * R * R) + 2.0 * a);
+    }
+  }
+  out.v = val, out.d1 = slope, out.d2 = curv;
+}
+
+struct SlotLutsRaw {
+  LutAt akc, akx, aax;
+  LutKnots kc, kx, vr, nl, nr;
+};
+struct SlotLuts {
+  Lut3 kc, kx, vr, nl, nr;
+};
+__device__ __forceinline__ void slot_luts_fetch_c(const Tables& T, double sc, SlotLutsRaw& R) {
+  lut_at(T.s_kappa, T.n, T.g0_kappa, T.inv_kappa, T.period, sc, R.akc);
+  lut_knots(T.kappa, T.n, R.akc, R.kc);
+}
+__device__ __forceinline__ void slot_luts_fetch_x(const Tables& T, double sx, SlotLutsRaw& R) {
+  lut_at(T.s_kappa, T.n, T.g0_kappa, T.inv_kappa, T.period, sx, R.akx);
+  lut_at(T.s_arc, T.n, T.g0_arc, T.inv_arc, T.period, sx, R.aax);
+  lut_knots(T.kappa, T.n, R.akx, R.kx);
+  lut_knots(T.v_ref, T.n, R.aax, R.vr), lut_knots(T.n_left, T.n, R.aax, R.nl), lut_knots(T.n_right, T.n, R.aax, R.nr);
+}
+__device__ __forceinline__ void slot_luts_fetch(const Tables& T, double sc, double sx, SlotLutsRaw& R) {
+  slot_luts_fetch_c(T, sc, R), slot_luts_fetch_x(T, sx, R);
+}
+__device__ __forceinline__ void slot_luts_pin_c(SlotLutsRaw& R) { lut_pin(R.akc), lut_pin(R.kc); }
+__device__ __forceinline__ void slot_luts_pin_x(SlotLutsRaw& R) {
+  lut_pin(R.akx), lut_pin(R.aax), lut_pin(R.kx), lut_pin(R.vr), lut_pin(R.nl), lut_pin(R.nr);
+}
+__device__ __forceinline__ void slot_luts_pin(SlotLutsRaw& R) { slot_luts_pin_c(R), slot_luts_pin_x(R); }
+__device__ __forceinline__ void slot_luts_finish_c(const Tables& T, const SlotLutsRaw& R, double eps, SlotLuts& L) {
+  lut_finish(T.s_kappa, T.kappa, T.n, R.akc, R.kc, eps, L.kc);
+}
+__device__ __forceinline__ void slot_luts_finish_x(const Tables& T, const SlotLutsRaw& R, double eps, bool stage_cost, bool track,
+                                                   SlotLuts& L) {
+  lut_finish(T.s_kappa, T.kappa, T.n, R.akx, R.kx, eps, L.kx);
+  L.vr = L.nl = L.nr = Lut3{0.0, 0.0, 0.0};
+  if (stage_cost) lut_finish(T.s_arc, T.v_ref, T.n, R.aax, R.vr, eps, L.vr);
+  if (track) {
+    lut_finish(T.s_arc, T.n_left, T.n, R.aax, R.nl, eps, L.nl);
+    lut_finish(T.s_arc, T.n_right, T.n, R.aax, R.nr, eps, L.nr);
+  }
+}
+__device__ __forceinline__ void slot_luts_finish(const Tables& T, const SlotLutsRaw& R, double eps, bool stage_cost, bool track,
+                                                 SlotLuts& L) {
+  slot_luts_finish_c(T, R, eps, L), slot_luts_finish_x(T, R, eps, stage_cost, track, L);
+}
+
 struct Jet4 {
   double v, g[4], h[10];
 };
@@ -148,6 +270,28 @@
   P.h[sidx(3, 3)] += 2.0 * F.g[3] * s1 + F.v * s2;
 }
 
+__device__ __forceinline__ void rhs_val(const ltompc_params& p, const double kap, const double* x, const double* u, double* f) {
+  double n = x[1], mu = x[2], vx = x[3], vy = x[4], r = x[5], de = x[6], th = x[7];
+  double sm, cm, sd, cd;
+  sincos(mu, &sm, &cm);
+  sincos(de, &sd, &cd);
+  double sdot = (vx * cm - vy * sm) / (1.0 - n * kap);
+  double af = atan2(vy + p.length_f * r, vx) - de;
+  double ar = atan2(vy - p.length_r * r, vx);
+  double L = p.length_f + p.length_r;
+  double Fnf = p.length_r * p.mass * p.gravity / L, Fnr = p.length_f * p.mass * p.gravity / L;
+  double Fyf = -Fnf * p.D_f * sin(p.C_f * atan(p.B_f * af));
+  double Fyr = -Fnr * p.D_r * sin(p.C_r * atan(p.B_r * ar));
+  double Fx = p.C_m * th - p.Cr_0 - p.Cr_2 * vx * vx;
+  f[0] = sdot;
+  f[1] = vx * sm + vy * cm;
+  f[2] = r - kap * sdot;
+  f[3] = (Fx - Fyf * sd + p.mass * vy * r) / p.mass;
+  f[4] = (Fyr + Fyf * cd - p.mass * vx * r) / p.mass;
+  f[5] = (Fyf * p.length_f * cd - Fyr * p.length_r + p.ptv * (sd / cd * vx / L - r)) / p.inertia_z;
+  f[6] = u[0];
+  f[7] = u[1];
+}
 __device__ __forceinline__ void rhs_val(const ltompc_params& p, const Tables& T, double eps, const double* x,
                                         const double* u, double* f) {
   double kap = lut_val(T.s_kappa, T.kappa, T.n, T.g0_kappa, T.inv_kappa, T.period, x[0], eps);
@@ -173,13 +317,12 @@
   f[7] = u[1];
 }
 
-__device__ __forceinline__ void rhs_derivs(const ltompc_params& p, const Tables& T, double eps, const double* x,
+__device__ __forceinline__ void rhs_derivs(const ltompc_params& p, const Lut3& kappa, const double* x,
                                            double* f, double* J, const double* lam, double scale, double* H) {
-  double s = x[0], n = x[1], mu = x[2], vx = x[3], vy = x[4], r = x[5], de = x[6], th = x[7];
+  double n = x[1], mu = x[2], vx = x[3], vy = x[4], r = x[5], de = x[6], th = x[7];
 #pragma unroll
   for (int i = 0; i < 48; i++) J[i] = 0.0;
-  double kap, kp, kpp;
-  lut_eval(T.s_kappa, T.kappa, T.n, T.g0_kappa, T.inv_kappa, T.period, s, eps, kap, kp, kpp);
+  const double kap = kappa.v, kp = kappa.d1, kpp = kappa.d2;
   double sm, cm;
   sincos(mu, &sm, &cm);
   double w = vx * cm - vy * sm, nd = vx * sm + vy * cm;
@@ -272,7 +415,143 @@
     H[sidx(5, 3)] += -l4;
   }
 }
-
+__device__ __forceinline__ void rhs_derivs(const ltompc_params& p, const Tables& T, double eps, const double* x,
+                                           double* f, double* J, const double* lam, double scale, double* H) {
+  double s = x[0], n = x[1], mu = x[2], vx = x[3], vy = x[4], r = x[5], de = x[6], th = x[7];
+#pragma unroll
+  for (int i = 0; i < 48; i++) J[i] = 0.0;
+  double kap, kp, kpp;
+  lut_eval(T.s_kappa, T.kappa, T.n, T.g0_kappa, T.inv_kappa, T.period, s, eps, kap, kp, kpp);
+  double sm, cm;
+  sincos(mu, &sm, &cm);
+  double w = vx * cm - vy * sm, nd = vx * sm + vy * cm;
+  double g = 1.0 / (1.0 - n * kap), g2 = g * g, g3 = g2 * g;
+  double g_s = n * kp * g2, g_n = kap * g2;
+  double g_ss = n * kpp * g2 + 2.0 * n * n * kp * kp * g3;
+  double g_sn = kp * g2 + 2.0 * n * kap * kp * g3;
+  double g_nn = 2.0 * kap * kap * g3;
+  double sdot = w * g;
+  double S1[5] = {w * g_s, w * g_n, -nd * g, cm * g, -sm * g};
+  f[0] = sdot;
+  f[1] = nd;
+  f[2] = r - kap * sdot;
+#pragma unroll
+  for (int j = 0; j < 5; j++) J[0 * 8 + j] = S1[j];
+  J[1 * 8 + 2] = w, J[1 * 8 + 3] = sm, J[1 * 8 + 4] = cm;
+  J[2 * 8 + 0] = -kp * sdot - kap * S1[0];
+#pragma unroll
+  for (int j = 1; j < 5; j++) J[2 * 8 + j] = -kap * S1[j];
+  J[2 * 8 + 5] = 1.0;
+  if (lam) {
+    double S2[15];
+    S2[sidx(0, 0)] = w * g_ss;
+    S2[sidx(1, 0)] = w * g_sn;
+    S2[sidx(1, 1)] = w * g_nn;
+    S2[sidx(2, 0)] = -nd * g_s;
+    S2[sidx(2, 1)] = -nd * g_n;
+    S2[sidx(2, 2)] = -w * g;
+    S2[sidx(3, 0)] = cm * g_s;
+    S2[sidx(3, 1)] = cm * g_n;
+    S2[sidx(3, 2)] = -sm * g;
+    S2[sidx(3, 3)] = 0.0;
+    S2[sidx(4, 0)] = -sm * g_s;
+    S2[sidx(4, 1)] = -sm * g_n;
+    S2[sidx(4, 2)] = -cm * g;
+    S2[sidx(4, 3)] = 0.0;
+    S2[sidx(4, 4)] = 0.0;
+    double l0 = scale * lam[0], l1 = scale * lam[1], l2 = scale * lam[2];
+    double c0 = l0 - l2 * kap;
+#pragma unroll
+    for (int i = 0; i < 15; i++) H[i] += c0 * S2[i];
+    H[sidx(0, 0)] += l2 * (-kpp * sdot - 2.0 * kp * S1[0]);
+#pragma unroll
+    for (int j = 1; j < 5; j++) H[sidx(j, 0)] += l2 * (-kp * S1[j]);
+    H[sidx(2, 2)] += l1 * (-nd);
+    H[sidx(3, 2)] += l1 * cm;
+    H[sidx(4, 2)] += l1 * (-sm);
+  }
+  double L = p.length_f + p.length_r;
+  double Kf = p.length_r * p.mass * p.gravity / L * p.D_f, Kr = p.length_f * p.mass * p.gravity / L * p.D_r;
+  Jet4 Ff, Fr, Ps, Pc;
+  pacejka_jet(vx, vy, r, de, p.length_f, 1.0, p.B_f, p.C_f, Kf, Ff);
+  pacejka_jet(vx, vy, r, de, -p.length_r, 0.0, p.B_r, p.C_r, Kr, Fr);
+  double sd, cd;
+  sincos(de, &sd, &cd);
+  jet4_mul_delta(Ff, sd, cd, -sd, Ps);
+  jet4_mul_delta(Ff, cd, -sd, -cd, Pc);
+  double im = 1.0 / p.mass, iz = 1.0 / p.inertia_z;
+  f[3] = (p.C_m * th - p.Cr_0 - p.Cr_2 * vx * vx - Ps.v) * im + vy * r;
+  f[4] = (Fr.v + Pc.v) * im - vx * r;
+  const double td = sd / cd, sec2 = 1.0 / (cd * cd), pz = p.ptv * iz, iL = 1.0 / L;
+  f[5] = (p.length_f * Pc.v - p.length_r * Fr.v) * iz + pz * (td * vx * iL - r);
+#pragma unroll
+  for (int j = 0; j < 4; j++) {
+    J[3 * 8 + 3 + j] = -Ps.g[j] * im;
+    J[4 * 8 + 3 + j] = (Fr.g[j] + Pc.g[j]) * im;
+    J[5 * 8 + 3 + j] = (p.length_f * Pc.g[j] - p.length_r * Fr.g[j]) * iz;
+  }
+  J[5 * 8 + 3] += pz * td * iL, J[5 * 8 + 5] += -pz, J[5 * 8 + 6] += pz * vx * sec2 * iL;
+  J[3 * 8 + 3] += -2.0 * p.Cr_2 * vx * im;
+  J[3 * 8 + 4] += r;
+  J[3 * 8 + 5] += vy;
+  J[3 * 8 + 7] = p.C_m * im;
+  J[4 * 8 + 3] += -r;
+  J[4 * 8 + 5] += -vx;
+  if (lam) {
+    double l3 = scale * lam[3], l4 = scale * lam[4], l5 = scale * lam[5];
+    double cs = -l3 * im;
+    double cc = l4 * im + l5 * p.length_f * iz;
+    double cr = l4 * im - l5 * p.length_r * iz;
+#pragma unroll
+    for (int i = 0; i < 4; i++)
+#pragma unroll
+      for (int j = 0; j <= i; j++)
+        H[sidx(3 + i, 3 + j)] += cs * Ps.h[sidx(i, j)] + cc * Pc.h[sidx(i, j)] + cr * Fr.h[sidx(i, j)];
+    H[sidx(3, 3)] += l3 * (-2.0 * p.Cr_2 * im);
+    H[sidx(6, 3)] += l5 * pz * sec2 * iL;
+    H[sidx(6, 6)] += l5 * pz * vx * 2.0 * sec2 * td * iL;
+    H[sidx(5, 4)] += l3;
+    H[sidx(5, 3)] += -l4;
+  }
+}
+
+__device__ __forceinline__ double cost_eval(const ltompc_params& p, const Lut3& vref, const double* x,
+                                            bool terminal, double* g, double* H) {
+  double n = x[1], mu = x[2], vx = x[3], vy = x[4], de = x[6];
+  double val = p.q_n * n * n + p.q_mu * mu * mu + p.q_vy * vy * vy;
+  if (g) {
+    g[1] += 2.0 * p.q_n * n, g[2] += 2.0 * p.q_mu * mu, g[4] += 2.0 * p.q_vy * vy;
+    H[sidx(1, 1)] += 2.0 * p.q_n, H[sidx(2, 2)] += 2.0 * p.q_mu, H[sidx(4, 4)] += 2.0 * p.q_vy;
+  }
+  if (terminal) return val;
+  const double vr = vref.v, vr1 = vref.d1, vr2 = vref.d2;
+  double cv = p.vref_scale;
+  double e = vx - cv * vr;
+  double rho = p.length_r / (p.length_f + p.length_r);
+  double q = vx * vx + vy * vy, iq = 1.0 / q;
+  double d = 1.0 + rho * rho * de * de;
+  double b = atan(vy / vx) - atan(rho * de);
+  val += p.q_v * e * e + p.q_B * b * b;
+  if (g) {
+    g[0] += -2.0 * p.q_v * e * cv * vr1;
+    g[3] += 2.0 * p.q_v * e;
+    H[sidx(0, 0)] += 2.0 * p.q_v * (cv * cv * vr1 * vr1 - e * cv * vr2);
+    H[sidx(3, 0)] += -2.0 * p.q_v * cv * vr1;
+    H[sidx(3, 3)] += 2.0 * p.q_v;
+    double bx = -vy * iq, by = vx * iq, bd = -rho / d;
+    double bxx = 2.0 * vx * vy * iq * iq, byy = -bxx, bxy = (vy * vy - vx * vx) * iq * iq;
+    double bdd = 2.0 * rho * rho * rho * de / (d * d);
+    double k2 = 2.0 * p.q_B;
+    g[3] += k2 * b * bx, g[4] += k2 * b * by, g[6] += k2 * b * bd;
+    H[sidx(3, 3)] += k2 * (bx * bx + b * bxx);
+    H[sidx(4, 3)] += k2 * (bx * by + b * bxy);
+    H[sidx(4, 4)] += k2 * (by * by + b * byy);
+    H[sidx(6, 3)] += k2 * (bx * bd);
+    H[sidx(6, 4)] += k2 * (by * bd);
+    H[sidx(6, 6)] += k2 * (bd * bd + b * bdd);
+  }
+  return val;
+}
 __device__ __forceinline__ double cost_eval(const ltompc_params& p, const Tables& T, double eps, const double* x,
                                             bool terminal, double* g, double* H) {
   double n = x[1], mu = x[2], vx = x[3], vy = x[4], de = x[6];
@@ -312,6 +591,29 @@
   return val;
 }
 
+__device__ __forceinline__ void cons_eval(const ltompc_params& p, const Lut3& nleft, const Lut3& nright, const double* x,
+                                          double* val, double* gs, double* gn, double* gm, double* hss, double* hmm) {
+  const double NL = nleft.v, NL1 = nleft.d1, NL2 = nleft.d2, NR = nright.v, NR1 = nright.d1, NR2 = nright.d2;
+  double hl = 0.5 * (p.length_f + p.length_r), hw = 0.5 * p.width;
+  double mu = x[2], sm, cm;
+  sincos(mu, &sm, &cm);
+  double sg = (mu > 0.0) - (mu < 0.0);
+  double sabs = sg * sm;
+  val[0] = x[1] - hl * sabs + hw * cm - NL;
+  val[1] = -x[1] + hl * sm + hw * cm - NR;
+  val[2] = -x[1] - hl * sm + hw * cm - NR;
+  if (gs) {
+    gs[0] = -NL1, gs[1] = -NR1, gs[2] = -NR1;
+    gn[0] = 1.0, gn[1] = -1.0, gn[2] = -1.0;
+    gm[0] = -hl * sg * cm - hw * sm;
+    gm[1] = hl * cm - hw * sm;
+    gm[2] = -hl * cm - hw * sm;
+    hss[0] = -NL2, hss[1] = -NR2, hss[2] = -NR2;
+    hmm[0] = hl * sg * sg * sabs - hw * cm;
+    hmm[1] = -hl * sm - hw * cm;
+    hmm[2] = hl * sm - hw * cm;
+  }
+}
 __device__ __forceinline__ void cons_eval(const ltompc_params& p, const Tables& T, double eps, const double* x,
                                           double* val, double* gs, double* gn, double* gm, double* hss, double* hmm) {
   double NL, NL1, NL2, NR, NR1, NR2;
diff --git a/lap-time-optimization_amd/solver.py b/lap-time-optimization_amd/solver.py
--- a/lap-time-optimization_amd/solver.py
+++ b/lap-time-optimization_amd/solver.py
@@ -650,6 +650,13 @@
                                       *(dptr(out[k]) for k in ("f", "J", "H", "cval", "cgrad", "cH", "gval", "ggrad", "gH"))))
         return out
 
+    def test_lut(self, s, eps: float = 0.0):
+        s = np.ascontiguousarray(np.asarray(s, float).ravel())
+        n = s.shape[0]
+        direct, batched = np.empty((n, 5, 3)), np.empty((n, 5, 3))
+        check(lib().ltompc_test_lut(self._h, n, C.c_double(eps), dptr(s), dptr(direct), dptr(batched)))
+        return direct, batched
+
     def test_ellipse(self, x):
         x = np.ascontiguousarray(np.asarray(x, float).reshape(-1, NX))
         n = x.shape[0]
```

Result: faster. 169,600 (median of 6 runs) (+2.0%).
